# viridityzhu/HiFiHR

Hardware: AMD Instinct MI355X
Metric: train images/sec, FreiHAND 224x224 (ResNet-18 + MANO LBS + render + losses + Adam) (higher is better)
Workload: dtype f32; 1 GPU; BASELINE configs[1]: FreiHAND batch=32/GPU, ResNet-18 encoder + MANO LBS + silhouette/texture render losses, 224x224, aa=3 (672^2 samples); per_gpu_batch=32, global_batch=32, parallelism=dp1

## Files before the change

### hifihr_amd/_lib.py

```python
from __future__ import annotations

import ctypes
import os
import struct
from ctypes import POINTER, c_double, c_float, c_int, c_int32, c_long, c_size_t, c_void_p

import numpy as np
import torch

_HERE = os.path.dirname(os.path.abspath(__file__))
LIB_PATH = os.path.join(_HERE, "libhifihr.so")

_c_float_p = POINTER(c_float)
_c_int_p = POINTER(c_int32)


class _LinearDesc(ctypes.Structure):
    _fields_ = [("x", c_void_p), ("w", c_void_p), ("b", c_void_p), ("y", c_void_p), ("B", c_int), ("I", c_int), ("O", c_int), ("act", c_int),
                ("dy", c_void_p), ("dz_scratch", c_void_p), ("dW_acc", c_void_p), ("db_acc", c_void_p), ("dx", c_void_p)]


class HifihrError(RuntimeError):
    pass

# ... 161 lines not shown
        self._run("hifihr_mano_lbs_bwd", h, pose, beta, saved, gverts, gjtr, pose.shape[0], gpose, gbeta)

    def mano_joints_fwd(self, h, verts, root_id, joints_rel, verts_rel, root):
        self._run("hifihr_mano_joints_fwd", h, verts, verts.shape[0], root_id, joints_rel, verts_rel, root)

    def mano_joints_bwd(self, h, gjoints_rel, gverts_rel, groot, root_id, gverts):
        self._run("hifihr_mano_joints_bwd", h, gjoints_rel, gverts_rel, groot, gverts.shape[0], root_id, gverts)

    def mano_full_fwd(self, h, pose, beta, root_id, root_xyz, verts, joints_rel, verts_rel, verts_cam, root, saved):
        self._run("hifihr_mano_full_fwd", h, pose, beta, pose.shape[0], root_id, root_xyz, verts, joints_rel, verts_rel, verts_cam, root, saved)

    def mano_full_bwd(self, h, pose, beta, saved, gjoints_rel, gverts_rel, gverts_cam, groot, root_id, gpose, gbeta, gpose_add=None,
                      gbeta_add=None):
        self._run("hifihr_mano_full_bwd", h, pose, beta, saved, gjoints_rel, gverts_rel, gverts_cam, groot, gpose_add, gbeta_add,
                  pose.shape[0], root_id, gpose, gbeta)

    def lbs_create(self, v_template, shapedirs, j_regressor, weights, parents) -> c_void_p:
        V, J, S = int(v_template.shape[0]), int(weights.shape[1]), int(shapedirs.shape[2])
        assert shapedirs.shape == (V, 3, S) and j_regressor.shape == (J, V) and weights.shape == (V, J) and len(parents) == J
        h = c_void_p()
        keep = [_host_f32(a) for a in (v_template, shapedirs, j_regressor, weights)] + [_host_i32(parents)]
        self._run("hifihr_lbs_create", ctypes.byref(h), V, J, S, *[k[1] for k in keep])
        return h

    def lbs_destroy(self, h):
        self._call("hifihr_lbs_destroy", h)

    def lbs_fwd(self, h, theta, beta, verts, joints):
        self._run("hifihr_lbs_fwd", h, theta, beta, theta.shape[0], verts, joints)

    def lbs_bwd(self, h, theta, beta, gverts, gjoints, scratch, gtheta, gbeta):
        self._run("hifihr_lbs_bwd", h, theta, beta, gverts, gjoints, theta.shape[0], scratch, gtheta, gbeta)

    def conv2d_workspace_bytes(self, N, H, W, C, K, R, S, stride, pad, bwd_data=False):
        return self._call("hifihr_conv2d_workspace_bytes", N, H, W, C, K, R, S, stride, pad, bool(bwd_data))

    def conv2d_fwd(self, x, w, bias, y, N, H, W, C, K, R, S, stride, pad, ws=None, act=0):
        self._run("hifihr_conv2d_fwd", x, w, bias, act, y, N, H, W, C, K, R, S, stride, pad, ws, _nbytes(ws))

    def bias_relu_bwd(self, dy, y, M, C, g, db_acc):
        self._run("hifihr_bias_relu_bwd", dy, y, M, C, g, db_acc)

    def conv2d_fwd_bnstats(self, x, w, y, stats, N, H, W, C, K, R, S, stride, pad, ws=None):
        self._run("hifihr_conv2d_fwd_bnstats", x, w, y, stats, N, H, W, C, K, R, S, stride, pad, ws, _nbytes(ws))

    def conv2d_fwd_bnstats_pair_supported(self, N, H, W, C, stride, K1, R1, pad1, K2, R2, pad2):
        return bool(self._call("hifihr_conv2d_fwd_bnstats_pair_supported", N, H, W, C, stride, K1, R1, pad1, K2, R2, pad2))

    def conv2d_fwd_bnstats_pair(self, x, w1, y1, stats1, K1, R1, pad1, w2, y2, stats2, K2, R2, pad2, N, H, W, C, stride):
        self._run("hifihr_conv2d_fwd_bnstats_pair", x, w1, y1, stats1, K1, R1, pad1, w2, y2, stats2, K2, R2, pad2, N, H, W, C, stride)

    def bn_stats_floats(self, C):
        return self._call("hifihr_bn_stats_floats", C)

    def bn_stats(self, x, M, C, stats):
        self._run("hifihr_bn_stats", x, M, C, stats)

    def bn_act_fwd(self, x, stats, gamma, beta, residual, act, M, C, eps, momentum, y, save_mean, save_invstd, rmean, rvar):
        self._run("hifihr_bn_act_fwd", x, stats, gamma, beta, residual, act, M, C, eps, momentum, y, save_mean, save_invstd, rmean, rvar)

    def bn_act_eval(self, x, rmean, rvar, gamma, beta, residual, act, M, C, eps, y):
        self._run("hifihr_bn_act_eval", x, rmean, rvar, gamma, beta, residual, act, M, C, eps, y)

    def bn_act_bwd(self, dy, y, x, save_mean, save_invstd, gamma, beta, act, M, C, red, dx, dres, dgamma_acc, dbeta_acc):
        self._run("hifihr_bn_act_bwd", dy, y, x, save_mean, save_invstd, gamma, beta, act, M, C, red, dx, dres, dgamma_acc, dbeta_acc)

    def bn_relu_maxpool_supported(self, N, H, W, C):
        return bool(self._call("hifihr_bn_relu_maxpool_supported", N, H, W, C))

    def bn_relu_maxpool_fwd(self, x, stats, gamma, beta, N, H, W, C, eps, momentum, pooled, tap, save_mean, save_invstd, running_mean,
                            running_var):
        self._run("hifihr_bn_relu_maxpool_fwd", x, stats, gamma, beta, N, H, W, C, eps, momentum, pooled, tap, save_mean, save_invstd,
                  running_mean, running_var)

    def bn_relu_maxpool_bwd_y(self, gy, pooled, tap, x, save_mean, save_invstd, gamma, beta, N, H, W, C, red, dx, dgamma_acc, dbeta_acc):
        self._run("hifihr_bn_relu_maxpool_bwd_y", gy, pooled, tap, x, save_mean, save_invstd, gamma, beta, N, H, W, C, red, dx, dgamma_acc,
                  dbeta_acc)

    def bn_relu_maxpool_bwd(self, gy, tap, x, save_mean, save_invstd, gamma, beta, N, H, W, C, red, dx, dgamma_acc, dbeta_acc):
        self._run("hifihr_bn_relu_maxpool_bwd", gy, tap, x, save_mean, save_invstd, gamma, beta, N, H, W, C, red, dx, dgamma_acc, dbeta_acc)

    def conv2d_bwd_weight_c3_supported(self, N, H, W, K, R, S, stride, pad):
        return bool(self._call("hifihr_conv2d_bwd_weight_c3_supported", N, H, W, K, R, S, stride, pad))

    def conv2d_bwd_weight_c3(self, x4, dy, dw3, N, H, W, K, R, S, stride, pad, ws):
        self._run("hifihr_conv2d_bwd_weight_c3", x4, dy, dw3, N, H, W, K, R, S, stride, pad, ws, _nbytes(ws))

    def dwconv2d_fwd(self, x, w, y, N, H, W, C, OH, OW, K, stride, pt, pl, stats=None):
        self._run("hifihr_dwconv2d_fwd", x, w, y, stats, N, H, W, C, OH, OW, K, stride, pt, pl)

    def dwconv2d_fwd_bnswish(self, x, mean, invstd, gamma, beta, w, y, N, H, W, C, OH, OW, K, stride, pt, pl, stats=None):
        self._run("hifihr_dwconv2d_fwd_bnswish", x, mean, invstd, gamma, beta, w, y, stats, N, H, W, C, OH, OW, K, stride, pt, pl)

    def dwconv2d_bwd_weight_bnswish(self, x, mean, invstd, gamma, beta, dy, dw, N, H, W, C, OH, OW, K, stride, pt, pl):
        self._run("hifihr_dwconv2d_bwd_weight_bnswish", x, mean, invstd, gamma, beta, dy, dw, N, H, W, C, OH, OW, K, stride, pt, pl)

    def bn_finalize_fwd(self, stats, M, C, eps, momentum, save_mean, save_invstd, rmean, rvar):
        self._run("hifihr_bn_finalize_fwd", stats, M, C, eps, momentum, save_mean, save_invstd, rmean, rvar)

    def dwconv2d_bwd_data(self, dy, w, dx, N, H, W, C, OH, OW, K, stride, pt, pl):
        self._run("hifihr_dwconv2d_bwd_data", dy, w, dx, N, H, W, C, OH, OW, K, stride, pt, pl)

    def dwconv2d_bwd_weight(self, x, dy, dw, N, H, W, C, OH, OW, K, stride, pt, pl):
        self._run("hifihr_dwconv2d_bwd_weight", x, dy, dw, N, H, W, C, OH, OW, K, stride, pt, pl)

    def light_split_fwd(self, lights, colors, directions):
        self._run("hifihr_light_split_fwd", lights, lights.shape[0], colors, directions)

    def light_split_bwd(self, lights, gcolors, gdirections, glights):
        self._run("hifihr_light_split_bwd", lights, gcolors, gdirections, lights.shape[0], glights)

    def loss_total_fwd(self, parts, counts, total):
        n = len(parts)
        self._run("hifihr_loss_total_fwd", _fp_table(parts), (c_int * n)(*[int(c) for c in counts]), n, total)

    def loss_total_bwd(self, gtotal, grads, counts):
        n = len(grads)
        self._run("hifihr_loss_total_bwd", gtotal, _fp_table(grads), (c_int * n)(*[int(c) for c in counts]), (c_int * n)(*[int(t.numel()) for t in grads]), n)

    def joint_terms_fwd(self, j2d, j2d_gt, joints, joints_gt, mse, lam3, out):
        ref = j2d if j2d is not None else joints
        self._run("hifihr_joint_terms_fwd", j2d, j2d_gt, joints, joints_gt, ref.shape[0], ref.shape[1], mse, _floats(lam3, 3), out)

    def joint_terms_bwd(self, j2d, j2d_gt, joints, joints_gt, mse, lam3, gout, g_j2d, g_joints):
        ref = j2d if j2d is not None else joints
        self._run("hifihr_joint_terms_bwd", j2d, j2d_gt, joints, joints_gt, ref.shape[0], ref.shape[1], mse, _floats(lam3, 3), gout, g_j2d,
                  g_joints)

    def geom_loss_fwd(self, joints, joints_gt, verts, verts_gt, shape, pose, faces, mse, lam, partial, out):
        B, J, V = joints.shape[0], joints.shape[1], verts.shape[1]
        F = 0 if faces is None else faces.shape[0]
        NS = 0 if shape is None else shape.shape[1]
        NP = 0 if pose is None else pose.shape[1]
        self._run("hifihr_geom_loss_fwd", joints, joints_gt, verts, verts_gt, shape, pose, faces, B, J, V, F, NS, NP, mse, _floats(lam, 5),
                  partial, out)

    def geom_loss_bwd(self, joints, joints_gt, verts, verts_gt, shape, pose, faces, vf_off, vf_idx, mse, lam, gout, gj, gv, gshape,
                      gpose):
        B, J, V = joints.shape[0], joints.shape[1], verts.shape[1]
        F = 0 if faces is None else faces.shape[0]
        NS = 0 if shape is None else shape.shape[1]
        NP = 0 if pose is None else pose.shape[1]
        self._run("hifihr_geom_loss_bwd", joints, joints_gt, verts, verts_gt, shape, pose, faces, vf_off, vf_idx, B, J, V, F, NS, NP, mse,
                  _floats(lam, 5), gout, gj, gv, gshape, gpose)

    def photo_loss_partial_floats(self):
        return self._call("hifihr_photo_loss_partial_floats")

    def photo_loss_fwd(self, rgba, imgs, seg, l_tex, l_mrgb, l_sil, re_img_m, mask_rgbs, partial, out):
        B, _, H, W = rgba.shape
        assert seg.dtype == torch.int64 and seg.is_contiguous() and rgba.is_contiguous() and imgs.is_contiguous()
        self._run("hifihr_photo_loss_fwd", rgba, imgs, seg, B, H, W, l_tex, l_mrgb, l_sil, re_img_m, mask_rgbs, partial, out)

    def photo_loss_bwd(self, rgba, re_img_m, mask_rgbs, g_re_img, gout, fwd_out, l_tex, l_mrgb, grad_rgba):
        B, _, H, W = rgba.shape
        self._run("hifihr_photo_loss_bwd", rgba, re_img_m, mask_rgbs, g_re_img, gout, fwd_out, B, H, W, l_tex, l_mrgb, grad_rgba)

    def sil_post(self, rgba, imgs, re_sil, mask_rgbs):
        B, _, H, W = rgba.shape
        assert rgba.is_contiguous() and (imgs is None or imgs.is_contiguous())
        self._run("hifihr_sil_post", rgba, imgs, B, H, W, re_sil, mask_rgbs)

    def wino_tile(self, N, H, W, C, K):
        return self._call("hifihr_wino_tile", N, H, W, C, K)

    def wino_gemm_workspace_bytes(self, N, H, W, C, K, m=2):
        return self._call("hifihr_wino_gemm_workspace_bytes", N, H, W, C, K, m)

    def wino4_bwd_gemm_pair_supported(self, N, H, W, C, K):
        key = (N, H, W, C, K)
        hit = self._pair_ok.get(key)
        if hit is None:
            hit = self._pair_ok[key] = bool(self._call("hifihr_wino4_bwd_gemm_pair_supported", N, H, W, C, K))
        return hit

    def wino4_bwd_gemm_pair(self, V2, U2, M2, Vx, Yt, dU_parts, N, H, W, C, K, parts):
        self._run("hifihr_wino4_bwd_gemm_pair", V2, U2, M2, Vx, Yt, dU_parts, N, H, W, C, K, parts)

    def wino_weight_transform(self, w, U, K, C, flip, m=2):
        self._run("hifihr_wino_weight_transform", w, U, K, C, flip, m)

    def wino_input_transform(self, x, V, N, H, W, C, m=2):
        self._run("hifihr_wino_input_transform", x, V, N, H, W, C, m)

    def zero_page_ready(self, device=None):
        idx = torch.cuda.current_device() if device is None else torch.device(device).index
        idx = torch.cuda.current_device() if idx is None else idx
        if idx in self._zero_page:
            return True
        with torch.cuda.device(idx):
            ok = bool(self._call("hifihr_zero_page_ready", stream=torch.cuda.current_stream(idx).cuda_stream))
        if ok:
            self._zero_page.add(idx)
        return ok

    def conv3x3_c64_wino_supported(self, N, H, W, C, K):
        return bool(self._call("hifihr_conv3x3_c64_wino_supported", N, H, W, C, K))

    def conv3x3_c64_wino(self, x, U, bias, relu, y, stats, N, H, W):
        self._run("hifihr_conv3x3_c64_wino", x, U, bias, bool(relu), y, stats, N, H, W)

    def conv3x3_c64_wino_res(self, x, U, res, y, N, H, W):
        self._run("hifihr_conv3x3_c64_wino_res", x, U, res, y, N, H, W)

    def conv3x3_c64_bwd_pair_supported(self, N, H, W):
        return bool(self._call("hifihr_conv3x3_c64_bwd_pair_supported", N, H, W))

    def conv3x3_c64_bwd_pair(self, dy, U_bwd, res, dx, x, dw, N, H, W, ws=None):
        self._run("hifihr_conv3x3_c64_bwd_pair", dy, U_bwd, res, dx, x, dw, ws, _nbytes(ws), N, H, W)

    def conv3x3_c64_bwd_pair_slabs(self, dy, U_bwd, res, dx, x, slabs, N, H, W):
        n = c_int32(0)
        self._run("hifihr_conv3x3_c64_bwd_pair_slabs", dy, U_bwd, res, dx, x, slabs, _nbytes(slabs), N, H, W, ctypes.byref(n))
        return n.value

    def conv_halo_wgrad_reduce_multi(self, jobs):
        raw = b"".join(struct.pack("<QQii", sl.data_ptr(), dw.data_ptr(), int(n), 0) for sl, n, dw in jobs)
        buf = ctypes.create_string_buffer(raw, len(raw))
        self._run("hifihr_conv_halo_wgrad_reduce_multi", ctypes.cast(buf, c_void_p), len(jobs), stream=jobs[0][0])

    def wino_bn_input_supported(self, C, m):
        return bool(self._call("hifihr_wino_bn_input_supported", C, m))

    def wino_bn_input_transform(self, x, stats, gamma, beta, residual, out, V, N, H, W, C, m, eps, momentum, save_mean, save_invstd,
                                running_mean, running_var):
        self._run("hifihr_wino_bn_input_transform", x, stats, gamma, beta, residual, out, V, N, H, W, C, m, eps, momentum, save_mean,
                  save_invstd, running_mean, running_var)

    def wino_output_transform_bnred(self, Mm, x, out, gadd, save_mean, save_invstd, gamma, beta, red, g, N, H, W, C, m):
        self._run("hifihr_wino_output_transform_bnred", Mm, x, out, gadd, save_mean, save_invstd, gamma, beta, red, g, N, H, W, C, m)

    def wino_bn_bwd_dual_transform(self, g, y, save_mean, save_invstd, gamma, red, V, Yt, N, H, W, K, m, dgamma_acc, dbeta_acc):
        self._run("hifihr_wino_bn_bwd_dual_transform", g, y, save_mean, save_invstd, gamma, red, V, Yt, N, H, W, K, m, dgamma_acc, dbeta_acc)

    def bn_bwd_apply(self, g, x, save_mean, save_invstd, gamma, M, C, red, dx, dgamma_acc, dbeta_acc):
        self._run("hifihr_bn_bwd_apply", g, x, save_mean, save_invstd, gamma, M, C, red, dx, dgamma_acc, dbeta_acc)

    def wino_gemm(self, V, U, M, N, H, W, C, K, ws=None, m=2):
        self._run("hifihr_wino_gemm", V, U, M, N, H, W, C, K, m, ws, _nbytes(ws))

    def wino_input_dy_transform(self, dy, V, Yt, N, H, W, K, m=2):
        self._run("hifihr_wino_input_dy_transform", dy, V, Yt, N, H, W, K, m)

    def conv2d_bwd_data_pre(self, dy, wt, dx, N, H, W, C, K, R, S, stride, pad, ws=None):
        self._run("hifihr_conv2d_bwd_data_pre", dy, wt, dx, N, H, W, C, K, R, S, stride, pad, ws, _nbytes(ws))

    def conv2d_bwd_data_pre_res(self, dy, wt, res, dx, N, H, W, C, K, R, S, stride, pad, ws=None):
        self._run("hifihr_conv2d_bwd_data_pre_res", dy, wt, res, dx, N, H, W, C, K, R, S, stride, pad, ws, _nbytes(ws))

    def conv2d_bwd_data_pre_plus1x1_supported(self, N, H, W, C, K, R, S, stride, pad):
        return bool(self._call("hifihr_conv2d_bwd_data_pre_plus1x1_supported", N, H, W, C, K, R, S, stride, pad))

    def conv2d_bwd_data_pre_plus1x1(self, dy, wt, dy2, wt2, dx, N, H, W, C, K, R, S, stride, pad):
        self._run("hifihr_conv2d_bwd_data_pre_plus1x1", dy, wt, dy2, wt2, dx, N, H, W, C, K, R, S, stride, pad)

    def conv2d_bwd_weight_plus1x1_supported(self, N, H, W, C, K, R, S, stride, pad):
        return bool(self._call("hifihr_conv2d_bwd_weight_plus1x1_supported", N, H, W, C, K, R, S, stride, pad))

    def conv2d_bwd_weight_plus1x1(self, x, dy, dw, dy2, dw2, N, H, W, C, K, R, S, stride, pad):
        self._run("hifihr_conv2d_bwd_weight_plus1x1", x, dy, dw, dy2, dw2, N, H, W, C, K, R, S, stride, pad)

    @staticmethod
    def prep_jobs(jobs, device):
        raw = b"".join(struct.pack("<QQiiii", s.data_ptr(), d.data_ptr(), K, C, RS, kind) for s, d, K, C, RS, kind in jobs)
        return torch.frombuffer(bytearray(raw), dtype=torch.uint8).to(device)

    def weight_prep(self, table, njobs, blocks_per_job=64):
        self._run("hifihr_weight_prep", table, njobs, blocks_per_job)

    def freihand_batch(self, img_rgbx, mask, Ks, joints, verts, scales, packed, B, out, root_id=None, image_size=None):
        n, H, W = img_rgbx.shape
        J, V = joints.shape[1], verts.shape[1]
        g = out.get
        for k in ("segms_gt", "idxs"):
            assert g(k) is None or g(k).dtype == torch.int64
        for t in out.values():
            assert t.is_contiguous()
        batch = (img_rgbx, mask, Ks, joints, verts, scales, J, V, packed, B, H, W, g("imgs"), g("masks"), g("segms_gt"), g("Ks"), g("Ps"),
                 g("joints"), g("verts"), g("j2d_gt"), g("scales"), g("idxs"))
        if root_id is None:
            self._run("hifihr_freihand_batch", *batch)
            return
        self._run("hifihr_freihand_batch_step", *batch, root_id, image_size or H, g("root_xyz"), g("joints_rel"), g("verts_rel"), g("cam_ndc"))

    def ho3d_workspace_bytes(self, B, out_size):
        return self._call("hifihr_ho3d_workspace_bytes", B, out_size)

    def ho3d_batch(self, img_rgbx, hand_mask, Ks, uv21, xyz21, packed, B, out_size, ws, out):
        n, FH, FW = img_rgbx.shape
        g = out.get
        for t in out.values():
            assert t.is_contiguous() and t.dtype == torch.float32
        self._run("hifihr_ho3d_batch", img_rgbx, hand_mask, Ks, uv21, xyz21, FH, FW, packed, B, out_size, ws, _nbytes(ws), g("img_crop"),
                  g("hand_mask_crop"), g("K_crop"), g("uv21_crop"), g("xyz21"))

    def freihand_augment(self, img_rgbx, mask, idx, coef_fix, out_img, out_mask):
        ref = img_rgbx if img_rgbx is not None else mask
        self._run("hifihr_freihand_augment", img_rgbx, mask, idx, coef_fix, idx.shape[0], ref.shape[1], ref.shape[2], out_img, out_mask)

    def procrustes_error(self, pred, gt, aligned, err_sum):
        self._run("hifihr_procrustes_error", pred, gt, pred.shape[0], pred.shape[1], aligned, err_sum)

    def point_error_hist(self, pred, gt, vis, thresholds, hist, sum_d):
        (thr, thr_p), n, K = _host_f64(thresholds), pred.shape[0], pred.shape[1]
        assert vis is None or (vis.dtype == torch.uint8 and vis.is_contiguous() and tuple(vis.shape) == (n, K))
        assert sum_d.dtype == torch.float64 and sum_d.is_contiguous() and tuple(hist.shape) == (K, len(thr) + 1) and tuple(sum_d.shape) == (K,)
# ... 464 lines not shown
```

### hifihr_amd/csrc/hifihr_api.hip

```cpp
#include <hip/hip_runtime.h>

#include <algorithm>
#include <array>
#include <cmath>
#include <cstdarg>
#include <cstdio>
#include <cstring>
#include <new>
#include <vector>

#include "../../include/hifihr.h"
#include "hifihr_internal.h"
#include "mano_math.h"

namespace {

thread_local char g_err[512] = "";

int fail(int code, const char* fmt, ...) {
  va_list ap;
  va_start(ap, fmt);
  vsnprintf(g_err, sizeof(g_err), fmt, ap);
  va_end(ap);
  return code;
// ... 1138 lines not shown
}

int hifihr_dwconv2d_bwd_data(const float* dy, const float* w, float* dx, int N, int H, int W, int C, int OH, int OW, int K, int stride,
                             int pad_top, int pad_left, void* stream) {
  if (!dy || !w || !dx || !dw_ok(N, H, W, C, OH, OW, K, stride, pad_top, pad_left)) return fail(HIFIHR_EINVAL, "hifihr_dwconv2d_bwd_data: bad argument (C % 4 == 0; K 3 or 5; stride 1 or 2; 0 <= pad <= K - 1; -(stride - 1) <= implied bottom / right pad <= K - 1)");
  hifihr::DwGeom g{N, H, W, C, OH, OW, K, stride, pad_top, pad_left};
  HIP_TRY(hifihr::launch_dwconv_bwd_data(g, dy, w, dx, (hipStream_t)stream));
  return HIFIHR_OK;
}

int hifihr_dwconv2d_bwd_weight(const float* x, const float* dy, float* dw, int N, int H, int W, int C, int OH, int OW, int K,
                               int stride, int pad_top, int pad_left, void* stream) {
  if (!x || !dy || !dw || !dw_ok(N, H, W, C, OH, OW, K, stride, pad_top, pad_left)) return fail(HIFIHR_EINVAL, "hifihr_dwconv2d_bwd_weight: bad argument (C % 4 == 0; K 3 or 5; stride 1 or 2; 0 <= pad <= K - 1; -(stride - 1) <= implied bottom / right pad <= K - 1)");
  hifihr::DwGeom g{N, H, W, C, OH, OW, K, stride, pad_top, pad_left};
  HIP_TRY(hifihr::launch_dwconv_bwd_weight(g, x, dy, dw, (hipStream_t)stream));
  return HIFIHR_OK;
}

int hifihr_mmpool_fwd(const float* x, const float* p, int B, int HW, int C, float* y, int* argmax, float* xmax, float* xavg,
                      void* stream) {
  if (!x || !p || !y || !argmax || !xmax || !xavg || B <= 0 || HW <= 0 || C < 4 || C % 4 != 0)
    return fail(HIFIHR_EINVAL, "hifihr_mmpool_fwd: bad argument (C % 4 == 0)");
  HIP_TRY(hifihr::launch_mmpool_fwd(x, p, B, HW, C, y, argmax, xmax, xavg, (hipStream_t)stream));
  return HIFIHR_OK;
}

int hifihr_mmpool_bwd(const float* gy, const float* p, const int* argmax, const float* xmax, const float* xavg, int B, int HW, int C,
                      float* dx, float* dp_acc, void* stream) {
  if (!gy || !p || !argmax || !xmax || !xavg || !dx || B <= 0 || HW <= 0 || C < 4 || C % 4 != 0)
    return fail(HIFIHR_EINVAL, "hifihr_mmpool_bwd: bad argument (C % 4 == 0)");
  HIP_TRY(hifihr::launch_mmpool_bwd(gy, p, argmax, xmax, xavg, B, HW, C, dx, dp_acc, (hipStream_t)stream));
  return HIFIHR_OK;
}

static int pool_ok(int k, int s, int p) { return (k == 3 && s == 2 && p == 1) || (k == 3 && s == 1 && p == 1) || (k == 2 && s == 2 && p == 0); }

int hifihr_maxpool2d_fwd(const float* x, int N, int H, int W, int C, int k, int s, int p, float* y, unsigned char* tap, void* stream) {
  if (!x || !y || !tap || N <= 0 || H <= 0 || W <= 0 || C < 4 || C % 4 != 0 || !pool_ok(k, s, p) || H + 2 * p < k || W + 2 * p < k)
    return fail(HIFIHR_EINVAL, "hifihr_maxpool2d_fwd: bad argument (C % 4 == 0; (k,s,p) in {(3,2,1), (3,1,1), (2,2,0)})");
  HIP_TRY(hifihr::launch_maxpool_fwd(x, N, H, W, C, k, s, p, y, tap, (hipStream_t)stream));
  return HIFIHR_OK;
}

int hifihr_maxpool2d_bwd(const float* gy, const unsigned char* tap, int N, int H, int W, int C, int k, int s, int p, float* dx,
                         void* stream) {
  if (!gy || !tap || !dx || N <= 0 || H <= 0 || W <= 0 || C < 4 || C % 4 != 0 || !pool_ok(k, s, p) || H + 2 * p < k || W + 2 * p < k)
    return fail(HIFIHR_EINVAL, "hifihr_maxpool2d_bwd: bad argument (C % 4 == 0; (k,s,p) in {(3,2,1), (3,1,1), (2,2,0)})");
  HIP_TRY(hifihr::launch_maxpool_bwd(gy, tap, nullptr, N, H, W, C, k, s, p, dx, (hipStream_t)stream));
  return HIFIHR_OK;
}

int hifihr_maxpool2d_fwd_flat(const float* x, int N, int H, int W, int C, int k, int s, int p, float* y_flat, unsigned char* tap, void* stream) {
  if (!x || !y_flat || !tap || N <= 0 || H <= 0 || W <= 0 || C < 4 || C % 4 != 0 || !pool_ok(k, s, p) || H + 2 * p < k || W + 2 * p < k)
    return fail(HIFIHR_EINVAL, "hifihr_maxpool2d_fwd_flat: bad argument (C % 4 == 0; (k,s,p) in {(3,2,1), (3,1,1), (2,2,0)})");
  HIP_TRY(hifihr::launch_maxpool_flat(x, tap, N, H, W, C, k, s, p, y_flat, 0, (hipStream_t)stream));
  return HIFIHR_OK;
}

int hifihr_maxpool2d_bwd_flat(const float* gy_flat, const unsigned char* tap, int N, int H, int W, int C, int k, int s, int p, float* dx, void* stream) {
  if (!gy_flat || !dx || !tap || N <= 0 || H <= 0 || W <= 0 || C < 4 || C % 4 != 0 || !pool_ok(k, s, p) || H + 2 * p < k || W + 2 * p < k)
    return fail(HIFIHR_EINVAL, "hifihr_maxpool2d_bwd_flat: bad argument (C % 4 == 0; (k,s,p) in {(3,2,1), (3,1,1), (2,2,0)})");
  HIP_TRY(hifihr::launch_maxpool_flat(gy_flat, const_cast<unsigned char*>(tap), N, H, W, C, k, s, p, dx, 1, (hipStream_t)stream));
  return HIFIHR_OK;
}

int hifihr_maxpool2d_bwd_relu(const float* gy, const unsigned char* tap, const float* y, int N, int H, int W, int C, int k, int s, int p,
                              float* dx, void* stream) {
  if (!gy || !tap || !y || !dx || N <= 0 || H <= 0 || W <= 0 || C < 4 || C % 4 != 0 || !pool_ok(k, s, p) || H + 2 * p < k || W + 2 * p < k)
    return fail(HIFIHR_EINVAL, "hifihr_maxpool2d_bwd_relu: bad argument (C % 4 == 0; (k,s,p) in {(3,2,1), (3,1,1), (2,2,0)})");
  HIP_TRY(hifihr::launch_maxpool_bwd(gy, tap, y, N, H, W, C, k, s, p, dx, (hipStream_t)stream));
  return HIFIHR_OK;
}

int hifihr_bias_relu_bwd(const float* dy, const float* y, long M, int C, float* g, float* db_acc, void* stream) {
  if (!dy || !y || !g || M <= 0 || C < 4 || C % 4 != 0 || C > 256)
    return fail(HIFIHR_EINVAL, "hifihr_bias_relu_bwd: bad argument (C % 4 == 0, C <= 256)");
  HIP_TRY(hifihr::launch_bias_relu_bwd(dy, y, M, C, g, db_acc, (hipStream_t)stream));
  return HIFIHR_OK;
}

static int geom_args(hifihr::GeomLossArgs& a, const float* joints, const float* joints_gt, const float* verts, const float* verts_gt,
                     const float* shape, const float* pose, const int32_t* faces, int B, int J, int V, int F, int NS, int NP, int mse,
                     const float* lambda5) {
  if (!joints || !joints_gt || !verts || !verts_gt || !lambda5 || B <= 0 || J <= 0 || V <= 0 || F < 0 || NS < 0 || NP < 0 ||
      (F > 0 && !faces) || (NS > 0 && !shape) || (NP > 0 && !pose))
    return 0;
  a.joints = joints; a.joints_gt = joints_gt; a.verts = verts; a.verts_gt = verts_gt; a.shape = shape; a.pose = pose;
  a.faces = F > 0 ? faces : nullptr; a.vf_off = nullptr; a.vf_idx = nullptr;
  a.B = B; a.J = J; a.V = V; a.F = F; a.NS = NS; a.NP = NP; a.mse = mse ? 1 : 0;
  for (int k = 0; k < 5; ++k) a.lambda[k] = lambda5[k];
  return 1;
}

int hifihr_geom_loss_fwd(const float* joints, const float* joints_gt, const float* verts, const float* verts_gt, const float* shape,
                         const float* pose, const int32_t* faces, int B, int J, int V, int F, int NS, int NP, int mse,
                         const float* lambda5, float* partial, float* out, void* stream) {
  hifihr::GeomLossArgs a;
  if (!partial || !out || !geom_args(a, joints, joints_gt, verts, verts_gt, shape, pose, faces, B, J, V, F, NS, NP, mse, lambda5))
    return fail(HIFIHR_EINVAL, "hifihr_geom_loss_fwd: bad argument");
  HIP_TRY(hifihr::launch_geom_loss_fwd(a, partial, out, (hipStream_t)stream));
  return HIFIHR_OK;
}

int hifihr_joint_terms_fwd(const float* j2d, const float* j2d_gt, const float* joints, const float* joints_gt, int B, int J, int mse,
                           const float* lam3_host, float* out3, void* stream) {
  if ((!j2d && !joints) || (j2d && !j2d_gt) || (joints && !joints_gt) || !lam3_host || !out3 || B <= 0 || J != 21)
    return fail(HIFIHR_EINVAL, "hifihr_joint_terms_fwd: bad argument (J must be 21)");
  HIP_TRY(hifihr::launch_joint_terms_fwd(j2d, j2d_gt, joints, joints_gt, B, J, mse, lam3_host, out3, (hipStream_t)stream));
  return HIFIHR_OK;
}

int hifihr_joint_terms_bwd(const float* j2d, const float* j2d_gt, const float* joints, const float* joints_gt, int B, int J, int mse,
                           const float* lam3_host, const float* gout3, float* g_j2d, float* g_joints, void* stream) {
  if ((!j2d && !joints) || (j2d && !j2d_gt) || (joints && !joints_gt) || !lam3_host || !gout3 || B <= 0 || J != 21 || (g_j2d && !j2d) ||
      (g_joints && !joints))
    return fail(HIFIHR_EINVAL, "hifihr_joint_terms_bwd: bad argument (J must be 21)");
  HIP_TRY(hifihr::launch_joint_terms_bwd(j2d, j2d_gt, joints, joints_gt, B, J, mse, lam3_host, gout3, g_j2d, g_joints, (hipStream_t)stream));
  return HIFIHR_OK;
}

int hifihr_geom_loss_bwd(const float* joints, const float* joints_gt, const float* verts, const float* verts_gt, const float* shape,
                         const float* pose, const int32_t* faces, const int32_t* vf_off, const int32_t* vf_idx, int B, int J, int V,
                         int F, int NS, int NP, int mse, const float* lambda5, const float* gout, float* gj, float* gv, float* gshape,
                         float* gpose, void* stream) {
  hifihr::GeomLossArgs a;
  if (!gout || (F > 0 && (!vf_off || !vf_idx)) ||
      !geom_args(a, joints, joints_gt, verts, verts_gt, shape, pose, faces, B, J, V, F, NS, NP, mse, lambda5))
    return fail(HIFIHR_EINVAL, "hifihr_geom_loss_bwd: bad argument");
  a.vf_off = vf_off; a.vf_idx = vf_idx;
  HIP_TRY(hifihr::launch_geom_loss_bwd(a, gout, gj, gv, gshape, gpose, (hipStream_t)stream));
  return HIFIHR_OK;
}

int hifihr_photo_loss_partial_floats(void) { return hifihr::photo_loss_partial_floats(); }

int hifihr_photo_loss_fwd(const float* rgba, const float* imgs, const int64_t* seg, int B, int H, int W, float l_tex, float l_mrgb,
                          float l_sil, float* re_img_m, float* mask_rgbs, float* partial, float* out, void* stream) {
  if (!rgba || !imgs || !seg || !re_img_m || !mask_rgbs || !partial || !out || B <= 0 || H <= 0 || W <= 0 || (H * W) % 4 != 0)
    return fail(HIFIHR_EINVAL, "hifihr_photo_loss_fwd: bad argument (H*W % 4 == 0)");
  HIP_TRY(hifihr::launch_photo_loss_fwd(rgba, imgs, (const long long*)seg, B, H * W, l_tex, l_mrgb, l_sil, re_img_m, mask_rgbs, partial,
                                        out, (hipStream_t)stream));
  return HIFIHR_OK;
}

int hifihr_photo_loss_bwd(const float* rgba, const float* re_img_m, const float* mask_rgbs, const float* g_re_img, const float* gout,
                          const float* fwd_out, int B, int H, int W, float l_tex, float l_mrgb, float* grad_rgba, void* stream) {
  if (!rgba || !re_img_m || !mask_rgbs || !fwd_out || !grad_rgba || B <= 0 || H <= 0 || W <= 0 || (H * W) % 4 != 0)
    return fail(HIFIHR_EINVAL, "hifihr_photo_loss_bwd: bad argument (H*W % 4 == 0)");
  HIP_TRY(hifihr::launch_photo_loss_bwd(rgba, re_img_m, mask_rgbs, g_re_img, gout, fwd_out, B, H * W, l_tex, l_mrgb, grad_rgba,
                                        (hipStream_t)stream));
  return HIFIHR_OK;
}

int hifihr_sil_post(const float* rgba, const float* imgs, int B, int H, int W, float* re_sil, float* mask_rgbs, void* stream) {
  if (!rgba || !re_sil || (mask_rgbs && !imgs) || B <= 0 || H <= 0 || W <= 0 || (H * W) % 4 != 0)
    return fail(HIFIHR_EINVAL, "hifihr_sil_post: bad argument (H*W % 4 == 0)");
  HIP_TRY(hifihr::launch_sil_post(rgba, imgs, B, H * W, re_sil, mask_rgbs, (hipStream_t)stream));
  return HIFIHR_OK;
}

int hifihr_light_split_fwd(const float* lights, int B, float* colors, float* directions, void* stream) {
  if (!lights || !colors || !directions || B <= 0) return fail(HIFIHR_EINVAL, "hifihr_light_split_fwd: bad argument");
  HIP_TRY(hifihr::launch_light_split_fwd(lights, B, colors, directions, (hipStream_t)stream));
  return HIFIHR_OK;
}

int hifihr_light_split_bwd(const float* lights, const float* gcolors, const float* gdirections, int B, float* glights, void* stream) {
  if (!lights || !glights || B <= 0) return fail(HIFIHR_EINVAL, "hifihr_light_split_bwd: bad argument");
  HIP_TRY(hifihr::launch_light_split_bwd(lights, gcolors, gdirections, B, glights, (hipStream_t)stream));
  return HIFIHR_OK;
}

int hifihr_loss_total_fwd(const float* const* parts, const int* counts, int nparts, float* total, void* stream) {
  if (!parts || !counts || !total || nparts < 1 || nparts > hifihr::kLossTotalParts) return fail(HIFIHR_EINVAL, "hifihr_loss_total_fwd: 1 .. 4 parts");
  hifihr::LossTotalParts p{};
  for (int i = 0; i < nparts; ++i) {
    if (!parts[i] || counts[i] < 0 || counts[i] > 64) return fail(HIFIHR_EINVAL, "hifihr_loss_total_fwd: bad part");
    p.v[i] = parts[i]; p.n[i] = counts[i];
  }
  HIP_TRY(hifihr::launch_loss_total_fwd(p, total, (hipStream_t)stream));
  return HIFIHR_OK;
}

int hifihr_loss_total_bwd(const float* gtotal, float* const* grads, const int* counts, const int* lengths, int nparts, void* stream) {
  if (!gtotal || !grads || !counts || !lengths || nparts < 1 || nparts > hifihr::kLossTotalParts)
    return fail(HIFIHR_EINVAL, "hifihr_loss_total_bwd: 1 .. 4 parts");
  hifihr::LossTotalGrads q{};
  for (int i = 0; i < nparts; ++i) {
    if (!grads[i] || counts[i] < 0 || lengths[i] < counts[i] || lengths[i] > 64) return fail(HIFIHR_EINVAL, "hifihr_loss_total_bwd: bad part");
    q.g[i] = grads[i]; q.n[i] = counts[i]; q.len[i] = lengths[i];
  }
  HIP_TRY(hifihr::launch_loss_total_bwd(gtotal, q, (hipStream_t)stream));
  return HIFIHR_OK;
}

int hifihr_linear_fwd(const float* x, const float* w, const float* b, int B, int I, int O, int act, const float* gamma, const float* beta,
                      float eps, float momentum, float* running_mean, float* running_var, float* y, float* z, float* save_mean,
                      float* save_invstd, void* stream) {
  if (!x || !w || !y || B <= 0 || I <= 0 || O <= 0 || act < 0 || act > 3 || (act >= 2 && gamma) || (act == 2 && !z))
    return fail(HIFIHR_EINVAL, "hifihr_linear_fwd: bad argument (act 0..3; swish / sigmoid take no batch-norm; swish needs z)");
  if (gamma && (!beta || !z || !save_mean || !save_invstd || B > 64 || ((running_mean != nullptr) != (running_var != nullptr))))
    return fail(HIFIHR_EINVAL, "hifihr_linear_fwd: batch-norm needs beta, z, save_mean, save_invstd and B <= 64");
  hifihr::LinearArgs a{x, w, b, y, z, gamma, beta, save_mean, save_invstd, running_mean, running_var, eps, momentum, B, I, O, act};
  HIP_TRY(hifihr::launch_linear_fwd(a, (hipStream_t)stream));
  return HIFIHR_OK;
}

static int group_member_ok(const hifihr_linear_desc& d) {
  return d.x && d.w && d.y && d.B > 0 && d.I > 0 && d.O > 0 && (d.act == 0 || d.act == 1);
}

int hifihr_linear_fwd_group(const hifihr_linear_desc* descs, int n, void* stream) {
  if (!descs || n <= 0 || n > hifihr::kMaxLinearGroup) return fail(HIFIHR_EINVAL, "hifihr_linear_fwd_group: 1..6 members");
  hifihr::LinearGroup grp{};
  grp.n = n;
  for (int i = 0; i < n; ++i) {
    const hifihr_linear_desc& d = descs[i];
    if (!group_member_ok(d)) return fail(HIFIHR_EINVAL, "hifihr_linear_fwd_group: bad member (x, w, y, sizes; act 0 / 1)");
    grp.a[i] = hifihr::LinearArgs{d.x, d.w, d.b, d.y, nullptr, nullptr, nullptr, nullptr, nullptr, nullptr, nullptr, 0.f, 0.f, d.B, d.I, d.O, d.act};
  }
  HIP_TRY(hifihr::launch_linear_fwd_group(grp, (hipStream_t)stream));
  return HIFIHR_OK;
}

int hifihr_linear_bwd_group(const hifihr_linear_desc* descs, int n, void* stream) {
  if (!descs || n <= 0 || n > hifihr::kMaxLinearGroup) return fail(HIFIHR_EINVAL, "hifihr_linear_bwd_group: 1..6 members");
  hifihr::LinearGroup grp{};
  hifihr::LinearGradsGroup gg{};
  grp.n = n;
  for (int i = 0; i < n; ++i) {
    const hifihr_linear_desc& d = descs[i];
    if (!group_member_ok(d) || !d.dy || !d.dz_scratch) return fail(HIFIHR_EINVAL, "hifihr_linear_bwd_group: bad member (dy, dz_scratch, y for act 1)");
    grp.a[i] = hifihr::LinearArgs{d.x, d.w, nullptr, d.y, nullptr, nullptr, nullptr, nullptr, nullptr, nullptr, nullptr, 0.f, 0.f, d.B, d.I, d.O, d.act};
    gg.g[i] = hifihr::LinearGrads{d.dy, d.dz_scratch, d.dW_acc, d.db_acc, nullptr, nullptr, d.dx};
  }
  HIP_TRY(hifihr::launch_linear_bwd_group(grp, gg, (hipStream_t)stream));
  return HIFIHR_OK;
}

int hifihr_linear_bwd(const float* dy, const float* y, const float* x, const float* w, int B, int I, int O, int act, const float* gamma,
                      const float* z, const float* save_mean, const float* save_invstd, float* dz_scratch, float* dW_acc, float* db_acc,
                      float* dgamma_acc, float* dbeta_acc, float* dx, void* stream) {
  if (!dy || !x || !w || B <= 0 || I <= 0 || O <= 0 || act < 0 || act > 3 || ((act == 1 || act == 3) && !y) ||
      (act == 2 && !z) || (act >= 2 && gamma) || (dx && !dz_scratch))
    return fail(HIFIHR_EINVAL, "hifihr_linear_bwd: bad argument (act 1 / 3 need y, act 2 needs z; swish / sigmoid take no batch-norm; dx needs dz_scratch)");
  if (gamma && (!z || !save_mean || !save_invstd || B > 64))
    return fail(HIFIHR_EINVAL, "hifihr_linear_bwd: batch-norm needs z, save_mean, save_invstd and B <= 64");
  hifihr::LinearArgs a{x, w, nullptr, const_cast<float*>(y), const_cast<float*>(z), gamma, nullptr, const_cast<float*>(save_mean),
                       const_cast<float*>(save_invstd), nullptr, nullptr, 0.f, 0.f, B, I, O, act};
  hifihr::LinearGrads g{dy, dz_scratch, dW_acc, db_acc, dgamma_acc, dbeta_acc, dx};
  HIP_TRY(hifihr::launch_linear_bwd(a, g, (hipStream_t)stream));
  return HIFIHR_OK;
}

int hifihr_se_pool(const float* x, int B, int HW, int C, float* mean_zeroed, void* stream) {
  if (!x || !mean_zeroed || B <= 0 || HW <= 0 || C < 4 || C % 4 != 0) return fail(HIFIHR_EINVAL, "hifihr_se_pool: bad argument (C % 4 == 0)");
  HIP_TRY(hifihr::launch_se_pool(x, B, HW, C, mean_zeroed, (hipStream_t)stream));
  return HIFIHR_OK;
}

int hifihr_se_scale(const float* x, const float* gate, const float* add, float add_scale, int B, int HW, int C, float* y, void* stream) {
  if (!x || !gate || !y || B <= 0 || HW <= 0 || C < 4 || C % 4 != 0) return fail(HIFIHR_EINVAL, "hifihr_se_scale: bad argument (C % 4 == 0)");
  HIP_TRY(hifihr::launch_se_scale(x, gate, add, add_scale, B, HW, C, y, (hipStream_t)stream));
  return HIFIHR_OK;
}

int hifihr_se_bwd_gate(const float* dy, const float* x, int B, int HW, int C, float* dgate_zeroed, void* stream) {
  if (!dy || !x || !dgate_zeroed || B <= 0 || HW <= 0 || C < 4 || C % 4 != 0)
    return fail(HIFIHR_EINVAL, "hifihr_se_bwd_gate: bad argument (C % 4 == 0)");
  HIP_TRY(hifihr::launch_se_bwd_gate(dy, x, B, HW, C, dgate_zeroed, (hipStream_t)stream));
  return HIFIHR_OK;
}

int hifihr_se_mlp_supported(int C, int SQ) { return hifihr::se_mlp_supported(C, SQ) ? 1 : 0; }

int hifihr_drop_connect_add(const float* x, const float* skip, const float* u, float keep, int B, size_t per_sample, float* out, void* stream) {
  if (!x || !u || !out || B <= 0 || per_sample == 0 || per_sample % 4 != 0 || !(keep > 0.f))
    return fail(HIFIHR_EINVAL, "hifihr_drop_connect_add: bad argument (per_sample % 4 == 0, keep > 0)");
  HIP_TRY(hifihr::launch_drop_connect_add(x, skip, u, keep, B, per_sample, out, (hipStream_t)stream));
  return HIFIHR_OK;
}

int hifihr_se_mlp_fwd(float* mean_acc, const float* w1, const float* b1, const float* w2t, const float* b2, int B, int C, int SQ, float* mean,
                      float* z1, float* h1, float* gate, void* stream) {
  if (!mean_acc || !w1 || !b1 || !w2t || !b2 || !mean || !z1 || !h1 || !gate || B <= 0 || !hifihr::se_mlp_supported(C, SQ))
    return fail(HIFIHR_EINVAL, "hifihr_se_mlp_fwd: bad argument (C % 4 == 0, C <= 4096, SQ <= 256)");
  HIP_TRY(hifihr::launch_se_mlp_fwd(mean_acc, w1, b1, w2t, b2, B, C, SQ, mean, z1, h1, gate, (hipStream_t)stream));
  return HIFIHR_OK;
}

int hifihr_se_mlp_bwd(float* dgate_acc, const float* gate, const float* z1, const float* h1, const float* mean, const float* w1, const float* w2t,
                      int B, int C, int SQ, float* dz2, float* dz1, float* dmean, float* dw1_acc, float* db1_acc, float* dw2_acc, float* db2_acc,
                      void* stream) {
  if (!dgate_acc || !gate || !z1 || !h1 || !mean || !w1 || !w2t || !dz2 || !dz1 || !dmean || !dw1_acc || !db1_acc || !dw2_acc || !db2_acc ||
      B <= 0 || !hifihr::se_mlp_supported(C, SQ))
    return fail(HIFIHR_EINVAL, "hifihr_se_mlp_bwd: bad argument (C % 4 == 0, C <= 4096, SQ <= 256)");
  HIP_TRY(hifihr::launch_se_mlp_bwd(dgate_acc, gate, z1, h1, mean, w1, w2t, B, C, SQ, dz2, dz1, dmean, dw1_acc, db1_acc, dw2_acc, db2_acc,
                                    (hipStream_t)stream));
  return HIFIHR_OK;
}

int hifihr_weight_transpose(const float* w, float* wt, int K, int RS, int C, void* stream) {
  if (!w || !wt || K <= 0 || RS <= 0 || C <= 0) return fail(HIFIHR_EINVAL, "hifihr_weight_transpose: bad argument");
  HIP_TRY(hifihr::launch_weight_transpose(w, wt, K, RS, C, (hipStream_t)stream));
  return HIFIHR_OK;
}
// ... 397 lines not shown
```

### hifihr_amd/csrc/hifihr_internal.h

```cpp
#pragma once
#include <hip/hip_runtime.h>

#include <cstdint>
#include <cstdlib>
#include <stdint.h>

#include "render_math.h"

namespace hifihr {

inline int device_cus() {
  static int cus = 0;
  if (cus == 0) {
    int dev = 0;
    hipDeviceProp_t prop;
    if (hipGetDevice(&dev) == hipSuccess && hipGetDeviceProperties(&prop, dev) == hipSuccess && prop.multiProcessorCount > 0) cus = prop.multiProcessorCount;
  }
  return cus > 0 ? cus : 256;
}

static inline int env_int(const char* name, int unset) {
  const char* e = getenv(name);
  return e ? atoi(e) : unset;
}
// ... 71 lines not shown
hipError_t launch_soft_sil_fwd(const RenderDev& r, const float* verts, const float* cam, int B, float sigma, float blur, float* alpha,
                               float* neglog, void* ws, hipStream_t st);
hipError_t launch_soft_sil_bwd(const RenderDev& r, const float* verts, const float* cam, const float* neglog, const float* galpha, int B,
                               float sigma, float blur, float* gverts, void* ws, hipStream_t st);
hipError_t launch_soft_sil_loss_fwd(const float* alpha, const void* mask, int mask_i64, int B, int HW, float lam_s, float lam_i, double* sums,
                                    float* out, hipStream_t st);
hipError_t launch_soft_sil_loss_bwd(const float* alpha, const void* mask, int mask_i64, const double* sums, const float* gout, int B, int HW,
                                    float lam_s, float lam_i, float* galpha, hipStream_t st);

size_t render_depth_workspace_bytes(const RenderDev& r, int B);
hipError_t launch_render_depth_fwd(const RenderDev& r, const float* verts, const float* cam, const int* face_id, int B, float* depth, int* hits,
                                   hipStream_t st);
hipError_t launch_render_depth_bwd(const RenderDev& r, const float* verts, const float* cam, const int* face_id, const float* gdepth,
                                   const int* hits, int B, float* gverts, void* ws, hipStream_t st);
hipError_t launch_depth_loss_fwd(const float* depth, const int* hits, const float* target, const void* mask, int mask_i64, int B, int HW, float lam,
                                 float trunc, double* sums, float* out, hipStream_t st);
hipError_t launch_depth_loss_bwd(const float* depth, const int* hits, const float* target, const void* mask, int mask_i64, const double* sums,
                                 const float* gout, int B, int HW, float lam, float trunc, float* gdepth, hipStream_t st);

struct ConvGeom {
  int N, IH, IW, IC, OH, OW, OC, R, S, stride, pad, dgrad;
  int relu;
  int batch;
  long src_bs, wgt_bs, dst_bs;
  const float* residual = nullptr;
  const float* src2 = nullptr;
  const float* wgt2 = nullptr;
};
hipError_t launch_conv_igemm(const ConvGeom& g, const float* src, const float* wgt, const float* bias, float* dst, float* stats,
                             void* sk_ws, size_t sk_ws_bytes, hipStream_t st);
size_t conv_sk_workspace_bytes(const ConvGeom& g);
void conv_describe(const ConvGeom& g, char* out, int cap);
void conv_wgrad_describe(const ConvGeom& g, char* out, int cap);
bool conv_wgrad_plus1x1_supported(const ConvGeom& g);
hipError_t launch_conv_wgrad_plus1x1(const ConvGeom& g, const float* x, const float* dy, float* dw, const float* dy2, float* dw2, hipStream_t st);
bool conv_halo_supported(const ConvGeom& g, const float* bias);
const float* conv_halo_zero_page(hipStream_t st);
bool conv_stem_supported(const ConvGeom& g, const float* bias);
hipError_t launch_conv_stem(const ConvGeom& g, const float* src, const float* wgt, float* dst, float* stats, const float* zeros, hipStream_t st);
bool conv_stem_wgrad_supported(const ConvGeom& g);
size_t conv_stem_wgrad_slab_bytes();
hipError_t launch_conv_stem_wgrad(const ConvGeom& g, const float* x, const float* dy, float* dw, float* slabs_or_null, hipStream_t st,
                                  int dw_channels = 4);
bool conv_halo_wgrad_supported(const ConvGeom& g);
size_t conv_halo_wgrad_slab_bytes();
hipError_t launch_conv_halo_wgrad(const ConvGeom& g, const float* x, const float* dy, float* dw, float* slabs_or_null, hipStream_t st);
bool conv_wino2_supported(int N, int H, int W, int C, int K);
hipError_t launch_conv_wino2(const float* src, const float* U, const float* bias_or_null, int relu, float* dst, float* stats_or_null, int N,
                             int H, int W, hipStream_t st, const float* res_or_null = nullptr);
bool conv_c64_bwd_pair_supported(int N, int H, int W);
hipError_t launch_conv_c64_bwd_pair(const float* dy, const float* U_bwd, const float* res_or_null, float* dx, const float* x, float* dw,
                                    float* slabs_or_null, int N, int H, int W, hipStream_t st, int* nslab_out = nullptr);
struct HaloReduceJob { const float* slabs; float* dw; int nslab; };
hipError_t launch_conv_halo_wgrad_reduce_multi(const HaloReduceJob* jobs, int njobs, hipStream_t st);
hipError_t launch_conv_halo(const ConvGeom& g, const float* src, const float* wgt, const float* bias_or_null, float* dst, float* stats,
                            const float* zeros, hipStream_t st);
constexpr int kStatSlots = 32;
__host__ __device__ inline int stat_slots_used(int C) { return C >= 512 ? 8 : (C >= 256 ? 16 : 32); }
constexpr int kStatCounters = 64;
__host__ __device__ inline size_t stat_fwd_doubles(int C) { return (size_t)kStatSlots * 2 * C; }
__host__ __device__ inline unsigned* stat_fwd_counters(float* stats, int C) {
  return reinterpret_cast<unsigned*>(reinterpret_cast<double*>(stats) + stat_fwd_doubles(C));
}
__host__ __device__ inline unsigned* stat_bwd_counters(float* red, int C) { return reinterpret_cast<unsigned*>(red + (size_t)kStatSlots * 2 * C); }
__host__ __device__ inline float* stat_bwd_totals(float* red, int C) { return red + (size_t)kStatSlots * 4 * C + kStatCounters; }
__host__ __device__ inline int stat_buffer_floats(int C) { return kStatSlots * 4 * C + kStatCounters + 2 * C; }
#if defined(__HIPCC__) || defined(HIFIHR_HOSTSIM)
__device__ __forceinline__ void stat_unshift(int n, float k, float s, float q, double& S1, double& S2) {
  const double kd = (double)k, sd = (double)s, nd = (double)n;
  S1 = nd * kd + sd;
  S2 = (double)q + 2.0 * kd * sd + nd * kd * kd;
}
__device__ __forceinline__ void stat_atomic_add(double* p, double v) { unsafeAtomicAdd(p, v); }
struct Stat4 {
  float4 k, s, q;
  int n;
  __device__ __forceinline__ Stat4() : k(make_float4(0.f, 0.f, 0.f, 0.f)), s(k), q(k), n(0) {}
  __device__ __forceinline__ void seed(const float4& v) {
    if (n == 0) k = v;
  }
  __device__ __forceinline__ void add(const float4& v) {
    const float dx = v.x - k.x, dy = v.y - k.y, dz = v.z - k.z, dw = v.w - k.w;
    s.x += dx; s.y += dy; s.z += dz; s.w += dw;
    q.x = fmaf(dx, dx, q.x); q.y = fmaf(dy, dy, q.y); q.z = fmaf(dz, dz, q.z); q.w = fmaf(dw, dw, q.w);
    ++n;
  }
  __device__ __forceinline__ void fold16(double (*red)[16][16][4], int tl, int cl, bool mine, double* slot, int C) const {
    double S1[4], S2[4];
    stat_unshift(n, k.x, s.x, q.x, S1[0], S2[0]); stat_unshift(n, k.y, s.y, q.y, S1[1], S2[1]);
    stat_unshift(n, k.z, s.z, q.z, S1[2], S2[2]); stat_unshift(n, k.w, s.w, q.w, S1[3], S2[3]);
#pragma unroll
    for (int e = 0; e < 4; ++e) { red[0][tl][cl][e] = S1[e]; red[1][tl][cl][e] = S2[e]; }
    __syncthreads();
    if (tl == 0 && mine) {
      for (int r = 1; r < 16; ++r)
#pragma unroll
        for (int e = 0; e < 4; ++e) { S1[e] += red[0][r][cl][e]; S2[e] += red[1][r][cl][e]; }
#pragma unroll
      for (int e = 0; e < 4; ++e) { stat_atomic_add(slot + e, S1[e]); stat_atomic_add(slot + C + e, S2[e]); }
    }
  }
};
#endif
hipError_t launch_bn_stats(const float* x, long M, int C, float* stats, hipStream_t st);
hipError_t launch_bn_act_fwd(const float* x, float* stats, const float* gamma, const float* beta, const float* residual,
                             int relu, long M, int C, float eps, float momentum, float* y, float* save_mean, float* save_invstd,
                             float* running_mean, float* running_var, hipStream_t st);
hipError_t launch_bn_act_eval(const float* x, const float* running_mean, const float* running_var, const float* gamma, const float* beta,
                              const float* residual, int act, long M, int C, float eps, float* y, hipStream_t st);
hipError_t launch_bn_act_bwd(const float* dy, const float* y, const float* x, const float* save_mean, const float* save_invstd,
                             const float* gamma, const float* beta, int act, long M, int C, float* red, float* dx, float* dres,
                             float* dgamma_acc, float* dbeta_acc, hipStream_t st);
bool bn_relu_maxpool_supported(int N, int H, int W, int C);
hipError_t launch_bn_relu_maxpool_fwd(const float* x, float* stats, const float* gamma, const float* beta, int N, int H, int W, int C,
                                      float eps, float momentum, float* y, unsigned char* tap, float* save_mean, float* save_invstd,
                                      float* running_mean, float* running_var, hipStream_t st);
hipError_t launch_bn_relu_maxpool_bwd(const float* gy, const unsigned char* tap, const float* x, const float* save_mean,
                                      const float* save_invstd, const float* gamma, const float* beta, int N, int H, int W, int C, float* red,
                                      float* dx, float* dgamma_acc, float* dbeta_acc, hipStream_t st, const float* pooled = nullptr);
size_t conv_wgrad_workspace_bytes(const ConvGeom& g);
hipError_t launch_conv_wgrad(const ConvGeom& g, const float* x, const float* dy, float* dw, void* ws, size_t ws_bytes, hipStream_t st);
bool conv_is_gemm(const ConvGeom& g);
bool conv_wgrad_c3_supported(const ConvGeom& g);
hipError_t launch_conv_wgrad_c3(const ConvGeom& g, const float* x, const float* dy, float* dw3, void* ws, size_t ws_bytes, hipStream_t st);
hipError_t launch_weight_transpose(const float* w, float* wt, int K, int RS, int C, hipStream_t st);
hipError_t launch_image_to_nhwc4(const float* img, float* out, int B, int H, int W, int OH, int OW, int pt, int pl, int normalize,
                                 hipStream_t st);

hipError_t launch_image_scale_to_nhwc4(const float* img, float* out, int B, int H, int W, const float* shift3, const float* scale3,
                                       hipStream_t st);
hipError_t launch_maxpool_notap(const float* x, int N, int H, int W, int C, int k, int s, int p, float* y, hipStream_t st);
int lpips_tap_max_channels();
size_t lpips_tap_partial_floats(int B);
hipError_t launch_lpips_tap(const float* f0, const float* f1, const float* w, int B, int HW, int C, int accumulate, float* partial, float* val,
                            hipStream_t st);
hipError_t launch_lpips_tap_bwd(const float* f0, const float* f1, const float* w, const float* gval, int B, int HW, int C, int accumulate,
                                int relu_mask, float* gf0, hipStream_t st);
hipError_t launch_lpips_maxpool_fwd(const float* x, int N, int H, int W, int C, float* y, hipStream_t st);
hipError_t launch_lpips_maxpool_bwd(const float* gy, const float* x, int N, int H, int W, int C, float* dx, hipStream_t st);
hipError_t launch_image_scale_to_nhwc4_bwd(const float* g4, float* gimg, int B, int H, int W, const float* scale3, hipStream_t st);
bool lpips_stem_bwd_data_supported(int N, int H, int W, int C, int K, int R, int S, int stride, int pad);
hipError_t launch_lpips_stem_bwd_data(const float* dy, const float* w, float* dx, int N, int H, int W, int C, int K, int R, int S, int stride, int pad,
                                      hipStream_t st);

struct SsimWindow {
  float g[11];
};
int ssim_tile_edge();
hipError_t launch_ssim_fwd(const SsimWindow& win, const float* img1, const float* img2, int planes, int H, int W, float* partial,
                           float* dA, float* dB, float* dC, hipStream_t st);
hipError_t launch_ssim_bwd(const SsimWindow& win, const float* img1, const float* img2, const float* dA, const float* dB,
                           const float* dC, const float* gscale, int planes, int H, int W, float* gimg1, hipStream_t st, float out_scale = 1.0f);
hipError_t launch_ssim_finish(const float* partial, int count, float scale, float offset, float* out, hipStream_t st);

struct DwGeom {
  int N, H, W, C, OH, OW, K, stride, pt, pl;
};
hipError_t launch_dwconv_fwd(const DwGeom& g, const float* x, const float* w, float* y, float* stats, hipStream_t st,
                             const float* pre_mean = nullptr, const float* pre_invstd = nullptr, const float* pre_gamma = nullptr,
                             const float* pre_beta = nullptr);
hipError_t launch_dwconv_bwd_data(const DwGeom& g, const float* dy, const float* w, float* dx, hipStream_t st);
hipError_t launch_dwconv_bwd_weight(const DwGeom& g, const float* x, const float* dy, float* dw, hipStream_t st,
                                    const float* pre_mean = nullptr, const float* pre_invstd = nullptr, const float* pre_gamma = nullptr,
                                    const float* pre_beta = nullptr);
hipError_t launch_bn_finalize_fwd(float* stats, long M, int C, float eps, float momentum, float* save_mean, float* save_invstd,
                                  float* running_mean, float* running_var, hipStream_t st);

hipError_t launch_mmpool_fwd(const float* x, const float* p, int B, int HW, int C, float* y, int* argmax, float* xmax, float* xavg,
                             hipStream_t st);
hipError_t launch_mmpool_bwd(const float* gy, const float* p, const int* argmax, const float* xmax, const float* xavg, int B, int HW,
                             int C, float* dx, float* dp_acc, hipStream_t st);
hipError_t launch_maxpool_flat(const float* x_or_gy, unsigned char* tap, int N, int H, int W, int C, int k, int s, int p, float* y_or_dx, int bwd,
                               hipStream_t st);
hipError_t launch_maxpool_fwd(const float* x, int N, int H, int W, int C, int k, int s, int p, float* y, unsigned char* tap,
                              hipStream_t st);
hipError_t launch_maxpool_bwd(const float* gy, const unsigned char* tap, const float* ymask, int N, int H, int W, int C, int k, int s, int p, float* dx,
                              hipStream_t st);
hipError_t launch_bias_relu_bwd(const float* dy, const float* y, long M, int C, float* g, float* db_acc, hipStream_t st);
hipError_t launch_light_split_fwd(const float* lights, int B, float* colors, float* dirs, hipStream_t st);
hipError_t launch_light_split_bwd(const float* lights, const float* gcolors, const float* gdirs, int B, float* glights, hipStream_t st);

struct GeomLossArgs {
  const float *joints, *joints_gt, *verts, *verts_gt, *shape, *pose;
  const int *faces, *vf_off, *vf_idx;
  int B, J, V, F, NS, NP, mse;
  float lambda[5];
};
hipError_t launch_geom_loss_fwd(const GeomLossArgs& a, float* partial, float* out, hipStream_t st);
hipError_t launch_geom_loss_bwd(const GeomLossArgs& a, const float* gout, float* gj, float* gv, float* gshape, float* gpose,
                                hipStream_t st);
int photo_loss_partial_floats();
hipError_t launch_photo_loss_fwd(const float* rgba, const float* imgs, const long long* seg, int B, int HW, float l_tex, float l_mrgb,
                                 float l_sil, float* re_img_m, float* mask_rgbs, float* partial, float* out, hipStream_t st);
hipError_t launch_photo_loss_bwd(const float* rgba, const float* re_img_m, const float* mask_rgbs, const float* g_re_img,
                                 const float* gout, const float* fwd_out, int B, int HW, float l_tex, float l_mrgb, float* grad_rgba,
                                 hipStream_t st);
hipError_t launch_sil_post(const float* rgba, const float* imgs, int B, int HW, float* re_sil, float* mask_rgbs, hipStream_t st);
constexpr int kLossTotalParts = 4;
struct LossTotalParts { const float* v[kLossTotalParts]; int n[kLossTotalParts]; };
struct LossTotalGrads { float* g[kLossTotalParts]; int n[kLossTotalParts]; int len[kLossTotalParts]; };
hipError_t launch_loss_total_fwd(const LossTotalParts& p, float* total, hipStream_t st);
hipError_t launch_loss_total_bwd(const float* gtotal, const LossTotalGrads& q, hipStream_t st);

struct MeshTopoDev {
  const int *nbr_off, *nbr_idx, *quads, *vq_off, *vq_idx;
  const float* deg;
  int V, E, Q;
};
int mesh_reg_blocks(const MeshTopoDev& t);
hipError_t launch_mesh_reg_fwd(const MeshTopoDev& t, const float* verts, int B, float lam_lap, float lam_nc, float* unit, float* partial,
                               float* out, hipStream_t st);
hipError_t launch_mesh_reg_bwd(const MeshTopoDev& t, const float* verts, const float* unit, const float* gout, int B, float lam_lap,
                               float lam_nc, float* gverts, hipStream_t st);

constexpr int kChamferQ = 256, kChamferTile = 512;
long long chamfer_chunks(int N, int M);
hipError_t launch_chamfer_fwd(const float* x, const float* y, int B, int N, int M, float w_xy, float w_yx, int* idx_xy, int* idx_yx,
                              double* min_xy, double* min_yx, double* sums, float* out, double* partial, hipStream_t st);
hipError_t launch_chamfer_bwd(const float* x, const float* y, const int* idx_xy, const int* idx_yx, const float* gout, int B, int N, int M,
                              float w_xy, float w_yx, float* gx, float* gy, hipStream_t st);

constexpr int kPointMeshPQ = 64, kPointMeshFT = 256, kPointMeshFQ = 128, kPointMeshPT = 512;
bool point_mesh_grid_ok(int B, int N, int V, int F);
size_t point_mesh_partial_doubles(int B, int N, int F);
hipError_t launch_point_mesh_fwd(const float* p, const float* v, const int* faces, int B, int N, int V, int F, float w_pf, float w_fp,
                                 int* idx_pf, double* bary_pf, double* min_pf, int* idx_fp, double* bary_fp, double* min_fp, double* sums,
                                 float* out, double* ws, hipStream_t st);
hipError_t launch_point_mesh_bwd(const float* p, const float* v, const int* faces, const int* idx_pf, const double* bary_pf, const int* idx_fp,
                                 const double* bary_fp, const float* gout, const int* v2c_off, const int* v2c_corner, int B, int N, int V, int F,
                                 float w_pf, float w_fp, float* gp, float* gv, double* ws, hipStream_t st);

__device__ __forceinline__ float fast_sigmoid(float z) {
#if defined(HIFIHR_HOSTSIM)
  return 1.0f / (1.0f + expf(-z));
#else
  return __builtin_amdgcn_rcpf(1.0f + __expf(-z));
#endif
}
struct LinearArgs {
  const float *x, *W, *b;
  float *y, *z;
  const float *gamma, *beta;
  float *save_mean, *save_invstd, *running_mean, *running_var;
  float eps, momentum;
  int B, I, O, act;
};
struct LinearGrads {
  const float* dy;
  float *dz, *dW_acc, *db_acc, *dgamma_acc, *dbeta_acc, *dx;
};
constexpr int kMaxLinearGroup = 6;
struct LinearGroup {
  LinearArgs a[kMaxLinearGroup];
  int n;
};
struct LinearGradsGroup {
  LinearGrads g[kMaxLinearGroup];
};
hipError_t launch_linear_fwd_group(const LinearGroup& grp, hipStream_t st);
hipError_t launch_linear_bwd_group(const LinearGroup& grp, const LinearGradsGroup& gg, hipStream_t st);
hipError_t launch_linear_fwd(const LinearArgs& a, hipStream_t st);
hipError_t launch_linear_bwd(const LinearArgs& a, const LinearGrads& g, hipStream_t st);

hipError_t launch_se_pool(const float* x, int B, int HW, int C, float* mean_zeroed, hipStream_t st);
hipError_t launch_se_bwd_gate(const float* dy, const float* x, int B, int HW, int C, float* dgate_zeroed, hipStream_t st);
hipError_t launch_se_scale(const float* x, const float* gate, const float* add, float ascale, int B, int HW, int C, float* y, hipStream_t st);
hipError_t launch_drop_connect_add(const float* x, const float* skip, const float* u, float keep, int B, size_t per_sample, float* out,
                                   hipStream_t st);
bool se_mlp_supported(int C, int SQ);
hipError_t launch_se_mlp_fwd(float* mean_acc, const float* W1, const float* b1, const float* W2T, const float* b2, int B, int C, int SQ,
                             float* mean_out, float* z1, float* h1, float* gate, hipStream_t st);
hipError_t launch_se_mlp_bwd(float* dgate_acc, const float* gate, const float* z1, const float* h1, const float* mean, const float* W1,
                             const float* W2T, int B, int C, int SQ, float* dz2, float* dz1, float* dmean, float* dW1_acc, float* db1_acc,
                             float* dW2_acc, float* db2_acc, hipStream_t st);

hipError_t launch_wino_weight_transform(const float* w, float* U, int K, int C, int flip, hipStream_t st);
hipError_t launch_wino_input_transform(const float* x, float* V, float* Y , int N, int H, int W, int C, hipStream_t st);
struct PrepJob {
  const float* src;
  float* dst;
  int K, C, RS, kind;
};
hipError_t launch_weight_prep(const PrepJob* jobs, int njobs, int blocks_per_job, hipStream_t st);
hipError_t launch_freihand_augment(const uint32_t* img, const uint8_t* mask, const int* idx, const int* coef, int B, int H, int W,
                                   float* out_img, float* out_mask, hipStream_t st);
struct BatchStepOut {
  int root_id;
  float image_size;
  float *oroot, *ojoints_rel, *overts_rel, *ocam;
};
hipError_t launch_freihand_batch(const uint32_t* img, const uint8_t* mask, const float* Ks, const float* joints, const float* verts,
                                 const float* scales, int J, int V, const int* packed, int B, int H, int W, float* out_img, float* out_mask,
                                 long long* out_segm, float* oKs, float* oPs, float* ojoints, float* overts, float* oj2d, float* oscales,
                                 long long* oidx, const BatchStepOut& step, hipStream_t st);
size_t ho3d_workspace_bytes(int B, int out_size);
hipError_t launch_ho3d_batch(const uint32_t* img, const uint8_t* mask, const float* Ks, const float* uv21, const float* xyz21, int FH, int FW,
                             const int* packed, int B, int out_size, void* ws, float* out_img, float* out_mask, float* out_K,
                             float* out_uv, float* out_xyz, hipStream_t st);
hipError_t launch_procrustes(const float* pred, const float* gt, int B, int N, float* aligned, float* err_sum, hipStream_t st);
constexpr int kHistMaxT = 128, kFscoreMaxT = 8;
struct HistThresholds { double v[kHistMaxT]; };
struct FscoreThresholds { double v[kFscoreMaxT]; };
bool thresholds_ok(const double* thr_h, int T, bool positive);
hipError_t launch_point_error_hist(const float* pred, const float* gt, const unsigned char* vis, int n, int K, const double* thr_h, int T,
                                   int* hist, double* sum, hipStream_t st);
hipError_t launch_fscore_counts(const float* pred, const float* gt, int B, int Np, int Ng, const double* thr_h, int T, int* counts,
// ... 98 lines not shown
```

### hifihr_amd/csrc/losses.hip

```cpp
#include <hip/hip_runtime.h>

#include "hifihr_internal.h"

namespace hifihr {

template <int K>
__device__ __forceinline__ void block_sum(float (&v)[K], float* lds ) {
#pragma unroll
  for (int k = 0; k < K; ++k) {
#pragma unroll
    for (int off = 32; off > 0; off >>= 1) v[k] += __shfl_down(v[k], off, 64);
  }
  const int lane = threadIdx.x & 63, wave = threadIdx.x >> 6;
  if (lane == 0) {
#pragma unroll
    for (int k = 0; k < K; ++k) lds[k * 4 + wave] = v[k];
  }
  __syncthreads();
  if (threadIdx.x == 0) {
#pragma unroll
    for (int k = 0; k < K; ++k) v[k] = (lds[k * 4] + lds[k * 4 + 1]) + (lds[k * 4 + 2] + lds[k * 4 + 3]);
  }
}

__device__ __forceinline__ float base_term(int mse, float d) { return mse ? d * d : fabsf(d); }
__device__ __forceinline__ float base_grad(int mse, float d) { return mse ? 2.f * d : (d > 0.f ? 1.f : (d < 0.f ? -1.f : 0.f)); }

__device__ __forceinline__ float edge_len(const float* __restrict__ v, int a, int b) {
  const float dx = v[3 * a] - v[3 * b], dy = v[3 * a + 1] - v[3 * b + 1], dz = v[3 * a + 2] - v[3 * b + 2];
  return sqrtf(dx * dx + dy * dy + dz * dz);
}

__global__ __launch_bounds__(256) void geom_loss_fwd_kernel(GeomLossArgs a, float* __restrict__ partial) {
  __shared__ float lds[5 * 4];
  const int b = blockIdx.x;
  float s[5] = {0.f, 0.f, 0.f, 0.f, 0.f};
  const float* j = a.joints + (size_t)b * a.J * 3, *jg = a.joints_gt + (size_t)b * a.J * 3;
  for (int i = threadIdx.x; i < a.J * 3; i += 256) s[0] += base_term(a.mse, j[i] - jg[i]);
  const float* v = a.verts + (size_t)b * a.V * 3, *vg = a.verts_gt + (size_t)b * a.V * 3;
  for (int i = threadIdx.x; i < a.V * 3; i += 256) s[1] += base_term(a.mse, v[i] - vg[i]);
  if (a.faces != nullptr) {
    for (int f = threadIdx.x; f < a.F; f += 256) {
      const int i0 = a.faces[3 * f], i1 = a.faces[3 * f + 1], i2 = a.faces[3 * f + 2];
      s[2] += fabsf(edge_len(v, i0, i1) - edge_len(vg, i0, i1)) + fabsf(edge_len(v, i0, i2) - edge_len(vg, i0, i2)) +
              fabsf(edge_len(v, i1, i2) - edge_len(vg, i1, i2));
    }
  }
  for (int i = threadIdx.x; i < a.NS; i += 256) { const float t = a.shape[(size_t)b * a.NS + i]; s[3] += t * t; }
  for (int i = threadIdx.x; i < a.NP; i += 256) { const float t = a.pose[(size_t)b * a.NP + i]; s[4] += t * t; }
  block_sum<5>(s, lds);
  if (threadIdx.x == 0) {
#pragma unroll
    for (int k = 0; k < 5; ++k) partial[b * 5 + k] = s[k];
  }
}

__global__ __launch_bounds__(64) void geom_loss_finish_kernel(GeomLossArgs a, const float* __restrict__ partial, float* __restrict__ out) {
  const int k = threadIdx.x;
  if (k >= 5) return;
  float s = 0.f;
  for (int b = 0; b < a.B; ++b) s += partial[b * 5 + k];
  const float cnt[5] = {(float)a.B * a.J * 3, (float)a.B * a.V * 3, (float)a.B * a.F * 3, (float)a.B * a.NS, (float)a.B * a.NP};
  out[k] = (cnt[k] > 0.f) ? a.lambda[k] * s / cnt[k] : 0.f;
}

__global__ __launch_bounds__(256) void geom_loss_bwd_kernel(GeomLossArgs a, const float* __restrict__ gout, float* __restrict__ gj,
                                                           float* __restrict__ gv, float* __restrict__ gshape, float* __restrict__ gpose) {
  const int b = blockIdx.x;
  const float cj = gout[0] * a.lambda[0] / ((float)a.B * a.J * 3), cv = gout[1] * a.lambda[1] / ((float)a.B * a.V * 3);
  const float ce = (a.F > 0) ? gout[2] * a.lambda[2] / ((float)a.B * a.F * 3) : 0.f;
  const float cs = gout[3] * a.lambda[3] * 2.f / ((float)a.B * a.NS), cp = gout[4] * a.lambda[4] * 2.f / ((float)a.B * a.NP);
  const float* j = a.joints + (size_t)b * a.J * 3, *jg = a.joints_gt + (size_t)b * a.J * 3;
  if (gj && blockIdx.y == 0)
    for (int i = threadIdx.x; i < a.J * 3; i += 256) gj[(size_t)b * a.J * 3 + i] = cj * base_grad(a.mse, j[i] - jg[i]);
  const float* v = a.verts + (size_t)b * a.V * 3, *vg = a.verts_gt + (size_t)b * a.V * 3;
  if (gv) {
    for (int vi = blockIdx.y * 256 + threadIdx.x; vi < a.V; vi += 256 * gridDim.y) {
      float g[3];
#pragma unroll
      for (int d = 0; d < 3; ++d) g[d] = cv * base_grad(a.mse, v[3 * vi + d] - vg[3 * vi + d]);
      if (a.faces != nullptr) {
        for (int e = a.vf_off[vi]; e < a.vf_off[vi + 1]; ++e) {
          const int f = a.vf_idx[e] >> 2, role = a.vf_idx[e] & 3;
#pragma unroll
          for (int o = 1; o <= 2; ++o) {
            const int u = a.faces[3 * f + (role + o) % 3];
            const float lp = edge_len(v, vi, u), lg = edge_len(vg, vi, u);
            const float sg = (lp > lg) ? 1.f : ((lp < lg) ? -1.f : 0.f);
            if (lp > 0.f) {
              const float k = ce * sg / lp;
#pragma unroll
              for (int d = 0; d < 3; ++d) g[d] += k * (v[3 * vi + d] - v[3 * u + d]);
            }
          }
        }
      }
#pragma unroll
      for (int d = 0; d < 3; ++d) gv[((size_t)b * a.V + vi) * 3 + d] = g[d];
    }
  }
  if (gshape && blockIdx.y == 0)
    for (int i = threadIdx.x; i < a.NS; i += 256) gshape[(size_t)b * a.NS + i] = cs * a.shape[(size_t)b * a.NS + i];
  if (gpose && blockIdx.y == 0)
    for (int i = threadIdx.x; i < a.NP; i += 256) gpose[(size_t)b * a.NP + i] = cp * a.pose[(size_t)b * a.NP + i];
}

hipError_t launch_geom_loss_fwd(const GeomLossArgs& a, float* partial, float* out, hipStream_t st) {
  hipLaunchKernelGGL(geom_loss_fwd_kernel, dim3(a.B), dim3(256), 0, st, a, partial);
  hipLaunchKernelGGL(geom_loss_finish_kernel, dim3(1), dim3(64), 0, st, a, partial, out);
  return hipGetLastError();
}

hipError_t launch_geom_loss_bwd(const GeomLossArgs& a, const float* gout, float* gj, float* gv, float* gshape, float* gpose,
                                hipStream_t st) {
  hipLaunchKernelGGL(geom_loss_bwd_kernel, dim3(a.B, gv != nullptr ? (a.V + 255) / 256 : 1), dim3(256), 0, st, a, gout, gj, gv, gshape, gpose);
  return hipGetLastError();
}

constexpr int kPhotoBlocks = 512;

__device__ __forceinline__ float sil_scale(float alpha) { return alpha > 0.f ? 1.0f : alpha / 255.0f; }

__global__ __launch_bounds__(256) void photo_loss_fwd_kernel(const float* __restrict__ rgba, const float* __restrict__ imgs,
                                                            const long long* __restrict__ seg, int B, int HW,
                                                            float* __restrict__ re_img_m, float* __restrict__ mask_rgbs,
                                                            float* __restrict__ partial) {
  __shared__ float lds[4 * 4];
  const int Q = HW / 4;
  float s[4] = {0.f, 0.f, 0.f, 0.f};
  for (size_t i = (size_t)blockIdx.x * 256 + threadIdx.x; i < (size_t)B * Q; i += (size_t)gridDim.x * 256) {
    const size_t b = i / Q, p = (i - b * Q) * 4;
    const float4 al = *reinterpret_cast<const float4*>(rgba + (b * 4 + 3) * HW + p);
    const float a4[4] = {al.x, al.y, al.z, al.w};
    float sc[4], sg[4];
#pragma unroll
    for (int e = 0; e < 4; ++e) {
      sc[e] = sil_scale(a4[e]);
      sg[e] = (float)seg[b * HW + p + e];
      const float re_sil = a4[e] > 0.f ? 255.0f : a4[e];
      s[3] += fabsf(re_sil - sg[e]);
    }
#pragma unroll
    for (int c = 0; c < 3; ++c) {
      const float4 r = *reinterpret_cast<const float4*>(rgba + (b * 4 + c) * HW + p);
      const float4 im = *reinterpret_cast<const float4*>(imgs + (b * 3 + c) * HW + p);
      const float4 rr = make_float4(r.x * sc[0], r.y * sc[1], r.z * sc[2], r.w * sc[3]);
      const float4 mm = make_float4(sg[0] * im.x, sg[1] * im.y, sg[2] * im.z, sg[3] * im.w);
      *reinterpret_cast<float4*>(re_img_m + (b * 3 + c) * HW + p) = rr;
      *reinterpret_cast<float4*>(mask_rgbs + (b * 3 + c) * HW + p) = mm;
      s[0] += fabsf(rr.x - mm.x) + fabsf(rr.y - mm.y) + fabsf(rr.z - mm.z) + fabsf(rr.w - mm.w);
      s[1] += (rr.x + rr.y) + (rr.z + rr.w);
      s[2] += (mm.x + mm.y) + (mm.z + mm.w);
    }
  }
  block_sum<4>(s, lds);
  if (threadIdx.x == 0) {
#pragma unroll
    for (int k = 0; k < 4; ++k) partial[blockIdx.x * 4 + k] = s[k];
  }
}

__global__ __launch_bounds__(256) void photo_loss_finish_kernel(const float* __restrict__ partial, int nblk, float n3, float n1,
                                                               float l_tex, float l_mrgb, float l_sil, float* __restrict__ out) {
  __shared__ float lds[4 * 4];
  float s[4] = {0.f, 0.f, 0.f, 0.f};
  for (int i = threadIdx.x; i < nblk; i += 256) {
#pragma unroll
    for (int k = 0; k < 4; ++k) s[k] += partial[i * 4 + k];
  }
  block_sum<4>(s, lds);
  if (threadIdx.x == 0) {
    const float dm = s[1] / n3 - s[2] / n3;
    out[0] = l_tex * s[0] / n3;
    out[1] = l_mrgb * dm * dm;
    out[2] = l_sil * s[3] / n1;
    out[3] = dm;
  }
}

__global__ __launch_bounds__(256) void photo_loss_bwd_kernel(const float* __restrict__ rgba, const float* __restrict__ re_img_m,
                                                            const float* __restrict__ mask_rgbs, const float* __restrict__ g_re_img,
                                                            const float* __restrict__ gout, const float* __restrict__ fwd_out, int B,
                                                            int HW, float n3, float l_tex, float l_mrgb, float* __restrict__ grad_rgba) {
  const int Q = HW / 4;
  const float kt = (gout ? gout[0] : 0.f) * l_tex / n3;
  const float km = (gout ? gout[1] : 0.f) * l_mrgb * 2.f * fwd_out[3] / n3;
  for (size_t i = (size_t)blockIdx.x * 256 + threadIdx.x; i < (size_t)B * Q; i += (size_t)gridDim.x * 256) {
    const size_t b = i / Q, p = (i - b * Q) * 4;
    const float4 al = *reinterpret_cast<const float4*>(rgba + (b * 4 + 3) * HW + p);
    const float sc[4] = {sil_scale(al.x), sil_scale(al.y), sil_scale(al.z), sil_scale(al.w)};
#pragma unroll
    for (int c = 0; c < 3; ++c) {
      const size_t o = (b * 3 + c) * HW + p;
      const float4 r = *reinterpret_cast<const float4*>(re_img_m + o), m = *reinterpret_cast<const float4*>(mask_rgbs + o);
      float4 g = g_re_img ? *reinterpret_cast<const float4*>(g_re_img + o) : make_float4(0.f, 0.f, 0.f, 0.f);
      g.x += kt * base_grad(0, r.x - m.x) + km; g.y += kt * base_grad(0, r.y - m.y) + km;
      g.z += kt * base_grad(0, r.z - m.z) + km; g.w += kt * base_grad(0, r.w - m.w) + km;
      *reinterpret_cast<float4*>(grad_rgba + (b * 4 + c) * HW + p) = make_float4(g.x * sc[0], g.y * sc[1], g.z * sc[2], g.w * sc[3]);
    }
    *reinterpret_cast<float4*>(grad_rgba + (b * 4 + 3) * HW + p) = make_float4(0.f, 0.f, 0.f, 0.f);
  }
}

__global__ __launch_bounds__(256) void sil_post_kernel(const float* __restrict__ rgba, const float* __restrict__ imgs, int B, int HW,
                                                      float* __restrict__ re_sil, float* __restrict__ mask_rgbs) {
  const int Q = HW / 4;
  for (size_t i = (size_t)blockIdx.x * 256 + threadIdx.x; i < (size_t)B * Q; i += (size_t)gridDim.x * 256) {
    const size_t b = i / Q, p = (i - b * Q) * 4;
    const float4 al = *reinterpret_cast<const float4*>(rgba + (b * 4 + 3) * HW + p);
    *reinterpret_cast<float4*>(re_sil + b * HW + p) =
        make_float4(al.x > 0.f ? 255.f : al.x, al.y > 0.f ? 255.f : al.y, al.z > 0.f ? 255.f : al.z, al.w > 0.f ? 255.f : al.w);
    if (mask_rgbs != nullptr) {
#pragma unroll
      for (int c = 0; c < 3; ++c) {
        const float4 im = *reinterpret_cast<const float4*>(imgs + (b * 3 + c) * HW + p);
        *reinterpret_cast<float4*>(mask_rgbs + (b * 3 + c) * HW + p) =
            make_float4(al.x > 0.f ? im.x : 0.f, al.y > 0.f ? im.y : 0.f, al.z > 0.f ? im.z : 0.f, al.w > 0.f ? im.w : 0.f);
      }
    }
  }
}

int photo_loss_partial_floats() { return kPhotoBlocks * 4; }

static unsigned photo_grid(int B, int HW) {
  size_t blocks = ((size_t)B * (HW / 4) + 255) / 256;
  if (blocks > (size_t)kPhotoBlocks) blocks = kPhotoBlocks;
  if (blocks < 1) blocks = 1;
  return (unsigned)blocks;
}

hipError_t launch_photo_loss_fwd(const float* rgba, const float* imgs, const long long* seg, int B, int HW, float l_tex, float l_mrgb,
                                 float l_sil, float* re_img_m, float* mask_rgbs, float* partial, float* out, hipStream_t st) {
  if (HW % 4 != 0) return hipErrorInvalidValue;
  const unsigned nblk = photo_grid(B, HW);
  hipLaunchKernelGGL(photo_loss_fwd_kernel, dim3(nblk), dim3(256), 0, st, rgba, imgs, seg, B, HW, re_img_m, mask_rgbs, partial);
  hipLaunchKernelGGL(photo_loss_finish_kernel, dim3(1), dim3(256), 0, st, partial, (int)nblk, (float)B * 3.f * HW, (float)B * HW, l_tex,
                     l_mrgb, l_sil, out);
  return hipGetLastError();
}

hipError_t launch_photo_loss_bwd(const float* rgba, const float* re_img_m, const float* mask_rgbs, const float* g_re_img,
                                 const float* gout, const float* fwd_out, int B, int HW, float l_tex, float l_mrgb, float* grad_rgba,
                                 hipStream_t st) {
  if (HW % 4 != 0) return hipErrorInvalidValue;
  hipLaunchKernelGGL(photo_loss_bwd_kernel, dim3(photo_grid(B, HW) * 4), dim3(256), 0, st, rgba, re_img_m, mask_rgbs, g_re_img, gout,
                     fwd_out, B, HW, (float)B * 3.f * HW, l_tex, l_mrgb, grad_rgba);
  return hipGetLastError();
}

__global__ __launch_bounds__(64) void loss_total_fwd_kernel(LossTotalParts p, float* __restrict__ total) {
  if (threadIdx.x != 0) return;
  float s = 0.f;
  for (int i = 0; i < kLossTotalParts; ++i)
    for (int j = 0; j < p.n[i]; ++j) s += p.v[i][j];
  total[0] = s;
}
__global__ __launch_bounds__(64) void loss_total_bwd_kernel(const float* __restrict__ gtotal, LossTotalGrads q) {
  const float g = gtotal[0];
  for (int i = 0; i < kLossTotalParts; ++i)
    for (int j = threadIdx.x; j < q.len[i]; j += 64) q.g[i][j] = j < q.n[i] ? g : 0.f;
}

hipError_t launch_loss_total_fwd(const LossTotalParts& p, float* total, hipStream_t st) {
  hipLaunchKernelGGL(loss_total_fwd_kernel, dim3(1), dim3(64), 0, st, p, total);
  return hipGetLastError();
}
hipError_t launch_loss_total_bwd(const float* gtotal, const LossTotalGrads& q, hipStream_t st) {
  hipLaunchKernelGGL(loss_total_bwd_kernel, dim3(1), dim3(64), 0, st, gtotal, q);
  return hipGetLastError();
}

hipError_t launch_sil_post(const float* rgba, const float* imgs, int B, int HW, float* re_sil, float* mask_rgbs, hipStream_t st) {
  if (HW % 4 != 0) return hipErrorInvalidValue;
// ... 119 lines not shown
```

### hifihr_amd/csrc/ssim.hip

```cpp
#include <hip/hip_runtime.h>

#include "hifihr_internal.h"

namespace hifihr {

constexpr int kST = 32;
constexpr int kSO = kST * kST / 256;
constexpr int kSR = 5;
constexpr int kSH = kST + 2 * kSR;

constexpr int kSF = 48;

template <bool VEC>
__device__ __forceinline__ void ssim_stage(float (*__restrict__ dst)[kSF], const float* __restrict__ p, int H, int W, int ox, int oy, int tid) {
  if (VEC) {
    for (int e = tid; e < kSH * (kSF / 4); e += 256) {
      const int r = e / (kSF / 4), sg = e - r * (kSF / 4);
      const int y = oy + r - kSR, x0 = ox - 8 + 4 * sg;
      const bool in = (y >= 0) && (y < H) && (x0 >= 0) && (x0 + 3 < W);
      float4 v = make_float4(0.f, 0.f, 0.f, 0.f);
      if (in) v = *reinterpret_cast<const float4*>(p + (size_t)y * W + x0);
      *reinterpret_cast<float4*>(&dst[r][4 * sg]) = v;
    }
  } else {
    for (int e = tid; e < kSH * kSH; e += 256) {
      const int r = e / kSH, c = e - r * kSH;
      const int y = oy + r - kSR, x = ox + c - kSR;
      const bool in = (y >= 0) && (y < H) && (x >= 0) && (x < W);
      dst[r][c + 3] = in ? p[(size_t)y * W + x] : 0.f;
    }
  }
}
__device__ __forceinline__ void ssim_row14(const float (*__restrict__ src)[kSF], int r, int c0, float* __restrict__ a) {
  float f[20];
#pragma unroll
  for (int q = 0; q < 5; ++q) {
    const float4 v = *reinterpret_cast<const float4*>(&src[r][c0 + 4 * q]);
    f[4 * q] = v.x; f[4 * q + 1] = v.y; f[4 * q + 2] = v.z; f[4 * q + 3] = v.w;
  }
#pragma unroll
  for (int k = 0; k < 14; ++k) a[k] = f[3 + k];
}

#if defined(HIFIHR_HOSTSIM)
__device__ __forceinline__ float ssim_rcp(float x) { return 1.0f / x; }
#else
__device__ __forceinline__ float ssim_rcp(float x) { return __builtin_amdgcn_rcpf(x); }
#endif

__device__ __forceinline__ float block_sum_256(float v, float* red) {
#pragma unroll
  for (int o = 32; o > 0; o >>= 1) v += __shfl_down(v, o, 64);
  const int lane = threadIdx.x & 63, wave = threadIdx.x >> 6;
  if (lane == 0) red[wave] = v;
  __syncthreads();
  return red[0] + red[1] + red[2] + red[3];
}

template <bool VEC>
__global__ __launch_bounds__(256) void ssim_fwd_kernel(SsimWindow win, const float* __restrict__ img1, const float* __restrict__ img2,
                                                      int H, int W, float* __restrict__ partial, float* __restrict__ dA,
                                                      float* __restrict__ dB, float* __restrict__ dC) {
  __shared__ __attribute__((aligned(16))) float xs[kSH][kSF], ys[kSH][kSF];
  __shared__ float hq[5][kSH][kST + 1];
  __shared__ float red[4];
  const int plane = blockIdx.z;
  const int ox = blockIdx.x * kST, oy = blockIdx.y * kST;
  const int tid = threadIdx.x;
  const float* p1 = img1 + (size_t)plane * H * W;
  const float* p2 = img2 + (size_t)plane * H * W;
  ssim_stage<VEC>(xs, p1, H, W, ox, oy, tid);
  ssim_stage<VEC>(ys, p2, H, W, ox, oy, tid);
  __syncthreads();
  for (int e = tid; e < kSH * (kST / 4); e += 256) {
    const int r = e / (kST / 4), c0 = 4 * (e - r * (kST / 4));
    float a[14], b[14], aa[14], bb[14], ab[14];
    ssim_row14(xs, r, c0, a);
    ssim_row14(ys, r, c0, b);
#pragma unroll
    for (int k = 0; k < 14; ++k) { aa[k] = a[k] * a[k]; bb[k] = b[k] * b[k]; ab[k] = a[k] * b[k]; }
#pragma unroll
    for (int o = 0; o < 4; ++o) {
      float m1 = 0.f, m2 = 0.f, e11 = 0.f, e22 = 0.f, e12 = 0.f;
#pragma unroll
      for (int k = 0; k < 11; ++k) {
        const float w = win.g[k];
        m1 = fmaf(w, a[o + k], m1); m2 = fmaf(w, b[o + k], m2); e11 = fmaf(w, aa[o + k], e11); e22 = fmaf(w, bb[o + k], e22);
        e12 = fmaf(w, ab[o + k], e12);
      }
      hq[0][r][c0 + o] = m1; hq[1][r][c0 + o] = m2; hq[2][r][c0 + o] = e11; hq[3][r][c0 + o] = e22; hq[4][r][c0 + o] = e12;
    }
  }
  __syncthreads();
  float val = 0.f;
  {
    const int tx = tid % kST, ty0 = (tid / kST) * kSO;
    const int x = ox + tx;
    float h[5][kSO + 10];
#pragma unroll
    for (int q = 0; q < 5; ++q)
#pragma unroll
      for (int k = 0; k < kSO + 10; ++k) h[q][k] = hq[q][ty0 + k][tx];
#pragma unroll
    for (int o4 = 0; o4 < kSO; ++o4) {
      const int y = oy + ty0 + o4;
      if (x < W && y < H) {
        float mu1 = 0.f, mu2 = 0.f, e11 = 0.f, e22 = 0.f, e12 = 0.f;
#pragma unroll
        for (int k = 0; k < 11; ++k) {
          const float w = win.g[k];
          mu1 = fmaf(w, h[0][o4 + k], mu1); mu2 = fmaf(w, h[1][o4 + k], mu2); e11 = fmaf(w, h[2][o4 + k], e11);
          e22 = fmaf(w, h[3][o4 + k], e22); e12 = fmaf(w, h[4][o4 + k], e12);
        }
        const float C1 = 0.01f * 0.01f, C2 = 0.03f * 0.03f;
        const float mu1_sq = mu1 * mu1, mu2_sq = mu2 * mu2, mu12 = mu1 * mu2;
        const float s1 = e11 - mu1_sq, s2 = e22 - mu2_sq, s12 = e12 - mu12;
        const float a1 = 2.f * mu12 + C1, a2 = 2.f * s12 + C2, b1 = mu1_sq + mu2_sq + C1, b2 = s1 + s2 + C2;
        const float ib1 = ssim_rcp(b1), ib2 = ssim_rcp(b2), inv = ib1 * ib2;
        const float sv = (a1 * a2) * inv;
        val += sv;
        if (dA) {
          const size_t o = (size_t)plane * H * W + (size_t)y * W + x;
          dA[o] = 2.f * mu2 * (a2 - a1) * inv - 2.f * mu1 * sv * ib1 + 2.f * mu1 * sv * ib2;
          dB[o] = -sv * ib2;
          dC[o] = 2.f * a1 * inv;
        }
      }
    }
  }
  const float tot = block_sum_256(val, red);
  if (tid == 0) partial[((size_t)plane * gridDim.y + blockIdx.y) * gridDim.x + blockIdx.x] = tot;
}

template <bool VEC>
__global__ __launch_bounds__(256) void ssim_bwd_kernel(SsimWindow win, const float* __restrict__ img1, const float* __restrict__ img2,
                                                      const float* __restrict__ dA, const float* __restrict__ dB,
                                                      const float* __restrict__ dC, const float* __restrict__ gscale, float inv_n,
                                                      int H, int W, float* __restrict__ gimg1) {
  __shared__ __attribute__((aligned(16))) float ta[kSH][kSF], tb[kSH][kSF], tc[kSH][kSF];
  __shared__ float hq[3][kSH][kST + 1];
  const int plane = blockIdx.z;
  const int ox = blockIdx.x * kST, oy = blockIdx.y * kST;
  const int tid = threadIdx.x;
  const size_t po = (size_t)plane * H * W;
  ssim_stage<VEC>(ta, dA + po, H, W, ox, oy, tid);
  ssim_stage<VEC>(tb, dB + po, H, W, ox, oy, tid);
  ssim_stage<VEC>(tc, dC + po, H, W, ox, oy, tid);
  __syncthreads();
  for (int e = tid; e < kSH * (kST / 4); e += 256) {
    const int r = e / (kST / 4), c0 = 4 * (e - r * (kST / 4));
    float va[14], vb[14], vc[14];
    ssim_row14(ta, r, c0, va);
    ssim_row14(tb, r, c0, vb);
    ssim_row14(tc, r, c0, vc);
#pragma unroll
    for (int o = 0; o < 4; ++o) {
      float a = 0.f, b = 0.f, cc = 0.f;
#pragma unroll
      for (int k = 0; k < 11; ++k) {
        const float w = win.g[k];
        a = fmaf(w, va[o + k], a); b = fmaf(w, vb[o + k], b); cc = fmaf(w, vc[o + k], cc);
      }
      hq[0][r][c0 + o] = a; hq[1][r][c0 + o] = b; hq[2][r][c0 + o] = cc;
    }
  }
  __syncthreads();
  const float sc = gscale[0] * inv_n;
  const int tx = tid % kST, ty0 = (tid / kST) * kSO;
  const int x = ox + tx;
  float h[3][kSO + 10];
#pragma unroll
  for (int q = 0; q < 3; ++q)
#pragma unroll
    for (int k = 0; k < kSO + 10; ++k) h[q][k] = hq[q][ty0 + k][tx];
#pragma unroll
  for (int o4 = 0; o4 < kSO; ++o4) {
    const int y = oy + ty0 + o4;
    if (x < W && y < H) {
      float a = 0.f, b = 0.f, cc = 0.f;
#pragma unroll
      for (int k = 0; k < 11; ++k) {
        const float w = win.g[k];
        a = fmaf(w, h[0][o4 + k], a); b = fmaf(w, h[1][o4 + k], b); cc = fmaf(w, h[2][o4 + k], cc);
      }
      const size_t o = po + (size_t)y * W + x;
      gimg1[o] = sc * (a + 2.f * img1[o] * b + img2[o] * cc);
    }
  }
}

__global__ __launch_bounds__(256) void ssim_finish_kernel(const float* __restrict__ partial, int count, float scale, float offset,
                                                         float* __restrict__ out) {
  __shared__ float red[4];
  float s0 = 0.f, s1 = 0.f, s2 = 0.f, s3 = 0.f;
  int i = threadIdx.x;
  for (; i + 768 < count; i += 1024) { s0 += partial[i]; s1 += partial[i + 256]; s2 += partial[i + 512]; s3 += partial[i + 768]; }
  for (; i < count; i += 256) s0 += partial[i];
  const float s = block_sum_256((s0 + s1) + (s2 + s3), red);
  if (threadIdx.x == 0) out[0] = offset + scale * s;
}

int ssim_tile_edge() { return kST; }

static bool ssim_vec_ok(int W, const float* a, const float* b, const float* c) {
  return W % 4 == 0 && ((reinterpret_cast<uintptr_t>(a) | reinterpret_cast<uintptr_t>(b) | reinterpret_cast<uintptr_t>(c)) & 15) == 0;
}

hipError_t launch_ssim_finish(const float* partial, int count, float scale, float offset, float* out, hipStream_t st) {
  hipLaunchKernelGGL(ssim_finish_kernel, dim3(1), dim3(256), 0, st, partial, count, scale, offset, out);
  return hipGetLastError();
}

hipError_t launch_ssim_fwd(const SsimWindow& win, const float* img1, const float* img2, int planes, int H, int W, float* partial,
                           float* dA, float* dB, float* dC, hipStream_t st) {
  const dim3 grid((W + kST - 1) / kST, (H + kST - 1) / kST, planes);
  if (ssim_vec_ok(W, img1, img2, nullptr))
    hipLaunchKernelGGL(ssim_fwd_kernel<true>, grid, dim3(256), 0, st, win, img1, img2, H, W, partial, dA, dB, dC);
  else
    hipLaunchKernelGGL(ssim_fwd_kernel<false>, grid, dim3(256), 0, st, win, img1, img2, H, W, partial, dA, dB, dC);
  return hipGetLastError();
}

hipError_t launch_ssim_bwd(const SsimWindow& win, const float* img1, const float* img2, const float* dA, const float* dB,
                           const float* dC, const float* gscale, int planes, int H, int W, float* gimg1, hipStream_t st, float out_scale) {
  const dim3 grid((W + kST - 1) / kST, (H + kST - 1) / kST, planes);
  const float inv_n = out_scale / ((float)planes * (float)H * (float)W);
  if (ssim_vec_ok(W, dA, dB, dC))
    hipLaunchKernelGGL(ssim_bwd_kernel<true>, grid, dim3(256), 0, st, win, img1, img2, dA, dB, dC, gscale, inv_n, H, W, gimg1);
  else
    hipLaunchKernelGGL(ssim_bwd_kernel<false>, grid, dim3(256), 0, st, win, img1, img2, dA, dB, dC, gscale, inv_n, H, W, gimg1);
  return hipGetLastError();
}

}
```

### hifihr_amd/losses.py

```python
from __future__ import annotations

import os

import torch
import torch.nn.functional as F

_BONES = [(0, 1), (1, 2), (2, 3), (3, 4), (0, 5), (5, 6), (6, 7), (7, 8), (0, 9), (9, 10), (10, 11), (11, 12),
          (0, 13), (13, 14), (14, 15), (15, 16), (0, 17), (17, 18), (18, 19), (19, 20)]


TERMS = ("joint_3d", "vert_3d", "edge_length", "mshape", "mpose", "joint_2d", "bone_direc", "bone_direc_3d", "mscale", "scale", "texture",
         "mrgb", "ssim_tex", "sil", "texture_self", "mrgb_self", "ssim_tex_self", "perceptual", "iou", "sil_soft", "iou_soft", "triangle",
         "normal_consistency", "lpips", "chamfer", "point_mesh", "depth", "mtex")

_BONE_IDX = {}


def bone_direction_loss(j, j_gt, conf=None):
    if j.device not in _BONE_IDX:
        _BONE_IDX[j.device] = (torch.tensor([b[0] for b in _BONES], device=j.device), torch.tensor([b[1] for b in _BONES], device=j.device))
    p, c = _BONE_IDX[j.device]
    v = j[:, c] - j[:, p]
    vg = j_gt[:, c] - j_gt[:, p]
    vn = v / (torch.sqrt((v ** 2).sum(-1, keepdim=True)) + 1e-4)
    vgn = vg / (torch.sqrt((vg ** 2).sum(-1, keepdim=True)) + 1e-4)
    return ((vn - vgn) ** 2).sum(-1).mean()


def edge_length_loss(pred, gt, face):
    f = face[0].long()
    def lens(x):
        a, b, c = x[:, f[:, 0]], x[:, f[:, 1]], x[:, f[:, 2]]
        return torch.cat([torch.sqrt(((a - b) ** 2).sum(2, keepdim=True)), torch.sqrt(((a - c) ** 2).sum(2, keepdim=True)),
                          torch.sqrt(((b - c) ** 2).sum(2, keepdim=True))], 1)
    return torch.abs(lens(pred) - lens(gt)).mean()


def iou(s_gt, s_est):
    b = s_gt.shape[0]
    mul = (s_gt * s_est).reshape(b, -1).sum(1)
    add = (s_gt + s_est).reshape(b, -1).sum(1)
    return 1 - torch.mean(mul / (add - mul))


_GEOM_BRANCH = os.environ.get("HIFIHR_GEOM_BRANCH", "0") != "0"


class LossFunction:
    def __init__(self, perceptual=None, lpips=None):
        self.perceptual_loss = perceptual
        self.lpips_loss = lpips

    def _lpips_module(self, args, device):
        if self.lpips_loss is None:
            from .lpips import LPIPS, load_lpips_weights
            m = LPIPS(net="alex", differentiable=True)
            paths = getattr(args, "lpips_weights", None)
            if paths:
                load_lpips_weights(m, *([paths] if isinstance(paths, str) else paths))
            else:
                import warnings
                warnings.warn("loss term 'lpips': no lpips_weights given -- the AlexNet trunk and the lin layers carry SEEDED random weights, "
                              "not the calibrated metric's (hifihr_amd/lpips.py)", stacklevel=3)
            self.lpips_loss = m.to(device)
        return self.lpips_loss

    def _fused_geometry(self, examples, outputs, loss_used, args, loss_dic):
        from . import ops
        lam = [args.lambda_j3d if "joint_3d" in loss_used else 0.0, args.lambda_vert_3d if "vert_3d" in loss_used else 0.0,
               args.lambda_edge_len if "edge_length" in loss_used else 0.0, args.lambda_shape if "mshape" in loss_used else 0.0,
               args.lambda_pose if "mpose" in loss_used else 0.0]
        faces = None
        if "edge_length" in loss_used:
            faces = outputs.get("_faces_i32")
            if faces is None:
                faces = outputs["mano_faces"][0].int().contiguous()
        joints_gt = examples["joints"] if "joints" in examples else outputs["joints"].detach()
        verts_gt = examples["verts"] if "verts" in examples else outputs["mano_verts"].detach()
        with ops.side_branch(outputs["joints"], "geom", enabled=_GEOM_BRANCH and "re_img" in outputs,
                             inputs=(joints_gt, outputs["mano_verts"], verts_gt, outputs["shape_params"], outputs["pose_params"])) as br:
            vec = ops.geom_losses(outputs["joints"], joints_gt, outputs["mano_verts"], verts_gt,
                                  outputs["shape_params"], outputs["pose_params"], faces, args.base_loss_fn != "L1", lam)
        self._pending_join = (br, vec)
        for k, v in zip(ops.GEOM_TERMS, vec.unbind(0)):
            if k in loss_used:
                loss_dic[k] = v
        self._total_parts.append((vec, 5, [k for k in ops.GEOM_TERMS if k in loss_used]))

    def __call__(self, examples, outputs, loss_used, dat_name, args) -> dict:
        self._pending_join = None
        self._total_parts = []
        try:
            return self._terms(examples, outputs, loss_used, dat_name, args)
        finally:
            if self._pending_join is not None:
                br, vec = self._pending_join
                br.join(vec)
                self._pending_join = None

    def total(self, loss_dic, losses):
        from . import ops
        parts = getattr(self, "_total_parts", [])
        covered = [k for _, _, names in parts for k in names]
        if (parts and len(parts) <= 4 and sorted(covered) == sorted(losses) and all(p.is_cuda for p, _, _ in parts)
                and all(loss_dic.get(k) is not None for k in losses)):
            return ops.loss_total([(p, n) for p, n, _ in parts])
        terms = [loss_dic[k] for k in losses]
        return terms[0] if len(terms) == 1 else torch.stack(terms).sum()

    def _terms(self, examples, outputs, loss_used, dat_name, args) -> dict:
        from . import ops
        loss_dic = {}
        base = F.l1_loss if args.base_loss_fn == "L1" else F.mse_loss
        if any(k in loss_used for k in ("joint_3d", "vert_3d", "edge_length", "mshape", "mpose")):
            self._fused_geometry(examples, outputs, loss_used, args, loss_dic)
            loss_used = [k for k in loss_used if k not in loss_dic]
        want = [k in loss_used for k in ("joint_2d", "bone_direc", "bone_direc_3d")]
        if any(want):
            two, three = want[0] or want[1], want[2]
            lam3 = (args.lambda_j2d_gt if want[0] else 0.0, args.lambda_bone_direc if want[1] else 0.0, args.lambda_bone_direc_3d if want[2] else 0.0)
            vals = ops.joint_terms(outputs["j2d"] if two else None, examples["j2d_gt"] if two else None,
                                   outputs["joints"] if three else None, examples["joints"] if three else None,
                                   args.base_loss_fn != "L1", lam3).unbind(0)
            for k, w, v in zip(("joint_2d", "bone_direc", "bone_direc_3d"), want, vals):
                if w:
                    loss_dic[k] = v
        if "mscale" in loss_used:
            bl = torch.sqrt(torch.sum((outputs["joints"][:, 9] - outputs["joints"][:, 10]) ** 2, 1))
            loss_dic["mscale"] = args.lambda_mscale * F.l1_loss(bl, torch.ones_like(bl) * 0.0282)
        if "scale" in loss_used and dat_name in ("FreiHand", "RHD"):
            bl = torch.sqrt(torch.sum((outputs["joints"][:, 9] - outputs["joints"][:, 10]) ** 2, 1))
            loss_dic["scale"] = args.lambda_scale * F.mse_loss(bl, examples["scales"].to(bl.device))
        if "re_img" in outputs and "re_sil" in outputs and "texture_con" in examples:
            mask_rgbs, re_img, con = outputs["maskRGBs"], outputs["re_img"], examples["texture_con"]
            b = re_img.shape[0]
            c2 = con.view(-1) ** 2
            per = torch.abs(re_img - mask_rgbs).reshape(b, -1).sum(1)
            loss_dic["texture_self"] = args.lambda_texture * (torch.sum(per * c2) / (torch.sum(c2) * (re_img.numel() // b)))
            dm = torch.abs(torch.mean(re_img.reshape(b, -1), 1) - torch.mean(mask_rgbs.reshape(b, -1), 1))
            loss_dic["mrgb_self"] = args.lambda_mrgb * (torch.sum(dm * c2) / torch.sum(c2))
            loss_dic["ssim_tex_self"] = ops.ssim_loss(re_img, mask_rgbs, args.lambda_ssim_tex)
        if "re_img" in outputs and "re_sil" in outputs:
            rgba = outputs.get("_rgba")
            if rgba is None:
                rgba = torch.cat([outputs["re_img"], (outputs["re_sil"] > 0).to(outputs["re_img"].dtype)], 1)
            out, re_img, mask_rgbs = ops.photo_losses(rgba, examples["imgs"], examples["segms_gt"], args.lambda_texture,
                                                      args.lambda_mrgb, args.lambda_silhouette)
            tex, mrgb, sil, _ = out.unbind(0)
            loss_dic["texture"], loss_dic["mrgb"] = tex, mrgb
            loss_dic["ssim_tex"] = ops.ssim_loss(re_img, mask_rgbs, args.lambda_ssim_tex)
            if "sil" in loss_used:
                loss_dic["sil"] = sil
                self._total_parts.append((out, 3, ["texture", "mrgb", "sil"]))
            else:
                self._total_parts.append((out, 2, ["texture", "mrgb"]))
            self._total_parts.append((loss_dic["ssim_tex"], 1, ["ssim_tex"]))
        if "perceptual" in loss_used:
            if self.perceptual_loss is None:
                from .perceptual import PerceptualLoss
                self.perceptual_loss = PerceptualLoss().to(outputs["re_img"].device)
            seg = examples["segms_gt"].unsqueeze(1)
            loss_dic["perceptual"] = args.lambda_percep * self.perceptual_loss(
                outputs["re_img"] * seg + examples["imgs"] * (1 - seg), examples["imgs"])
        if "lpips" in loss_used:
            seg = examples["segms_gt"].unsqueeze(1)
            fn = self._lpips_module(args, outputs["re_img"].device)
            loss_dic["lpips"] = args.lambda_lpips * fn(outputs["re_img"] * seg + examples["imgs"] * (1 - seg), examples["imgs"],
                                                       normalize=True).mean()
        if "iou" in loss_used:
            loss_dic["iou"] = args.lambda_iou * iou(outputs["re_sil"], examples["segms_gt"].unsqueeze(1).float())
        if "sil_soft" in loss_used or "iou_soft" in loss_used:
            assert "re_sil_soft" in outputs, ("the loss terms 'sil_soft' / 'iou_soft' need outputs['re_sil_soft']: build the model with "
                                              "Model(..., soft_silhouette=True) (options: soft_silhouette)")
            names = [k for k in ("sil_soft", "iou_soft") if k in loss_used]
            vec = ops.soft_sil_losses(outputs["re_sil_soft"], examples["segms_gt"],
                                      args.lambda_silhouette_soft if "sil_soft" in loss_used else 0.0,
                                      args.lambda_iou_soft if "iou_soft" in loss_used else 0.0)
            for k, v in zip(("sil_soft", "iou_soft"), vec.unbind(0)):
                if k in loss_used:
                    loss_dic[k] = v
            self._total_parts.append((vec, 2, names))
        if "triangle" in loss_used or "normal_consistency" in loss_used:
            if outputs.get("verts") is not None and outputs.get("faces") is not None:
                verts, faces = outputs["verts"], outputs["faces"]
                topo = ops.mesh_topology_of(faces[0] if faces.dim() == 3 else faces, verts.shape[1])
            else:
                verts, topo = outputs["mano_verts"], outputs.get("_mesh_topo")
                if topo is None:
                    faces = outputs.get("_faces_i32")
                    if faces is None:
                        faces = outputs["mano_faces"][0].int().contiguous()
                    topo = ops.mesh_topology_of(faces, verts.shape[1])
            names = [k for k in ops.MESH_REG_TERMS if k in loss_used]
            vec = ops.mesh_regularizers(topo, verts, args.lambda_laplacian if "triangle" in loss_used else 0.0,
                                        args.lambda_normal_consistency if "normal_consistency" in loss_used else 0.0)
            for k, v in zip(ops.MESH_REG_TERMS, vec.unbind(0)):
                if k in loss_used:
                    loss_dic[k] = v
            self._total_parts.append((vec, 2, names))
        if "chamfer" in loss_used:
            target = examples["chamfer_points"] if examples.get("chamfer_points") is not None else examples["verts"]
            if outputs.get("chamfer_points") is not None:
                pred = outputs["chamfer_points"]
            elif getattr(args, "hand_model", "mano") == "nimble" and outputs.get("verts") is not None and outputs.get("_pred_root") is not None:
                pred = outputs["verts"] - outputs["_pred_root"]
            else:
                pred = outputs["mano_verts"]
            loss_dic["chamfer"] = ops.chamfer_distance(pred, target, args.lambda_chamfer, args.lambda_chamfer)
            self._total_parts.append((loss_dic["chamfer"], 1, ["chamfer"]))
        if "point_mesh" in loss_used:
            target = examples["chamfer_points"] if examples.get("chamfer_points") is not None else examples["verts"]
            if outputs.get("verts") is not None and outputs.get("faces") is not None:
                verts, faces = outputs["verts"], outputs["faces"]
                faces = faces[0] if faces.dim() == 3 else faces
            elif (getattr(args, "hand_model", "mano") == "nimble" and outputs.get("verts") is not None and outputs.get("_pred_root") is not None
                  and outputs.get("_skin_faces_i32") is not None):
                verts, faces = outputs["verts"] - outputs["_pred_root"], outputs["_skin_faces_i32"]
            else:
                verts, faces = outputs["mano_verts"], outputs.get("_faces_i32")
                if faces is None:
                    faces = outputs["mano_faces"][0].int().contiguous()
            loss_dic["point_mesh"] = ops.point_mesh_distance(target, verts, faces, args.lambda_point_mesh, args.lambda_point_mesh_faces)
            self._total_parts.append((loss_dic["point_mesh"], 1, ["point_mesh"]))
        if "depth" in loss_used:
            assert "re_depth" in outputs and "_re_depth_hits" in outputs, (
                "the loss term 'depth' needs outputs['re_depth']: build the model with Model(..., render_depth=True) (options: render_depth)")
            loss_dic["depth"] = ops.depth_loss(outputs["re_depth"], outputs["_re_depth_hits"], examples["depths"], examples.get("segms_gt"),
                                               args.lambda_depth, getattr(args, "depth_trunc", 0.0))
            self._total_parts.append((loss_dic["depth"], 1, ["depth"]))
        if "mtex" in loss_used and outputs.get("texture_params") is not None:
            loss_dic["mtex"] = args.lambda_tex_reg * F.mse_loss(outputs["texture_params"], torch.zeros_like(outputs["texture_params"]))
        return loss_dic
```

### hifihr_amd/ops.py

```python
from __future__ import annotations

import math
import os
import threading

import numpy as np
import torch

from ._lib import get_lib, require_cuda


import os as _os

_DEBUG_SYNC = _os.environ.get("HIFIHR_DEBUG_SYNC", "0") == "1"


class _Profile:

    def __init__(self):
        self.on = False
        self.events = []
        self.last_render = None
        self.conv_log = []

# ... 1691 lines not shown
        N, C, H, W = x.shape
        if get_lib().bn_relu_maxpool_supported(N, H, W, C):
            return _BNReluMaxPool.apply(x, stats, bn.weight, bn.bias, float(bn.eps), float(bn.momentum), bn.running_mean, bn.running_var)
    return maxpool3x3s2(bn_act(x, stats, bn, None, True))


GEOM_TERMS = ("joint_3d", "vert_3d", "edge_length", "mshape", "mpose")
_VF_CACHE = {}


def _vertex_face_csr(faces, V):
    key = (faces.data_ptr(), int(faces.shape[0]), V, str(faces.device))
    hit = _VF_CACHE.get(key)
    if hit is None:
        import numpy as np
        f = faces.detach().cpu().numpy().astype(np.int64)
        flat = f.reshape(-1)
        order = np.argsort(flat, kind="stable")
        off = np.zeros(V + 1, dtype=np.int32)
        np.add.at(off, flat + 1, 1)
        off = np.cumsum(off).astype(np.int32)
        idx = ((order // 3) * 4 + (order % 3)).astype(np.int32)
        hit = (torch.from_numpy(off).to(faces.device), torch.from_numpy(idx).to(faces.device))
        _VF_CACHE[key] = hit
    return hit


class _GeomLoss(torch.autograd.Function):
    @staticmethod
    def forward(ctx, joints, joints_gt, verts, verts_gt, shape, pose, faces, mse, lam):
        require_cuda(joints, verts)
        lib = get_lib()
        joints, joints_gt, verts, verts_gt = (t.contiguous().float() for t in (joints, joints_gt, verts, verts_gt))
        shape = shape.contiguous() if shape is not None else None
        pose = pose.contiguous() if pose is not None else None
        B = joints.shape[0]
        partial = torch.empty(B * 5, device=joints.device)
        out = torch.empty(5, device=joints.device)
        PROFILE.bracket("geom_loss_fwd", lambda: lib.geom_loss_fwd(joints, joints_gt, verts, verts_gt, shape, pose, faces, mse, lam,
                                                                  partial, out))
        ctx.save_for_backward(joints, joints_gt, verts, verts_gt, shape, pose, faces)
        ctx.mse, ctx.lam = mse, tuple(lam)
        return out

    @staticmethod
    def backward(ctx, gout):
        joints, joints_gt, verts, verts_gt, shape, pose, faces = ctx.saved_tensors
        lib = get_lib()
        need = ctx.needs_input_grad
        gj = torch.empty_like(joints) if need[0] else None
        gv = torch.empty_like(verts) if need[2] else None
        gs = torch.empty_like(shape) if (shape is not None and need[4]) else None
        gp = torch.empty_like(pose) if (pose is not None and need[5]) else None
        vf_off, vf_idx = _vertex_face_csr(faces, verts.shape[1]) if faces is not None else (None, None)
        gout = gout.contiguous()
        PROFILE.bracket("geom_loss_bwd", lambda: lib.geom_loss_bwd(joints, joints_gt, verts, verts_gt, shape, pose, faces, vf_off, vf_idx,
                                                                  ctx.mse, ctx.lam, gout, gj, gv, gs, gp))
        return gj, None, gv, None, gs, gp, None, None, None


def geom_losses(joints, joints_gt, verts, verts_gt, shape, pose, faces, mse, lam):
    return _GeomLoss.apply(joints, joints_gt, verts, verts_gt, shape, pose, faces, bool(mse), tuple(float(v) for v in lam))


class _LossTotal(torch.autograd.Function):

    @staticmethod
    def forward(ctx, counts, *parts):
        require_cuda(*parts)
        ctx.orig = [p.shape for p in parts]
        parts = [p.contiguous().reshape(-1) for p in parts]
        total = torch.empty((), device=parts[0].device)
        PROFILE.bracket("loss_total", lambda: get_lib().loss_total_fwd(parts, counts, total))
        ctx.counts, ctx.shapes = counts, [p.shape for p in parts]
        return total

    @staticmethod
    def backward(ctx, g):
        g = g.contiguous()
        grads = [torch.empty(s, device=g.device) for s in ctx.shapes]
        PROFILE.bracket("loss_total", lambda: get_lib().loss_total_bwd(g, grads, ctx.counts))
        return (None, *[gr.reshape(s) for gr, s in zip(grads, ctx.orig)])


def loss_total(parts):
    return _LossTotal.apply(tuple(int(n) for _, n in parts), *[p for p, _ in parts])


class _JointTerms(torch.autograd.Function):
    @staticmethod
    def forward(ctx, j2d, j2d_gt, joints, joints_gt, mse, lam3):
        lib = get_lib()
        prep = lambda t: t.contiguous().float() if t is not None else None
        j2d, j2d_gt, joints, joints_gt = prep(j2d), prep(j2d_gt), prep(joints), prep(joints_gt)
        require_cuda(*(t for t in (j2d, joints) if t is not None))
        ref = j2d if j2d is not None else joints
        out = torch.empty(3, device=ref.device)
        PROFILE.bracket("joint_terms_fwd", lambda: lib.joint_terms_fwd(j2d, j2d_gt, joints, joints_gt, mse, lam3, out))
        ctx.save_for_backward(*(t if t is not None else ref.new_empty(0) for t in (j2d, j2d_gt, joints, joints_gt)))
        ctx.has2, ctx.has3, ctx.mse, ctx.lam3 = j2d is not None, joints is not None, mse, lam3
        return out

    @staticmethod
    def backward(ctx, gout):
        j2d, j2d_gt, joints, joints_gt = (t if t.numel() else None for t in ctx.saved_tensors)
        lib = get_lib()
        g2 = torch.empty_like(j2d) if (ctx.has2 and ctx.needs_input_grad[0]) else None
        g3 = torch.empty_like(joints) if (ctx.has3 and ctx.needs_input_grad[2]) else None
        if g2 is not None or g3 is not None:
            PROFILE.bracket("joint_terms_bwd", lambda: lib.joint_terms_bwd(j2d, j2d_gt, joints, joints_gt, ctx.mse, ctx.lam3, gout.contiguous(), g2, g3))
        return g2, None, g3, None, None, None


def joint_terms(j2d, j2d_gt, joints, joints_gt, mse, lam3):
    return _JointTerms.apply(j2d, j2d_gt, joints, joints_gt, bool(mse), tuple(float(v) for v in lam3))


class _PhotoLoss(torch.autograd.Function):
    @staticmethod
    def forward(ctx, rgba, imgs, seg, l_tex, l_mrgb, l_sil):
        require_cuda(rgba, imgs, seg)
        lib = get_lib()
        rgba, imgs, seg = rgba.contiguous(), imgs.contiguous(), seg.contiguous()
        B, _, H, W = rgba.shape
        re_img_m = torch.empty(B, 3, H, W, device=rgba.device)
        mask_rgbs = torch.empty_like(re_img_m)
        partial = torch.empty(lib.photo_loss_partial_floats(), device=rgba.device)
        out = torch.empty(4, device=rgba.device)
        PROFILE.bracket("photo_loss_fwd", lambda: lib.photo_loss_fwd(rgba, imgs, seg, l_tex, l_mrgb, l_sil, re_img_m, mask_rgbs, partial,
                                                                    out))
        ctx.save_for_backward(rgba, re_img_m, mask_rgbs, out)
        ctx.lams = (l_tex, l_mrgb)
        ctx.mark_non_differentiable(mask_rgbs)
        ctx.set_materialize_grads(False)
        return out, re_img_m, mask_rgbs

    @staticmethod
    def backward(ctx, gout, g_re_img, _gm):
        if gout is None and g_re_img is None:
            return (None,) * 6
        rgba, re_img_m, mask_rgbs, out = ctx.saved_tensors
        grad = torch.empty_like(rgba)
        gout = gout.contiguous() if gout is not None else None
        g_re_img = g_re_img.contiguous() if g_re_img is not None else None
        PROFILE.bracket("photo_loss_bwd", lambda: get_lib().photo_loss_bwd(rgba, re_img_m, mask_rgbs, g_re_img, gout, out, ctx.lams[0],
                                                                          ctx.lams[1], grad))
        return grad, None, None, None, None, None


def photo_losses(rgba, imgs, seg, l_tex, l_mrgb, l_sil):
    return _PhotoLoss.apply(rgba, imgs, seg, float(l_tex), float(l_mrgb), float(l_sil))


def sil_post(rgba, images):
    require_cuda(rgba, images)
    rgba = rgba.detach().contiguous()
    B, _, H, W = rgba.shape
    re_sil = torch.empty(B, 1, H, W, device=rgba.device)
    mask_rgbs = torch.empty(B, 3, H, W, device=rgba.device)
    get_lib().sil_post(rgba, images.contiguous(), re_sil, mask_rgbs)
    return re_sil, mask_rgbs


class _Linear(torch.autograd.Function):
    @staticmethod
    def forward(ctx, x, w, b, gamma, beta, act, eps, momentum, running_mean, running_var):
        require_cuda(x, w)
        lib = get_lib()
        x, w = x.contiguous(), w.contiguous()
        B, O = x.shape[0], w.shape[0]
        y = torch.empty(B, O, device=x.device)
        bn = None
        z = sm = si = None
        if gamma is not None:
            z, sm, si = torch.empty(B, O, device=x.device), torch.empty(O, device=x.device), torch.empty(O, device=x.device)
            bn = (gamma, beta, eps, momentum, running_mean, running_var, z, sm, si)
        PROFILE.bracket("linear_fwd", lambda: lib.linear_fwd(x, w, b, act, y, bn))
        ctx.save_for_backward(x, w, y if act == 1 else None, gamma, z, sm, si)
        ctx.act = act
        ctx.params = (w, b, gamma, beta)
        return y

    @staticmethod
    def backward(ctx, dy):
        x, w, y, gamma, z, sm, si = ctx.saved_tensors
        pw, pb, pg, pbeta = ctx.params
        lib = get_lib()
        dy = dy.contiguous()
        B, O = dy.shape
        need_dx = ctx.needs_input_grad[0]
        dz = torch.empty(B, O, device=dy.device)
        dx = torch.empty_like(x) if need_dx else None
        dw_t, dw_ret = _grad_target(pw, pw)
        db_t, db_ret = _grad_target(pb, pb) if pb is not None else (None, None)
        bn = None
        dg_ret = dbt_ret = None
        if gamma is not None:
            dg_t, dg_ret = _grad_target(pg, pg)
            dbt_t, dbt_ret = _grad_target(pbeta, pbeta)
            bn = (gamma, z, sm, si, dg_t, dbt_t)
        PROFILE.bracket("linear_bwd", lambda: lib.linear_bwd(dy, y, x, w, ctx.act, dz, dw_t, db_t, dx, bn))
        for p, ret in ((pw, dw_ret), (pb, db_ret), (pg, dg_ret), (pbeta, dbt_ret)):
            if p is not None and ret is None:
                _grad_ready(p)
        return dx, dw_ret, db_ret, dg_ret, dbt_ret, None, None, None, None, None


class _LinearGroup(torch.autograd.Function):

    @staticmethod
    def forward(ctx, n, acts, *tensors):
        xs, ws, bs = tensors[:n], tensors[n:2 * n], tensors[2 * n:3 * n]
        require_cuda(*xs, *ws)
        lib = get_lib()
        xs = [x.contiguous() for x in xs]
        ws_c = [w.contiguous() for w in ws]
        ys = [torch.empty(x.shape[0], w.shape[0], device=x.device) for x, w in zip(xs, ws_c)]
        members = [dict(x=x, w=w, b=b, y=y, act=a) for x, w, b, y, a in zip(xs, ws_c, bs, ys, acts)]
        PROFILE.bracket("linear_fwd", lambda: lib.linear_fwd_group(members))
        ctx.n, ctx.acts, ctx.params = n, acts, (ws, bs)
        ctx.save_for_backward(*xs, *ws_c, *ys)
        ctx.set_materialize_grads(False)
        return tuple(ys)

    @staticmethod
    def backward(ctx, *dys):
        n = ctx.n
        saved = ctx.saved_tensors
        xs, ws_c, ys = saved[:n], saved[n:2 * n], saved[2 * n:3 * n]
        pws, pbs = ctx.params
        lib = get_lib()
        dxs, dws, dbs = [None] * n, [None] * n, [None] * n
        members, ready = [], []
        shared = {}
        for i in range(n):
            if dys[i] is None:
                continue
            dy = dys[i].contiguous()
            dx = None
            if ctx.needs_input_grad[2 + i]:
                key = (xs[i].data_ptr(), tuple(xs[i].shape))
                dx = shared.get(key)
                first = dx is None
                if first:
                    dx = shared[key] = torch.empty_like(xs[i])
            dw_t, dws[i] = _grad_target(pws[i], pws[i])
            db_t = None
            if pbs[i] is not None:
                db_t, dbs[i] = _grad_target(pbs[i], pbs[i])
            dxs[i] = dx if (dx is not None and first) else None
            members.append(dict(x=xs[i], w=ws_c[i], y=ys[i], act=ctx.acts[i], dy=dy, dz=torch.empty_like(dy), dW=dw_t, db=db_t, dx=dx))
            ready += [p for p, ret in ((pws[i], dws[i]), (pbs[i], dbs[i])) if p is not None and ret is None]
        if members:
            PROFILE.bracket("linear_bwd", lambda: lib.linear_bwd_group(members))
        for p in ready:
            _grad_ready(p)
        return (None, None, *dxs, *dws, *dbs)


def linear_group(members):
    n = len(members)
    acts = tuple(1 if m[2] in (True, "relu", 1) else 0 for m in members)
    return list(_LinearGroup.apply(n, acts, *[m[0] for m in members], *[m[1].weight for m in members], *[m[1].bias for m in members]))


class _TexturePCA(torch.autograd.Function):
    @staticmethod
    def forward(ctx, coef, basis, mean):
        require_cuda(coef, basis)
        coef, basis = coef.contiguous(), basis.contiguous()
        out = torch.empty(coef.shape[0], basis.shape[1], device=coef.device)
        PROFILE.bracket("texture_pca_fwd", lambda: get_lib().texture_pca_fwd(coef, basis, mean, out))
        ctx.save_for_backward(basis)
        ctx.K = coef.shape[1]
        return out

    @staticmethod
    def backward(ctx, g):
        basis, = ctx.saved_tensors
        g = g.contiguous()
        dcoef = torch.zeros(g.shape[0], ctx.K, device=g.device)
        PROFILE.bracket("texture_pca_bwd", lambda: get_lib().texture_pca_bwd(g, basis, dcoef))
        return dcoef, None, None


def texture_pca_decode(coef, basis, mean=None):
    return _TexturePCA.apply(coef, basis, mean)


class _LightSplit(torch.autograd.Function):

    @staticmethod
    def forward(ctx, lights):
        require_cuda(lights)
        lights = lights.contiguous()
        B = lights.shape[0]
        colors, directions = torch.empty(B, 3, device=lights.device), torch.empty(B, 3, device=lights.device)
        get_lib().light_split_fwd(lights, colors, directions)
        ctx.save_for_backward(lights)
        ctx.set_materialize_grads(False)
        return colors, directions

    @staticmethod
    def backward(ctx, gc, gd):
        lights, = ctx.saved_tensors
        gl = torch.empty_like(lights)
# ... 467 lines not shown
```

### include/hifihr.h

```cpp
#ifndef HIFIHR_H
#define HIFIHR_H

#include <stddef.h>
#include <stdint.h>

#ifdef __cplusplus
extern "C" {
#endif

#define HIFIHR_OK 0
#define HIFIHR_EINVAL (-1)
#define HIFIHR_EHIP (-2)
#define HIFIHR_ENOMEM (-3)

#define HIFIHR_MANO_NV 778
#define HIFIHR_MANO_NF 1538
#define HIFIHR_MANO_NJ 16

int hifihr_version(void);
const char* hifihr_last_error(void);
int hifihr_device_count(void);

typedef struct hifihr_mano hifihr_mano_t;

// ... 198 lines not shown
                                   float* out_d, float* v_d, int N, int H, int W, int C, int m, float eps, float momentum,
                                   float* save_mean_d, float* save_invstd_d, float* running_mean_d, float* running_var_d, void* stream);
int hifihr_wino_output_transform_bnred(const float* m_d, const float* x_d, const float* out_d , const float* gadd_d ,
                                       const float* save_mean_d, const float* save_invstd_d, const float* gamma_d, const float* beta_d,
                                       float* red_d, float* g_d, int N, int H, int W, int C, int m, void* stream);
int hifihr_wino_bn_bwd_dual_transform(const float* g_d, const float* y_d, const float* save_mean_d, const float* save_invstd_d,
                                      const float* gamma_d, float* red_d, float* v_d, float* yt_d, int N, int H, int W, int K, int m,
                                      float* dgamma_acc_d, float* dbeta_acc_d, void* stream);
int hifihr_bn_bwd_apply(const float* g_d, const float* x_d, const float* save_mean_d, const float* save_invstd_d, const float* gamma_d, long M,
                        int C, float* red_d, float* dx_d, float* dgamma_acc_d, float* dbeta_acc_d, void* stream);
int hifihr_wino4_bwd_gemm_pair_supported(int N, int H, int W, int C, int K);
int hifihr_wino4_bwd_gemm_pair(const float* V2_d, const float* U2_d, float* M2_d, const float* Vx_d, const float* Yt_d, float* dU_parts_d,
                               int N, int H, int W, int C, int K, int parts, void* stream);
typedef struct hifihr_wino_dw_job {
  const float* du_parts_d;
  float* dw_acc_d;
  int parts, K, C;
} hifihr_wino_dw_job;
int hifihr_wino4_dw_transform_multi(const hifihr_wino_dw_job* jobs, int njobs, void* stream);
size_t hifihr_bgemm_nt_workspace_bytes(int M, int N, int K, int batch);
int hifihr_bgemm_nt(const float* a_d, const float* b_d, float* c_d, int M, int N, int K, int batch,
                    void* ws_d , size_t ws_bytes, void* stream);
int hifihr_bgemm_tn_parts(int M, int N, int T, int batch);
int hifihr_bgemm_tn_coherent(int M, int N, int T, int batch);
int hifihr_bgemm_describe(int tn, int M, int N, int K_or_T, int batch, char* out, int cap);
int hifihr_bgemm_tn(const float* a_d, const float* b_d, float* c_parts_d, int M, int N, int T, int batch, int parts, void* stream);
int hifihr_weight_transpose(const float* w_d, float* wt_d, int K, int RS, int C, void* stream);
int hifihr_conv2d_bwd_data_pre(const float* dy_d, const float* wt_d, float* dx_d, int N, int H, int W, int C, int K, int R, int S,
                               int stride, int pad, void* ws_d, size_t ws_bytes, void* stream);
int hifihr_conv2d_bwd_data_pre_res(const float* dy_d, const float* wt_d, const float* res_d, float* dx_d, int N, int H, int W, int C, int K,
                                   int R, int S, int stride, int pad, void* ws_d, size_t ws_bytes, void* stream);
int hifihr_conv2d_bwd_data_pre_plus1x1_supported(int N, int H, int W, int C, int K, int R, int S, int stride, int pad);
int hifihr_conv2d_bwd_data_pre_plus1x1(const float* dy_d, const float* wt_d, const float* dy2_d, const float* wt2_d, float* dx_d, int N, int H,
                                       int W, int C, int K, int R, int S, int stride, int pad, void* stream);
int hifihr_conv2d_bwd_weight_plus1x1_supported(int N, int H, int W, int C, int K, int R, int S, int stride, int pad);
int hifihr_conv2d_bwd_weight_plus1x1(const float* x_d, const float* dy_d, float* dw_d, const float* dy2_d, float* dw2_d, int N, int H, int W,
                                     int C, int K, int R, int S, int stride, int pad, void* stream);
typedef struct hifihr_prep_job {
  const float* src;
  float* dst;
  int K, C, RS, kind;
} hifihr_prep_job;
int hifihr_weight_prep(const hifihr_prep_job* jobs_d, int njobs, int blocks_per_job, void* stream);

int hifihr_conv2d_describe(int N, int H, int W, int C, int K, int R, int S, int stride, int pad, int direction, char* out, int cap);

int hifihr_conv2d_fwd_bnstats(const float* x_d, const float* w_d, float* y_d, float* stats_d, int N, int H, int W, int C, int K,
                              int R, int S, int stride, int pad, void* ws_d, size_t ws_bytes, void* stream);
int hifihr_conv2d_fwd_bnstats_pair_supported(int N, int H, int W, int C, int stride, int K1, int R1, int pad1, int K2, int R2, int pad2);
int hifihr_conv2d_fwd_bnstats_pair(const float* x_d, const float* w1_d, float* y1_d, float* stats1_d, int K1, int R1, int pad1, const float* w2_d,
                                   float* y2_d, float* stats2_d, int K2, int R2, int pad2, int N, int H, int W, int C, int stride, void* stream);

int hifihr_bn_stats_floats(int C);
int hifihr_bn_stats(const float* x_d, long M, int C, float* stats_d, void* stream);
int hifihr_bn_act_fwd(const float* x_d, float* stats_d , const float* gamma_d, const float* beta_d,
                      const float* residual_d , int act, long M, int C, float eps, float momentum, float* y_d,
                      float* save_mean_d, float* save_invstd_d, float* running_mean_d, float* running_var_d, void* stream);
int hifihr_bn_act_eval(const float* x_d, const float* running_mean_d, const float* running_var_d, const float* gamma_d, const float* beta_d,
                       const float* residual_d , int act, long M, int C, float eps, float* y_d, void* stream);
int hifihr_bn_act_bwd(const float* dy_d, const float* y_d , const float* x_d, const float* save_mean_d,
                      const float* save_invstd_d, const float* gamma_d, const float* beta_d , int act, long M, int C,
                      float* red_scratch_d, float* dx_d, float* dres_d, float* dgamma_acc_d, float* dbeta_acc_d, void* stream);

int hifihr_bn_relu_maxpool_supported(int N, int H, int W, int C);
int hifihr_bn_relu_maxpool_fwd(const float* x_d, float* stats_d, const float* gamma_d, const float* beta_d, int N, int H, int W, int C,
                               float eps, float momentum, float* pooled_d, unsigned char* tap_d, float* save_mean_d, float* save_invstd_d,
                               float* running_mean_d, float* running_var_d, void* stream);
int hifihr_bn_relu_maxpool_bwd(const float* pooled_grad_d, const unsigned char* tap_d, const float* x_d, const float* save_mean_d,
                               const float* save_invstd_d, const float* gamma_d, const float* beta_d, int N, int H, int W, int C,
                               float* red_scratch_d, float* dx_d, float* dgamma_acc_d, float* dbeta_acc_d, void* stream);
int hifihr_bn_relu_maxpool_bwd_y(const float* pooled_grad_d, const float* pooled_d, const unsigned char* tap_d, const float* x_d,
                                 const float* save_mean_d, const float* save_invstd_d, const float* gamma_d, const float* beta_d, int N, int H, int W,
                                 int C, float* red_scratch_d, float* dx_d, float* dgamma_acc_d, float* dbeta_acc_d, void* stream);

int hifihr_dwconv2d_fwd(const float* x_d, const float* w_d, float* y_d, float* stats_d , int N, int H, int W, int C,
                        int OH, int OW, int K, int stride, int pad_top, int pad_left, void* stream);
int hifihr_dwconv2d_bwd_data(const float* dy_d, const float* w_d, float* dx_d, int N, int H, int W, int C, int OH, int OW, int K,
                             int stride, int pad_top, int pad_left, void* stream);
int hifihr_dwconv2d_bwd_weight(const float* x_d, const float* dy_d, float* dw_d, int N, int H, int W, int C, int OH, int OW,
                               int K, int stride, int pad_top, int pad_left, void* stream);
int hifihr_dwconv2d_fwd_bnswish(const float* x_d, const float* mean_d, const float* invstd_d, const float* gamma_d, const float* beta_d,
                                const float* w_d, float* y_d, float* stats_d , int N, int H, int W, int C, int OH, int OW,
                                int K, int stride, int pad_top, int pad_left, void* stream);
int hifihr_dwconv2d_bwd_weight_bnswish(const float* x_d, const float* mean_d, const float* invstd_d, const float* gamma_d,
                                       const float* beta_d, const float* dy_d, float* dw_d, int N, int H, int W, int C, int OH, int OW,
                                       int K, int stride, int pad_top, int pad_left, void* stream);
int hifihr_bn_finalize_fwd(float* stats_d, long M, int C, float eps, float momentum, float* save_mean_d, float* save_invstd_d,
                           float* running_mean_d , float* running_var_d , void* stream);

int hifihr_mmpool_fwd(const float* x_d, const float* p_d, int B, int HW, int C, float* y_d, int* argmax_d, float* xmax_d,
                      float* xavg_d, void* stream);
int hifihr_mmpool_bwd(const float* gy_d, const float* p_d, const int* argmax_d, const float* xmax_d, const float* xavg_d, int B,
                      int HW, int C, float* dx_d, float* dp_acc_d, void* stream);
int hifihr_maxpool2d_fwd(const float* x_d, int N, int H, int W, int C, int k, int s, int p, float* y_d, unsigned char* tap_d,
                         void* stream);
int hifihr_maxpool2d_bwd(const float* gy_d, const unsigned char* tap_d, int N, int H, int W, int C, int k, int s, int p,
                         float* dx_d, void* stream);
int hifihr_maxpool2d_bwd_relu(const float* gy_d, const unsigned char* tap_d, const float* y_d, int N, int H, int W, int C, int k, int s, int p,
                              float* dx_d, void* stream);
int hifihr_maxpool2d_fwd_flat(const float* x_d, int N, int H, int W, int C, int k, int s, int p, float* y_flat_d, unsigned char* tap_d,
                              void* stream);
int hifihr_maxpool2d_bwd_flat(const float* gy_flat_d, const unsigned char* tap_d, int N, int H, int W, int C, int k, int s, int p, float* dx_d,
                              void* stream);

int hifihr_image_to_nhwc4(const float* images_d, float* out_d, int B, int H, int W, void* stream);
int hifihr_image_to_nhwc4_padded(const float* images_d, float* out_d, int B, int H, int W, int pad_top, int pad_left,
                                 int pad_bottom, int pad_right, int normalize, void* stream);

int hifihr_image_scale_to_nhwc4(const float* images_d, float* out_d, int B, int H, int W, const float* shift3_host,
                                const float* scale3_host, void* stream);
int hifihr_maxpool2d_fwd_notap(const float* x_d, int N, int H, int W, int C, int k, int s, int p, float* y_d, void* stream);
int hifihr_lpips_tap_max_channels(void);
size_t hifihr_lpips_tap_partial_floats(int B);
int hifihr_lpips_tap(const float* f0_d, const float* f1_d, const float* w_d, int B, int HW, int C, int accumulate, float* partial_d,
                     float* val_d, void* stream);

int hifihr_lpips_tap_bwd(const float* f0_d, const float* f1_d, const float* w_d, const float* gval_d, int B, int HW, int C, int accumulate,
                         float* gf0_d, void* stream);
int hifihr_lpips_tap_bwd_relu(const float* f0_d, const float* f1_d, const float* w_d, const float* gval_d, int B, int HW, int C, int accumulate,
                              float* gf0_d, void* stream);
int hifihr_lpips_maxpool_fwd(const float* x_d, int N, int H, int W, int C, float* y_d, void* stream);
int hifihr_lpips_maxpool_bwd(const float* gy_d, const float* x_d, int N, int H, int W, int C, float* dx_d, void* stream);
int hifihr_image_scale_to_nhwc4_bwd(const float* g4_d, float* gimg_d, int B, int H, int W, const float* scale3_host, void* stream);

int hifihr_ssim_partial_count(int planes, int H, int W);
int hifihr_ssim_fwd(const float* window11_h, const float* img1_d, const float* img2_d, int planes, int H, int W,
                    float* partial_d, float* dA_d, float* dB_d, float* dC_d, void* stream);
int hifihr_ssim_bwd(const float* window11_h, const float* img1_d, const float* img2_d, const float* dA_d, const float* dB_d,
                    const float* dC_d, const float* grad_out_d, int planes, int H, int W, float* gimg1_d, void* stream);
int hifihr_ssim_finish(const float* partial_d, int count, float scale, float offset, float* out_d, void* stream);
int hifihr_ssim_bwd_scaled(const float* window11_h, const float* img1_d, const float* img2_d, const float* dA_d, const float* dB_d,
                           const float* dC_d, const float* grad_out_d, float out_scale, int planes, int H, int W, float* gimg1_d, void* stream);

int hifihr_geom_loss_fwd(const float* joints_d, const float* joints_gt_d, const float* verts_d, const float* verts_gt_d,
                         const float* shape_d, const float* pose_d, const int32_t* faces_d, int B, int J, int V, int F, int NS,
                         int NP, int mse, const float* lambda5_h, float* partial_d, float* out_d, void* stream);
int hifihr_joint_terms_fwd(const float* j2d_d, const float* j2d_gt_d, const float* joints_d, const float* joints_gt_d, int B, int J, int mse,
                           const float* lam3_host, float* out3_d, void* stream);
int hifihr_joint_terms_bwd(const float* j2d_d, const float* j2d_gt_d, const float* joints_d, const float* joints_gt_d, int B, int J, int mse,
                           const float* lam3_host, const float* gout3_d, float* g_j2d_d, float* g_joints_d, void* stream);
int hifihr_geom_loss_bwd(const float* joints_d, const float* joints_gt_d, const float* verts_d, const float* verts_gt_d,
                         const float* shape_d, const float* pose_d, const int32_t* faces_d, const int32_t* vf_off_d,
                         const int32_t* vf_idx_d, int B, int J, int V, int F, int NS, int NP, int mse, const float* lambda5_h,
                         const float* gout_d, float* gj_d, float* gv_d, float* gshape_d, float* gpose_d, void* stream);
int hifihr_photo_loss_partial_floats(void);
int hifihr_photo_loss_fwd(const float* rgba_d, const float* imgs_d, const int64_t* seg_d, int B, int H, int W, float l_tex,
                          float l_mrgb, float l_sil, float* re_img_m_d, float* mask_rgbs_d, float* partial_d, float* out_d,
                          void* stream);
int hifihr_photo_loss_bwd(const float* rgba_d, const float* re_img_m_d, const float* mask_rgbs_d, const float* g_re_img_d,
                          const float* gout_d, const float* fwd_out_d, int B, int H, int W, float l_tex, float l_mrgb,
                          float* grad_rgba_d, void* stream);
int hifihr_sil_post(const float* rgba_d, const float* imgs_d, int B, int H, int W, float* re_sil_d, float* mask_rgbs_d,
                    void* stream);
int hifihr_loss_total_fwd(const float* const* parts, const int* counts, int nparts, float* total_d, void* stream);
int hifihr_loss_total_bwd(const float* gtotal_d, float* const* grads, const int* counts, const int* lengths, int nparts,
                          void* stream);

int hifihr_linear_fwd(const float* x_d, const float* w_d, const float* b_d , int B, int I, int O, int act,
                      const float* gamma_d , const float* beta_d, float eps, float momentum,
                      float* running_mean_d, float* running_var_d, float* y_d, float* z_d, float* save_mean_d,
                      float* save_invstd_d, void* stream);
int hifihr_linear_bwd(const float* dy_d, const float* y_d, const float* x_d, const float* w_d, int B, int I, int O, int act,
                      const float* gamma_d, const float* z_d, const float* save_mean_d, const float* save_invstd_d,
                      float* dz_scratch_d, float* dW_acc_d, float* db_acc_d, float* dgamma_acc_d, float* dbeta_acc_d,
                      float* dx_d, void* stream);

typedef struct hifihr_linear_desc {
  const float *x, *w, *b;
  float* y;
  int B, I, O, act;
  const float* dy;
  float *dz_scratch, *dW_acc, *db_acc, *dx;
} hifihr_linear_desc;
int hifihr_linear_fwd_group(const hifihr_linear_desc* descs, int n, void* stream);
int hifihr_linear_bwd_group(const hifihr_linear_desc* descs, int n, void* stream);

int hifihr_se_pool(const float* x_d, int B, int HW, int C, float* mean_zeroed_d, void* stream);
int hifihr_se_scale(const float* x_d, const float* gate_d, const float* add_d , float add_scale, int B, int HW, int C,
                    float* y_d, void* stream);
int hifihr_se_bwd_gate(const float* dy_d, const float* x_d, int B, int HW, int C, float* dgate_zeroed_d, void* stream);
int hifihr_se_mlp_supported(int C, int SQ);
int hifihr_drop_connect_add(const float* x_d, const float* skip_d , const float* u_d, float keep, int B, size_t per_sample,
                            float* out_d, void* stream);
int hifihr_se_mlp_fwd(float* mean_acc_d, const float* w1_d, const float* b1_d, const float* w2t_d, const float* b2_d, int B, int C, int SQ,
                      float* mean_d, float* z1_d, float* h1_d, float* gate_d, void* stream);
int hifihr_se_mlp_bwd(float* dgate_acc_d, const float* gate_d, const float* z1_d, const float* h1_d, const float* mean_d, const float* w1_d,
                      const float* w2t_d, int B, int C, int SQ, float* dz2_d, float* dz1_d, float* dmean_d, float* dw1_acc_d, float* db1_acc_d,
                      float* dw2_acc_d, float* db2_acc_d, void* stream);

int hifihr_procrustes_error(const float* pred_d, const float* gt_d, int B, int N, float* aligned_d ,
                            float* err_sum_d, void* stream);

int hifihr_point_error_hist(const float* pred_d, const float* gt_d, const uint8_t* vis_d , int n, int K, const double* thr_h,
                            int T, int32_t* hist_d, double* sum_d, void* stream);
int hifihr_fscore_counts(const float* pred_d, const float* gt_d, int B, int Np, int Ng, const double* thr_h, int T, int32_t* counts_d,
                         void* stream);

int hifihr_freihand_augment(const uint32_t* img_rgbx_d, const uint8_t* mask_d, const int* idx_d, const int* coef_fix_d, int B, int H,
                            int W, float* out_img_d, float* out_mask_d, void* stream);

int hifihr_freihand_batch(const uint32_t* img_rgbx_d, const uint8_t* mask_d, const float* Ks_d, const float* joints_d, const float* verts_d,
                          const float* scales_d, int J, int V, const int* packed_d, int B, int H, int W, float* out_img_d,
                          float* out_mask_d, long long* out_segm_d, float* out_Ks_d, float* out_Ps_d, float* out_joints_d,
                          float* out_verts_d, float* out_j2d_d, float* out_scales_d, long long* out_idxs_d, void* stream);
int hifihr_freihand_batch_step(const uint32_t* img_rgbx_d, const uint8_t* mask_d, const float* Ks_d, const float* joints_d,
                               const float* verts_d, const float* scales_d, int J, int V, const int* packed_d, int B, int H, int W,
                               float* out_img_d, float* out_mask_d, long long* out_segm_d, float* out_Ks_d, float* out_Ps_d,
                               float* out_joints_d, float* out_verts_d, float* out_j2d_d, float* out_scales_d, long long* out_idxs_d,
                               int root_id, float image_size, float* out_root_d, float* out_joints_rel_d, float* out_verts_rel_d,
                               float* out_cam_ndc_d, void* stream);

#define HIFIHR_HO3D_MAX_WINDOW 800
size_t hifihr_ho3d_workspace_bytes(int B, int out_size);
int hifihr_ho3d_batch(const uint32_t* img_rgbx_d, const uint8_t* hand_mask_d, const float* Ks_d, const float* uv21_d, const float* xyz21_d,
                      int FH, int FW, const int* packed_d, int B, int out_size, void* ws_d, size_t ws_bytes, float* out_img_d,
                      float* out_mask_d, float* out_K_d, float* out_uv21_d, float* out_xyz21_d, void* stream);

#ifdef __cplusplus
}
#endif
#endif
```

Baseline: 6704 images/sec.

## Fuse photometric losses with SSIM into single image-loss forward and backward kernels

Adds combined image_loss forward and backward kernels. The SSIM tile staging computes the masked rendered image and masked ground truth straight from rgba, imgs and seg, and accumulates the texture, mrgb and silhouette L1 partial sums while loading. This removes the separate photo-loss pass, the materialised re_img and mask_rgbs buffers, and the separate SSIM launches. It also folds the two variance accumulations into a single sum-of-squares term, so the horizontal SSIM pass keeps four shared-memory planes instead of five. The cost is more complex kernels with more registers per thread, and slightly different floating-point rounding.

```diff
diff --git a/hifihr_amd/_lib.py b/hifihr_amd/_lib.py
--- a/hifihr_amd/_lib.py
+++ b/hifihr_amd/_lib.py
@@ -337,6 +337,20 @@
         assert seg.dtype == torch.int64 and seg.is_contiguous() and rgba.is_contiguous() and imgs.is_contiguous()
         self._run("hifihr_photo_loss_fwd", rgba, imgs, seg, B, H, W, l_tex, l_mrgb, l_sil, re_img_m, mask_rgbs, partial, out)
 
+    def image_loss_partial_floats(self, B, H, W):
+        return 5 * self.ssim_partial_count(3 * B, H, W)
+
+    def image_loss_fwd(self, window, rgba, imgs, seg, l_tex, l_mrgb, l_sil, l_ssim, dA, dB, dC, partial, out_photo, out_ssim):
+        B, _, H, W = rgba.shape
+        assert seg.dtype == torch.int64 and seg.numel() == B * H * W
+        self._run("hifihr_image_loss_fwd", window, rgba, imgs, seg, B, H, W, l_tex, l_mrgb, l_sil, l_ssim, dA, dB, dC, partial, out_photo,
+                  out_ssim)
+
+    def image_loss_bwd(self, window, rgba, imgs, seg, dA, dB, dC, g_photo, g_ssim, fwd_out_photo, l_tex, l_mrgb, l_ssim, grad_rgba):
+        B, _, H, W = rgba.shape
+        self._run("hifihr_image_loss_bwd", window, rgba, imgs, seg, dA, dB, dC, g_photo, g_ssim, fwd_out_photo, B, H, W, l_tex, l_mrgb,
+                  l_ssim, grad_rgba)
+
     def photo_loss_bwd(self, rgba, re_img_m, mask_rgbs, g_re_img, gout, fwd_out, l_tex, l_mrgb, grad_rgba):
         B, _, H, W = rgba.shape
         self._run("hifihr_photo_loss_bwd", rgba, re_img_m, mask_rgbs, g_re_img, gout, fwd_out, B, H, W, l_tex, l_mrgb, grad_rgba)
diff --git a/hifihr_amd/csrc/hifihr_api.hip b/hifihr_amd/csrc/hifihr_api.hip
--- a/hifihr_amd/csrc/hifihr_api.hip
+++ b/hifihr_amd/csrc/hifihr_api.hip
@@ -1314,6 +1314,32 @@
   return HIFIHR_OK;
 }
 
+int hifihr_image_loss_fwd(const float* window11, const float* rgba, const float* imgs, const int64_t* seg, int B, int H, int W, float l_tex,
+                          float l_mrgb, float l_sil, float l_ssim, float* dA, float* dB, float* dC, float* partial, float* out_photo,
+                          float* out_ssim, void* stream) {
+  if (!window11 || !rgba || !imgs || !seg || !partial || !out_photo || !out_ssim || B <= 0 || H <= 0 || W <= 0 || (H * W) % 4 != 0 ||
+      ((dA != nullptr) != (dB != nullptr)) || ((dA != nullptr) != (dC != nullptr)))
+    return fail(HIFIHR_EINVAL, "hifihr_image_loss_fwd: bad argument (H*W % 4 == 0; all three maps or none)");
+  hifihr::SsimWindow win;
+  for (int k = 0; k < 11; ++k) win.g[k] = window11[k];
+  HIP_TRY(hifihr::launch_image_loss_fwd(win, rgba, imgs, (const long long*)seg, B, H, W, l_tex, l_mrgb, l_sil, l_ssim, dA, dB, dC, partial,
+                                        out_photo, out_ssim, (hipStream_t)stream));
+  return HIFIHR_OK;
+}
+
+int hifihr_image_loss_bwd(const float* window11, const float* rgba, const float* imgs, const int64_t* seg, const float* dA, const float* dB,
+                          const float* dC, const float* g_photo, const float* g_ssim, const float* fwd_out_photo, int B, int H, int W,
+                          float l_tex, float l_mrgb, float l_ssim, float* grad_rgba, void* stream) {
+  if (!window11 || !rgba || !imgs || !seg || !dA || !dB || !dC || !fwd_out_photo || !grad_rgba || B <= 0 || H <= 0 || W <= 0 ||
+      (H * W) % 4 != 0)
+    return fail(HIFIHR_EINVAL, "hifihr_image_loss_bwd: bad argument (H*W % 4 == 0)");
+  hifihr::SsimWindow win;
+  for (int k = 0; k < 11; ++k) win.g[k] = window11[k];
+  HIP_TRY(hifihr::launch_image_loss_bwd(win, rgba, imgs, (const long long*)seg, dA, dB, dC, g_photo, g_ssim, fwd_out_photo, B, H, W, l_tex,
+                                        l_mrgb, l_ssim, grad_rgba, (hipStream_t)stream));
+  return HIFIHR_OK;
+}
+
 int hifihr_sil_post(const float* rgba, const float* imgs, int B, int H, int W, float* re_sil, float* mask_rgbs, void* stream) {
   if (!rgba || !re_sil || (mask_rgbs && !imgs) || B <= 0 || H <= 0 || W <= 0 || (H * W) % 4 != 0)
     return fail(HIFIHR_EINVAL, "hifihr_sil_post: bad argument (H*W % 4 == 0)");
diff --git a/hifihr_amd/csrc/hifihr_internal.h b/hifihr_amd/csrc/hifihr_internal.h
--- a/hifihr_amd/csrc/hifihr_internal.h
+++ b/hifihr_amd/csrc/hifihr_internal.h
@@ -247,6 +247,14 @@
 hipError_t launch_ssim_bwd(const SsimWindow& win, const float* img1, const float* img2, const float* dA, const float* dB,
                            const float* dC, const float* gscale, int planes, int H, int W, float* gimg1, hipStream_t st, float out_scale = 1.0f);
 hipError_t launch_ssim_finish(const float* partial, int count, float scale, float offset, float* out, hipStream_t st);
+hipError_t launch_image_loss_fwd(const SsimWindow& win, const float* rgba, const float* imgs, const long long* seg, int B, int H, int W,
+                                 float l_tex, float l_mrgb, float l_sil, float l_ssim, float* dA, float* dB, float* dC, float* partial,
+                                 float* out_photo, float* out_ssim, hipStream_t st);
+hipError_t launch_image_loss_bwd(const SsimWindow& win, const float* rgba, const float* imgs, const long long* seg, const float* dA,
+                                 const float* dB, const float* dC, const float* g_photo, const float* g_ssim, const float* fwd_out_photo,
+                                 int B, int H, int W, float l_tex, float l_mrgb, float l_ssim, float* grad_rgba, hipStream_t st);
+__device__ __forceinline__ float sil_scale(float alpha) { return alpha > 0.f ? 1.0f : alpha / 255.0f; }
+__device__ __forceinline__ float l1_sign(float d) { return d > 0.f ? 1.f : (d < 0.f ? -1.f : 0.f); }
 
 struct DwGeom {
   int N, H, W, C, OH, OW, K, stride, pt, pl;
diff --git a/hifihr_amd/csrc/losses.hip b/hifihr_amd/csrc/losses.hip
--- a/hifihr_amd/csrc/losses.hip
+++ b/hifihr_amd/csrc/losses.hip
@@ -24,7 +24,7 @@
 }
 
 __device__ __forceinline__ float base_term(int mse, float d) { return mse ? d * d : fabsf(d); }
-__device__ __forceinline__ float base_grad(int mse, float d) { return mse ? 2.f * d : (d > 0.f ? 1.f : (d < 0.f ? -1.f : 0.f)); }
+__device__ __forceinline__ float base_grad(int mse, float d) { return mse ? 2.f * d : l1_sign(d); }
 
 __device__ __forceinline__ float edge_len(const float* __restrict__ v, int a, int b) {
   const float dx = v[3 * a] - v[3 * b], dy = v[3 * a + 1] - v[3 * b + 1], dz = v[3 * a + 2] - v[3 * b + 2];
@@ -118,8 +118,6 @@
 }
 
 constexpr int kPhotoBlocks = 512;
-
-__device__ __forceinline__ float sil_scale(float alpha) { return alpha > 0.f ? 1.0f : alpha / 255.0f; }
 
 __global__ __launch_bounds__(256) void photo_loss_fwd_kernel(const float* __restrict__ rgba, const float* __restrict__ imgs,
                                                             const long long* __restrict__ seg, int B, int HW,
diff --git a/hifihr_amd/csrc/ssim.hip b/hifihr_amd/csrc/ssim.hip
--- a/hifihr_amd/csrc/ssim.hip
+++ b/hifihr_amd/csrc/ssim.hip
@@ -11,23 +11,106 @@
 
 constexpr int kSF = 48;
 
-template <bool VEC>
-__device__ __forceinline__ void ssim_stage(float (*__restrict__ dst)[kSF], const float* __restrict__ p, int H, int W, int ox, int oy, int tid) {
+struct SsimPlanes {
+  const float* p1;
+  const float* p2;
+  __device__ __forceinline__ void pair1(size_t o, bool, float& a, float& b) { a = p1[o]; b = p2[o]; }
+  __device__ __forceinline__ void pair4(size_t o, bool, float4& a, float4& b) {
+    a = *reinterpret_cast<const float4*>(p1 + o);
+    b = *reinterpret_cast<const float4*>(p2 + o);
+  }
+};
+
+struct alignas(16) SegPair { long long x, y; };
+
+struct ImageLossPlanes {
+  const float* rgb;
+  const float* alpha;
+  const float* img;
+  const long long* seg;
+  bool c0;
+  float s[4];
+  __device__ __forceinline__ void pair1(size_t o, bool own, float& a, float& b) {
+    const float al = alpha[o], sg = (float)seg[o];
+    a = rgb[o] * sil_scale(al);
+    b = sg * img[o];
+    if (own) {
+      s[0] += fabsf(a - b); s[1] += a; s[2] += b;
+      if (c0) s[3] += fabsf((al > 0.f ? 255.0f : al) - sg);
+    }
+  }
+  __device__ __forceinline__ void pair4(size_t o, bool own, float4& a, float4& b) {
+    const float4 al = *reinterpret_cast<const float4*>(alpha + o), r = *reinterpret_cast<const float4*>(rgb + o);
+    const float4 im = *reinterpret_cast<const float4*>(img + o);
+    const SegPair s01 = *reinterpret_cast<const SegPair*>(seg + o), s23 = *reinterpret_cast<const SegPair*>(seg + o + 2);
+    const float sg[4] = {(float)s01.x, (float)s01.y, (float)s23.x, (float)s23.y};
+    a = make_float4(r.x * sil_scale(al.x), r.y * sil_scale(al.y), r.z * sil_scale(al.z), r.w * sil_scale(al.w));
+    b = make_float4(sg[0] * im.x, sg[1] * im.y, sg[2] * im.z, sg[3] * im.w);
+    if (own) {
+      s[0] += fabsf(a.x - b.x) + fabsf(a.y - b.y) + fabsf(a.z - b.z) + fabsf(a.w - b.w);
+      s[1] += (a.x + a.y) + (a.z + a.w);
+      s[2] += (b.x + b.y) + (b.z + b.w);
+      if (c0) {
+        const float a4[4] = {al.x, al.y, al.z, al.w};
+#pragma unroll
+        for (int e = 0; e < 4; ++e) s[3] += fabsf((a4[e] > 0.f ? 255.0f : a4[e]) - sg[e]);
+      }
+    }
+  }
+};
+
+template <bool VEC, class Src>
+__device__ __forceinline__ void ssim_stage_pair(float (*__restrict__ xs)[kSF], float (*__restrict__ ys)[kSF], Src& src, int H, int W, int ox,
+                                                int oy, int tid) {
   if (VEC) {
     for (int e = tid; e < kSH * (kSF / 4); e += 256) {
       const int r = e / (kSF / 4), sg = e - r * (kSF / 4);
       const int y = oy + r - kSR, x0 = ox - 8 + 4 * sg;
       const bool in = (y >= 0) && (y < H) && (x0 >= 0) && (x0 + 3 < W);
-      float4 v = make_float4(0.f, 0.f, 0.f, 0.f);
-      if (in) v = *reinterpret_cast<const float4*>(p + (size_t)y * W + x0);
-      *reinterpret_cast<float4*>(&dst[r][4 * sg]) = v;
+      float4 a = make_float4(0.f, 0.f, 0.f, 0.f), b = a;
+      if (in) src.pair4((size_t)y * W + x0, y >= oy && y < oy + kST && x0 >= ox && x0 < ox + kST, a, b);
+      *reinterpret_cast<float4*>(&xs[r][4 * sg]) = a;
+      *reinterpret_cast<float4*>(&ys[r][4 * sg]) = b;
     }
   } else {
     for (int e = tid; e < kSH * kSH; e += 256) {
       const int r = e / kSH, c = e - r * kSH;
       const int y = oy + r - kSR, x = ox + c - kSR;
       const bool in = (y >= 0) && (y < H) && (x >= 0) && (x < W);
-      dst[r][c + 3] = in ? p[(size_t)y * W + x] : 0.f;
+      float a = 0.f, b = 0.f;
+      if (in) src.pair1((size_t)y * W + x, y >= oy && y < oy + kST && x >= ox && x < ox + kST, a, b);
+      xs[r][c + 3] = a;
+      ys[r][c + 3] = b;
+    }
+  }
+}
+template <bool VEC>
+__device__ __forceinline__ void ssim_stage3(float (*__restrict__ ta)[kSF], float (*__restrict__ tb)[kSF], float (*__restrict__ tc)[kSF],
+                                            const float* __restrict__ pa, const float* __restrict__ pb, const float* __restrict__ pc, int H, int W,
+                                            int ox, int oy, int tid) {
+  if (VEC) {
+    for (int e = tid; e < kSH * (kSF / 4); e += 256) {
+      const int r = e / (kSF / 4), sg = e - r * (kSF / 4);
+      const int y = oy + r - kSR, x0 = ox - 8 + 4 * sg;
+      const bool in = (y >= 0) && (y < H) && (x0 >= 0) && (x0 + 3 < W);
+      float4 va = make_float4(0.f, 0.f, 0.f, 0.f), vb = va, vc = va;
+      if (in) {
+        const size_t o = (size_t)y * W + x0;
+        va = *reinterpret_cast<const float4*>(pa + o); vb = *reinterpret_cast<const float4*>(pb + o); vc = *reinterpret_cast<const float4*>(pc + o);
+      }
+      *reinterpret_cast<float4*>(&ta[r][4 * sg]) = va;
+      *reinterpret_cast<float4*>(&tb[r][4 * sg]) = vb;
+      *reinterpret_cast<float4*>(&tc[r][4 * sg]) = vc;
+    }
+  } else {
+    for (int e = tid; e < kSH * kSH; e += 256) {
+      const int r = e / kSH, c = e - r * kSH;
+      const int y = oy + r - kSR, x = ox + c - kSR;
+      const bool in = (y >= 0) && (y < H) && (x >= 0) && (x < W);
+      const size_t o = in ? (size_t)y * W + x : 0;
+      ta[r][c + 3] = in ? pa[o] : 0.f;
+      tb[r][c + 3] = in ? pb[o] : 0.f;
+      tc[r][c + 3] = in ? pc[o] : 0.f;
     }
   }
 }
@@ -57,38 +140,35 @@
   return red[0] + red[1] + red[2] + red[3];
 }
 
-template <bool VEC>
-__global__ __launch_bounds__(256) void ssim_fwd_kernel(SsimWindow win, const float* __restrict__ img1, const float* __restrict__ img2,
-                                                      int H, int W, float* __restrict__ partial, float* __restrict__ dA,
-                                                      float* __restrict__ dB, float* __restrict__ dC) {
+__device__ __forceinline__ size_t ssim_tile_index() { return ((size_t)blockIdx.z * gridDim.y + blockIdx.y) * gridDim.x + blockIdx.x; }
+
+template <bool VEC, class Src>
+__device__ __forceinline__ void ssim_fwd_tile(const SsimWindow& win, Src& src, int H, int W, float* __restrict__ partial,
+                                              float* __restrict__ dA, float* __restrict__ dB, float* __restrict__ dC) {
   __shared__ __attribute__((aligned(16))) float xs[kSH][kSF], ys[kSH][kSF];
-  __shared__ float hq[5][kSH][kST + 1];
+  __shared__ float hq[4][kSH][kST + 1];
   __shared__ float red[4];
   const int plane = blockIdx.z;
   const int ox = blockIdx.x * kST, oy = blockIdx.y * kST;
   const int tid = threadIdx.x;
-  const float* p1 = img1 + (size_t)plane * H * W;
-  const float* p2 = img2 + (size_t)plane * H * W;
-  ssim_stage<VEC>(xs, p1, H, W, ox, oy, tid);
-  ssim_stage<VEC>(ys, p2, H, W, ox, oy, tid);
+  ssim_stage_pair<VEC>(xs, ys, src, H, W, ox, oy, tid);
   __syncthreads();
   for (int e = tid; e < kSH * (kST / 4); e += 256) {
     const int r = e / (kST / 4), c0 = 4 * (e - r * (kST / 4));
-    float a[14], b[14], aa[14], bb[14], ab[14];
+    float a[14], b[14], ss[14], ab[14];
     ssim_row14(xs, r, c0, a);
     ssim_row14(ys, r, c0, b);
 #pragma unroll
-    for (int k = 0; k < 14; ++k) { aa[k] = a[k] * a[k]; bb[k] = b[k] * b[k]; ab[k] = a[k] * b[k]; }
+    for (int k = 0; k < 14; ++k) { ss[k] = fmaf(b[k], b[k], a[k] * a[k]); ab[k] = a[k] * b[k]; }
 #pragma unroll
     for (int o = 0; o < 4; ++o) {
-      float m1 = 0.f, m2 = 0.f, e11 = 0.f, e22 = 0.f, e12 = 0.f;
+      float m1 = 0.f, m2 = 0.f, ess = 0.f, e12 = 0.f;
 #pragma unroll
       for (int k = 0; k < 11; ++k) {
         const float w = win.g[k];
-        m1 = fmaf(w, a[o + k], m1); m2 = fmaf(w, b[o + k], m2); e11 = fmaf(w, aa[o + k], e11); e22 = fmaf(w, bb[o + k], e22);
-        e12 = fmaf(w, ab[o + k], e12);
-      }
-      hq[0][r][c0 + o] = m1; hq[1][r][c0 + o] = m2; hq[2][r][c0 + o] = e11; hq[3][r][c0 + o] = e22; hq[4][r][c0 + o] = e12;
+        m1 = fmaf(w, a[o + k], m1); m2 = fmaf(w, b[o + k], m2); ess = fmaf(w, ss[o + k], ess); e12 = fmaf(w, ab[o + k], e12);
+      }
+      hq[0][r][c0 + o] = m1; hq[1][r][c0 + o] = m2; hq[2][r][c0 + o] = ess; hq[3][r][c0 + o] = e12;
     }
   }
   __syncthreads();
@@ -96,26 +176,26 @@
   {
     const int tx = tid % kST, ty0 = (tid / kST) * kSO;
     const int x = ox + tx;
-    float h[5][kSO + 10];
-#pragma unroll
-    for (int q = 0; q < 5; ++q)
+    float h[4][kSO + 10];
+#pragma unroll
+    for (int q = 0; q < 4; ++q)
 #pragma unroll
       for (int k = 0; k < kSO + 10; ++k) h[q][k] = hq[q][ty0 + k][tx];
 #pragma unroll
     for (int o4 = 0; o4 < kSO; ++o4) {
       const int y = oy + ty0 + o4;
       if (x < W && y < H) {
-        float mu1 = 0.f, mu2 = 0.f, e11 = 0.f, e22 = 0.f, e12 = 0.f;
+        float mu1 = 0.f, mu2 = 0.f, ess = 0.f, e12 = 0.f;
 #pragma unroll
         for (int k = 0; k < 11; ++k) {
           const float w = win.g[k];
-          mu1 = fmaf(w, h[0][o4 + k], mu1); mu2 = fmaf(w, h[1][o4 + k], mu2); e11 = fmaf(w, h[2][o4 + k], e11);
-          e22 = fmaf(w, h[3][o4 + k], e22); e12 = fmaf(w, h[4][o4 + k], e12);
+          mu1 = fmaf(w, h[0][o4 + k], mu1); mu2 = fmaf(w, h[1][o4 + k], mu2); ess = fmaf(w, h[2][o4 + k], ess);
+          e12 = fmaf(w, h[3][o4 + k], e12);
         }
         const float C1 = 0.01f * 0.01f, C2 = 0.03f * 0.03f;
         const float mu1_sq = mu1 * mu1, mu2_sq = mu2 * mu2, mu12 = mu1 * mu2;
-        const float s1 = e11 - mu1_sq, s2 = e22 - mu2_sq, s12 = e12 - mu12;
-        const float a1 = 2.f * mu12 + C1, a2 = 2.f * s12 + C2, b1 = mu1_sq + mu2_sq + C1, b2 = s1 + s2 + C2;
+        const float s12 = e12 - mu12;
+        const float a1 = 2.f * mu12 + C1, a2 = 2.f * s12 + C2, b1 = mu1_sq + mu2_sq + C1, b2 = ((ess - mu1_sq) - mu2_sq) + C2;
         const float ib1 = ssim_rcp(b1), ib2 = ssim_rcp(b2), inv = ib1 * ib2;
         const float sv = (a1 * a2) * inv;
         val += sv;
@@ -129,7 +209,125 @@
     }
   }
   const float tot = block_sum_256(val, red);
-  if (tid == 0) partial[((size_t)plane * gridDim.y + blockIdx.y) * gridDim.x + blockIdx.x] = tot;
+  if (tid == 0) partial[ssim_tile_index()] = tot;
+}
+
+template <bool VEC>
+__global__ __launch_bounds__(256) void ssim_fwd_kernel(SsimWindow win, const float* __restrict__ img1, const float* __restrict__ img2,
+                                                      int H, int W, float* __restrict__ partial, float* __restrict__ dA,
+                                                      float* __restrict__ dB, float* __restrict__ dC) {
+  const size_t po = (size_t)blockIdx.z * H * W;
+  SsimPlanes src{img1 + po, img2 + po};
+  ssim_fwd_tile<VEC>(win, src, H, W, partial, dA, dB, dC);
+}
+
+template <bool VEC>
+__global__ __launch_bounds__(256) void image_loss_fwd_kernel(SsimWindow win, const float* __restrict__ rgba, const float* __restrict__ imgs,
+                                                            const long long* __restrict__ seg, int H, int W, float* __restrict__ partial,
+                                                            float* __restrict__ photo, float* __restrict__ dA, float* __restrict__ dB,
+                                                            float* __restrict__ dC) {
+  __shared__ float red4[4][4];
+  const int plane = blockIdx.z, b = plane / 3, c = plane - 3 * b;
+  const size_t HW = (size_t)H * W;
+  ImageLossPlanes src{rgba + ((size_t)b * 4 + c) * HW, rgba + ((size_t)b * 4 + 3) * HW, imgs + (size_t)plane * HW, seg + (size_t)b * HW,
+                      c == 0, {0.f, 0.f, 0.f, 0.f}};
+  ssim_fwd_tile<VEC>(win, src, H, W, partial, dA, dB, dC);
+#pragma unroll
+  for (int q = 0; q < 4; ++q) {
+#pragma unroll
+    for (int o = 32; o > 0; o >>= 1) src.s[q] += __shfl_down(src.s[q], o, 64);
+  }
+  const int lane = threadIdx.x & 63, wave = threadIdx.x >> 6;
+  if (lane == 0) {
+#pragma unroll
+    for (int q = 0; q < 4; ++q) red4[q][wave] = src.s[q];
+  }
+  __syncthreads();
+  if (threadIdx.x < 4) {
+    const int q = threadIdx.x;
+    photo[(size_t)q * (gridDim.x * gridDim.y * gridDim.z) + ssim_tile_index()] = (red4[q][0] + red4[q][1]) + (red4[q][2] + red4[q][3]);
+  }
+}
+
+struct SsimGradPlanes {
+  const float* img1;
+  const float* img2;
+  float* gimg1;
+  float sc;
+  __device__ __forceinline__ void emit(size_t po, size_t o, float a, float b, float cc) {
+    gimg1[po + o] = sc * (a + 2.f * img1[po + o] * b + img2[po + o] * cc);
+  }
+};
+struct ImageLossGrad {
+  const float* rgb;
+  const float* alpha;
+  const float* img;
+  const long long* seg;
+  float* grad;
+  float* galpha;
+  float sc, kt, km;
+  __device__ __forceinline__ void emit(size_t, size_t o, float a, float b, float cc) {
+    const float scl = sil_scale(alpha[o]);
+    const float x = rgb[o] * scl, y = (float)seg[o] * img[o];
+    float g = sc * (a + 2.f * x * b + y * cc);
+    g += kt * l1_sign(x - y) + km;
+    grad[o] = g * scl;
+    if (galpha) galpha[o] = 0.f;
+  }
+};
+
+template <bool VEC, class Sink>
+__device__ __forceinline__ void ssim_bwd_tile(const SsimWindow& win, Sink& sink, const float* __restrict__ dA, const float* __restrict__ dB,
+                                              const float* __restrict__ dC, bool filt, int H, int W) {
+  __shared__ __attribute__((aligned(16))) float ta[kSH][kSF], tb[kSH][kSF], tc[kSH][kSF];
+  __shared__ float hq[3][kSH][kST + 1];
+  const int ox = blockIdx.x * kST, oy = blockIdx.y * kST;
+  const int tid = threadIdx.x;
+  const size_t po = (size_t)blockIdx.z * H * W;
+  const int tx = tid % kST, ty0 = (tid / kST) * kSO;
+  const int x = ox + tx;
+  float h[3][kSO + 10];
+  if (filt) {
+    ssim_stage3<VEC>(ta, tb, tc, dA + po, dB + po, dC + po, H, W, ox, oy, tid);
+    __syncthreads();
+    for (int e = tid; e < kSH * (kST / 4); e += 256) {
+      const int r = e / (kST / 4), c0 = 4 * (e - r * (kST / 4));
+      float va[14], vb[14], vc[14];
+      ssim_row14(ta, r, c0, va);
+      ssim_row14(tb, r, c0, vb);
+      ssim_row14(tc, r, c0, vc);
+#pragma unroll
+      for (int o = 0; o < 4; ++o) {
+        float a = 0.f, b = 0.f, cc = 0.f;
+#pragma unroll
+        for (int k = 0; k < 11; ++k) {
+          const float w = win.g[k];
+          a = fmaf(w, va[o + k], a); b = fmaf(w, vb[o + k], b); cc = fmaf(w, vc[o + k], cc);
+        }
+        hq[0][r][c0 + o] = a; hq[1][r][c0 + o] = b; hq[2][r][c0 + o] = cc;
+      }
+    }
+    __syncthreads();
+#pragma unroll
+    for (int q = 0; q < 3; ++q)
+#pragma unroll
+      for (int k = 0; k < kSO + 10; ++k) h[q][k] = hq[q][ty0 + k][tx];
+  }
+#pragma unroll
+  for (int o4 = 0; o4 < kSO; ++o4) {
+    const int y = oy + ty0 + o4;
+    if (x < W && y < H) {
+      float a = 0.f, b = 0.f, cc = 0.f;
+      if (filt) {
+#pragma unroll
+        for (int k = 0; k < 11; ++k) {
+          const float w = win.g[k];
+          a = fmaf(w, h[0][o4 + k], a); b = fmaf(w, h[1][o4 + k], b); cc = fmaf(w, h[2][o4 + k], cc);
+        }
+      }
+      sink.emit(po, (size_t)y * W + x, a, b, cc);
+    }
+  }
 }
 
 template <bool VEC>
@@ -137,72 +335,82 @@
                                                       const float* __restrict__ dA, const float* __restrict__ dB,
                                                       const float* __restrict__ dC, const float* __restrict__ gscale, float inv_n,
                                                       int H, int W, float* __restrict__ gimg1) {
-  __shared__ __attribute__((aligned(16))) float ta[kSH][kSF], tb[kSH][kSF], tc[kSH][kSF];
-  __shared__ float hq[3][kSH][kST + 1];
-  const int plane = blockIdx.z;
-  const int ox = blockIdx.x * kST, oy = blockIdx.y * kST;
-  const int tid = threadIdx.x;
-  const size_t po = (size_t)plane * H * W;
-  ssim_stage<VEC>(ta, dA + po, H, W, ox, oy, tid);
-  ssim_stage<VEC>(tb, dB + po, H, W, ox, oy, tid);
-  ssim_stage<VEC>(tc, dC + po, H, W, ox, oy, tid);
-  __syncthreads();
-  for (int e = tid; e < kSH * (kST / 4); e += 256) {
-    const int r = e / (kST / 4), c0 = 4 * (e - r * (kST / 4));
-    float va[14], vb[14], vc[14];
-    ssim_row14(ta, r, c0, va);
-    ssim_row14(tb, r, c0, vb);
-    ssim_row14(tc, r, c0, vc);
-#pragma unroll
-    for (int o = 0; o < 4; ++o) {
-      float a = 0.f, b = 0.f, cc = 0.f;
-#pragma unroll
-      for (int k = 0; k < 11; ++k) {
-        const float w = win.g[k];
-        a = fmaf(w, va[o + k], a); b = fmaf(w, vb[o + k], b); cc = fmaf(w, vc[o + k], cc);
-      }
-      hq[0][r][c0 + o] = a; hq[1][r][c0 + o] = b; hq[2][r][c0 + o] = cc;
-    }
-  }
-  __syncthreads();
-  const float sc = gscale[0] * inv_n;
-  const int tx = tid % kST, ty0 = (tid / kST) * kSO;
-  const int x = ox + tx;
-  float h[3][kSO + 10];
-#pragma unroll
-  for (int q = 0; q < 3; ++q)
-#pragma unroll
-    for (int k = 0; k < kSO + 10; ++k) h[q][k] = hq[q][ty0 + k][tx];
-#pragma unroll
-  for (int o4 = 0; o4 < kSO; ++o4) {
-    const int y = oy + ty0 + o4;
-    if (x < W && y < H) {
-      float a = 0.f, b = 0.f, cc = 0.f;
-#pragma unroll
-      for (int k = 0; k < 11; ++k) {
-        const float w = win.g[k];
-        a = fmaf(w, h[0][o4 + k], a); b = fmaf(w, h[1][o4 + k], b); cc = fmaf(w, h[2][o4 + k], cc);
-      }
-      const size_t o = po + (size_t)y * W + x;
-      gimg1[o] = sc * (a + 2.f * img1[o] * b + img2[o] * cc);
-    }
-  }
-}
-
-__global__ __launch_bounds__(256) void ssim_finish_kernel(const float* __restrict__ partial, int count, float scale, float offset,
-                                                         float* __restrict__ out) {
-  __shared__ float red[4];
+  SsimGradPlanes sink{img1, img2, gimg1, gscale[0] * inv_n};
+  ssim_bwd_tile<VEC>(win, sink, dA, dB, dC, true, H, W);
+}
+
+template <bool VEC>
+__global__ __launch_bounds__(256) void image_loss_bwd_kernel(SsimWindow win, const float* __restrict__ rgba, const float* __restrict__ imgs,
+                                                            const long long* __restrict__ seg, const float* __restrict__ dA,
+                                                            const float* __restrict__ dB, const float* __restrict__ dC,
+                                                            const float* __restrict__ g_photo, const float* __restrict__ g_ssim,
+                                                            const float* __restrict__ fwd_out, float inv_n, float n3, float l_tex,
+                                                            float l_mrgb, int H, int W, float* __restrict__ grad_rgba) {
+  const int plane = blockIdx.z, b = plane / 3, c = plane - 3 * b;
+  const size_t HW = (size_t)H * W;
+  const float kt = (g_photo ? g_photo[0] : 0.f) * l_tex / n3;
+  const float km = (g_photo ? g_photo[1] : 0.f) * l_mrgb * 2.f * fwd_out[3] / n3;
+  ImageLossGrad sink{rgba + ((size_t)b * 4 + c) * HW, rgba + ((size_t)b * 4 + 3) * HW, imgs + (size_t)plane * HW, seg + (size_t)b * HW,
+                     grad_rgba + ((size_t)b * 4 + c) * HW, c == 0 ? grad_rgba + ((size_t)b * 4 + 3) * HW : nullptr,
+                     g_ssim ? g_ssim[0] * inv_n : 0.f, kt, km};
+  ssim_bwd_tile<VEC>(win, sink, dA, dB, dC, g_ssim != nullptr, H, W);
+}
+
+__device__ __forceinline__ float ssim_partial_sum(const float* __restrict__ partial, int count, float* red) {
   float s0 = 0.f, s1 = 0.f, s2 = 0.f, s3 = 0.f;
   int i = threadIdx.x;
   for (; i + 768 < count; i += 1024) { s0 += partial[i]; s1 += partial[i + 256]; s2 += partial[i + 512]; s3 += partial[i + 768]; }
   for (; i < count; i += 256) s0 += partial[i];
-  const float s = block_sum_256((s0 + s1) + (s2 + s3), red);
+  return block_sum_256((s0 + s1) + (s2 + s3), red);
+}
+
+__global__ __launch_bounds__(256) void ssim_finish_kernel(const float* __restrict__ partial, int count, float scale, float offset,
+                                                         float* __restrict__ out) {
+  __shared__ float red[4];
+  const float s = ssim_partial_sum(partial, count, red);
   if (threadIdx.x == 0) out[0] = offset + scale * s;
 }
 
+__global__ __launch_bounds__(256) void image_loss_finish_kernel(const float* __restrict__ partial, const float* __restrict__ photo, int count,
+                                                               float n3, float n1, float l_tex, float l_mrgb, float l_sil,
+                                                               float ssim_scale, float ssim_offset, float* __restrict__ out_photo,
+                                                               float* __restrict__ out_ssim) {
+  __shared__ float red[4], red4[4][4];
+  const float sv = ssim_partial_sum(partial, count, red);
+  float s[4] = {0.f, 0.f, 0.f, 0.f};
+#pragma unroll 4
+  for (int i = threadIdx.x; i < count; i += 256) {
+#pragma unroll
+    for (int q = 0; q < 4; ++q) s[q] += photo[(size_t)q * count + i];
+  }
+#pragma unroll
+  for (int q = 0; q < 4; ++q) {
+#pragma unroll
+    for (int o = 32; o > 0; o >>= 1) s[q] += __shfl_down(s[q], o, 64);
+  }
+  const int lane = threadIdx.x & 63, wave = threadIdx.x >> 6;
+  if (lane == 0) {
+#pragma unroll
+    for (int q = 0; q < 4; ++q) red4[q][wave] = s[q];
+  }
+  __syncthreads();
+  if (threadIdx.x == 0) {
+#pragma unroll
+    for (int q = 0; q < 4; ++q) s[q] = (red4[q][0] + red4[q][1]) + (red4[q][2] + red4[q][3]);
+    const float dm = s[1] / n3 - s[2] / n3;
+    out_photo[0] = l_tex * s[0] / n3;
+    out_photo[1] = l_mrgb * dm * dm;
+    out_photo[2] = l_sil * s[3] / n1;
+    out_photo[3] = dm;
+    out_ssim[0] = ssim_offset + ssim_scale * sv;
+  }
+}
+
 int ssim_tile_edge() { return kST; }
 
-static bool ssim_vec_ok(int W, const float* a, const float* b, const float* c) {
+static dim3 ssim_grid(int planes, int H, int W) { return dim3((W + kST - 1) / kST, (H + kST - 1) / kST, planes); }
+
+static bool ssim_vec_ok(int W, const void* a, const void* b, const void* c) {
   return W % 4 == 0 && ((reinterpret_cast<uintptr_t>(a) | reinterpret_cast<uintptr_t>(b) | reinterpret_cast<uintptr_t>(c)) & 15) == 0;
 }
 
@@ -213,7 +421,7 @@
 
 hipError_t launch_ssim_fwd(const SsimWindow& win, const float* img1, const float* img2, int planes, int H, int W, float* partial,
                            float* dA, float* dB, float* dC, hipStream_t st) {
-  const dim3 grid((W + kST - 1) / kST, (H + kST - 1) / kST, planes);
+  const dim3 grid = ssim_grid(planes, H, W);
   if (ssim_vec_ok(W, img1, img2, nullptr))
     hipLaunchKernelGGL(ssim_fwd_kernel<true>, grid, dim3(256), 0, st, win, img1, img2, H, W, partial, dA, dB, dC);
   else
@@ -223,7 +431,7 @@
 
 hipError_t launch_ssim_bwd(const SsimWindow& win, const float* img1, const float* img2, const float* dA, const float* dB,
                            const float* dC, const float* gscale, int planes, int H, int W, float* gimg1, hipStream_t st, float out_scale) {
-  const dim3 grid((W + kST - 1) / kST, (H + kST - 1) / kST, planes);
+  const dim3 grid = ssim_grid(planes, H, W);
   const float inv_n = out_scale / ((float)planes * (float)H * (float)W);
   if (ssim_vec_ok(W, dA, dB, dC))
     hipLaunchKernelGGL(ssim_bwd_kernel<true>, grid, dim3(256), 0, st, win, img1, img2, dA, dB, dC, gscale, inv_n, H, W, gimg1);
@@ -232,4 +440,34 @@
   return hipGetLastError();
 }
 
-}
+hipError_t launch_image_loss_fwd(const SsimWindow& win, const float* rgba, const float* imgs, const long long* seg, int B, int H, int W,
+                                 float l_tex, float l_mrgb, float l_sil, float l_ssim, float* dA, float* dB, float* dC, float* partial,
+                                 float* out_photo, float* out_ssim, hipStream_t st) {
+  const dim3 grid = ssim_grid(3 * B, H, W);
+  const int count = (int)(grid.x * grid.y * grid.z);
+  float* photo = partial + count;
+  if (ssim_vec_ok(W, rgba, imgs, seg))
+    hipLaunchKernelGGL(image_loss_fwd_kernel<true>, grid, dim3(256), 0, st, win, rgba, imgs, seg, H, W, partial, photo, dA, dB, dC);
+  else
+    hipLaunchKernelGGL(image_loss_fwd_kernel<false>, grid, dim3(256), 0, st, win, rgba, imgs, seg, H, W, partial, photo, dA, dB, dC);
+  const float n3 = (float)B * 3.f * ((float)H * (float)W), n1 = (float)B * ((float)H * (float)W);
+  hipLaunchKernelGGL(image_loss_finish_kernel, dim3(1), dim3(256), 0, st, partial, photo, count, n3, n1, l_tex, l_mrgb, l_sil,
+                     (float)(-(double)l_ssim / ((double)B * 3.0 * H * W)), l_ssim, out_photo, out_ssim);
+  return hipGetLastError();
+}
+
+hipError_t launch_image_loss_bwd(const SsimWindow& win, const float* rgba, const float* imgs, const long long* seg, const float* dA,
+                                 const float* dB, const float* dC, const float* g_photo, const float* g_ssim, const float* fwd_out_photo,
+                                 int B, int H, int W, float l_tex, float l_mrgb, float l_ssim, float* grad_rgba, hipStream_t st) {
+  const dim3 grid = ssim_grid(3 * B, H, W);
+  const float inv_n = -l_ssim / ((float)(3 * B) * (float)H * (float)W), n3 = (float)B * 3.f * (H * W);
+  if (ssim_vec_ok(W, dA, dB, dC) && ssim_vec_ok(W, rgba, imgs, seg))
+    hipLaunchKernelGGL(image_loss_bwd_kernel<true>, grid, dim3(256), 0, st, win, rgba, imgs, seg, dA, dB, dC, g_photo, g_ssim, fwd_out_photo,
+                       inv_n, n3, l_tex, l_mrgb, H, W, grad_rgba);
+  else
+    hipLaunchKernelGGL(image_loss_bwd_kernel<false>, grid, dim3(256), 0, st, win, rgba, imgs, seg, dA, dB, dC, g_photo, g_ssim, fwd_out_photo,
+                       inv_n, n3, l_tex, l_mrgb, H, W, grad_rgba);
+  return hipGetLastError();
+}
+
+}
diff --git a/hifihr_amd/losses.py b/hifihr_amd/losses.py
--- a/hifihr_amd/losses.py
+++ b/hifihr_amd/losses.py
@@ -144,11 +144,16 @@
             rgba = outputs.get("_rgba")
             if rgba is None:
                 rgba = torch.cat([outputs["re_img"], (outputs["re_sil"] > 0).to(outputs["re_img"].dtype)], 1)
-            out, re_img, mask_rgbs = ops.photo_losses(rgba, examples["imgs"], examples["segms_gt"], args.lambda_texture,
-                                                      args.lambda_mrgb, args.lambda_silhouette)
+            if ops.image_losses_supported(rgba):
+                out, ssim_tex = ops.image_losses(rgba, examples["imgs"], examples["segms_gt"], args.lambda_texture, args.lambda_mrgb,
+                                                 args.lambda_silhouette, args.lambda_ssim_tex)
+            else:
+                out, re_img, mask_rgbs = ops.photo_losses(rgba, examples["imgs"], examples["segms_gt"], args.lambda_texture,
+                                                          args.lambda_mrgb, args.lambda_silhouette)
+                ssim_tex = ops.ssim_loss(re_img, mask_rgbs, args.lambda_ssim_tex)
             tex, mrgb, sil, _ = out.unbind(0)
             loss_dic["texture"], loss_dic["mrgb"] = tex, mrgb
-            loss_dic["ssim_tex"] = ops.ssim_loss(re_img, mask_rgbs, args.lambda_ssim_tex)
+            loss_dic["ssim_tex"] = ssim_tex
             if "sil" in loss_used:
                 loss_dic["sil"] = sil
                 self._total_parts.append((out, 3, ["texture", "mrgb", "sil"]))
diff --git a/hifihr_amd/ops.py b/hifihr_amd/ops.py
--- a/hifihr_amd/ops.py
+++ b/hifihr_amd/ops.py
@@ -1867,6 +1867,53 @@
     return _PhotoLoss.apply(rgba, imgs, seg, float(l_tex), float(l_mrgb), float(l_sil))
 
 
+class _ImageLoss(torch.autograd.Function):
+
+    @staticmethod
+    def forward(ctx, rgba, imgs, seg, l_tex, l_mrgb, l_sil, l_ssim):
+        global _SSIM_WIN
+        require_cuda(rgba, imgs, seg)
+        lib = get_lib()
+        if _SSIM_WIN is None:
+            _SSIM_WIN = _ssim_window()
+        rgba, imgs, seg = rgba.contiguous(), imgs.contiguous(), seg.contiguous()
+        B, _, H, W = rgba.shape
+        need = ctx.needs_input_grad[0]
+        maps = torch.empty(3, B, 3, H, W, device=rgba.device) if need else None
+        partial = torch.empty(lib.image_loss_partial_floats(B, H, W), device=rgba.device)
+        out_photo, out_ssim = torch.empty(4, device=rgba.device), torch.empty((), device=rgba.device)
+        PROFILE.bracket("image_loss_fwd", lambda: lib.image_loss_fwd(_SSIM_WIN, rgba, imgs, seg, l_tex, l_mrgb, l_sil, l_ssim,
+                                                                    maps[0] if need else None, maps[1] if need else None,
+                                                                    maps[2] if need else None, partial, out_photo, out_ssim))
+        if need:
+            ctx.save_for_backward(rgba, imgs, seg, maps, out_photo)
+        ctx.lams = (l_tex, l_mrgb, l_ssim)
+        ctx.set_materialize_grads(False)
+        return out_photo, out_ssim
+
+    @staticmethod
+    def backward(ctx, g_photo, g_ssim):
+        if g_photo is None and g_ssim is None:
+            return (None,) * 7
+        rgba, imgs, seg, maps, out_photo = ctx.saved_tensors
+        grad = torch.empty_like(rgba)
+        g_photo = g_photo.contiguous() if g_photo is not None else None
+        if g_ssim is not None:
+            g_ssim = g_ssim.reshape(1) if (g_ssim.dtype == torch.float32 and g_ssim.is_contiguous()) else g_ssim.reshape(1).float().contiguous()
+        PROFILE.bracket("image_loss_bwd", lambda: get_lib().image_loss_bwd(_SSIM_WIN, rgba, imgs, seg, maps[0], maps[1], maps[2], g_photo,
+                                                                          g_ssim, out_photo, ctx.lams[0], ctx.lams[1], ctx.lams[2], grad))
+        return grad, None, None, None, None, None, None
+
+
+def image_losses_supported(rgba):
+    return rgba.dim() == 4 and rgba.shape[1] == 4 and rgba.shape[0] > 0 and rgba.shape[2] * rgba.shape[3] > 0 and (
+        rgba.shape[2] * rgba.shape[3]) % 4 == 0
+
+
+def image_losses(rgba, imgs, seg, l_tex, l_mrgb, l_sil, l_ssim):
+    return _ImageLoss.apply(rgba, imgs, seg, float(l_tex), float(l_mrgb), float(l_sil), float(l_ssim))
+
+
 def sil_post(rgba, images):
     require_cuda(rgba, images)
     rgba = rgba.detach().contiguous()
diff --git a/include/hifihr.h b/include/hifihr.h
--- a/include/hifihr.h
+++ b/include/hifihr.h
@@ -374,6 +374,13 @@
                           float* grad_rgba_d, void* stream);
 int hifihr_sil_post(const float* rgba_d, const float* imgs_d, int B, int H, int W, float* re_sil_d, float* mask_rgbs_d,
                     void* stream);
+int hifihr_image_loss_fwd(const float* window11_h, const float* rgba_d, const float* imgs_d, const int64_t* seg_d, int B, int H, int W,
+                          float l_tex, float l_mrgb, float l_sil, float l_ssim, float* dA_d, float* dB_d, float* dC_d, float* partial_d,
+                          float* out_photo_d, float* out_ssim_d, void* stream);
+int hifihr_image_loss_bwd(const float* window11_h, const float* rgba_d, const float* imgs_d, const int64_t* seg_d, const float* dA_d,
+                          const float* dB_d, const float* dC_d, const float* g_photo_d, const float* g_ssim_d,
+                          const float* fwd_out_photo_d, int B, int H, int W, float l_tex, float l_mrgb, float l_ssim, float* grad_rgba_d,
+                          void* stream);
 int hifihr_loss_total_fwd(const float* const* parts, const int* counts, int nparts, float* total_d, void* stream);
 int hifihr_loss_total_bwd(const float* gtotal_d, float* const* grads, const int* counts, const int* lengths, int nparts,
                           void* stream);
```

Measured after the change: 6755 images/sec (median of 6 runs). No clear change (+0.8%).
